# mohammadmarghzari/monte-carlo-portfolio

Measured on AMD Instinct MI355X. Metric: simulated paths/sec (16 assets x 252 steps) + VaR abs-err vs NumPy ref, higher is better.
Workload: dtype f32; 1 GPU; configs[1]: 16 synthetic assets, 1,000,000 paths per GPU, 252 steps, fp32, full pass = paths + moments + exact VaR/CVaR; n_assets=16, n_steps=252, parallelism=path-sharded x1, math=exact

## Files before the change

### include/mcport.h

```cpp
#ifndef MCPORT_H
#define MCPORT_H

#include <stddef.h>
#include <stdint.h>

#ifdef __cplusplus
extern "C" {
#endif

#define MCP_ABI_VERSION 4
#define MCP_MAX_ASSETS 64
#define MCP_SELECT_BINS 2048
#define MCP_MAX_HORIZONS 64
#define MCP_MAX_LEVELS 16
#define MCP_MAX_BOOT_ROWS (1 << 20)
#define MCP_MAX_OVERLAY_ROWS 8
#define MCP_MAX_T_DOF 32
#define MCP_MAX_ATTR_PORTFOLIOS 16
#define MCP_MAX_JUMPS 8

enum {
    MCP_OK = 0,
    MCP_E_ARG = -1,
    MCP_E_NODEVICE = -2,
// ... 63 lines not shown
    MCP_EXCHANGE_P2P = 4
};
int mcp_ctx_exchange_mode(const mcp_ctx *ctx);
const char *mcp_ctx_exchange_note(const mcp_ctx *ctx);
void mcp_ctx_destroy(mcp_ctx *ctx);

int mcp_ctx_set_terminal_budget(mcp_ctx *ctx, size_t bytes);

int mcp_simulate(mcp_ctx *ctx, const mcp_params *prm,
                 const float *mu,
                 const float *chol,
                 const float *W,
                 uint64_t seed, uint64_t path_begin, uint64_t n_paths,
                 float *terminal_out,
                 mcp_stats *stats_out  );

int mcp_simulate_drawdown(mcp_ctx *ctx, const mcp_params *prm, const float *mu, const float *chol, const float *W,
                          uint64_t seed, uint64_t path_begin, uint64_t n_paths,
                          float *terminal_out,
                          mcp_stats *stats_out,
                          float *mdd_out,
                          mcp_stats *dd_stats_out  );

int mcp_simulate_horizons(mcp_ctx *ctx, const mcp_params *prm, const float *mu, const float *chol, const float *W,
                          uint64_t seed, uint64_t path_begin, uint64_t n_paths,
                          int n_horizons, const int32_t *horizons,
                          int n_levels, const double *levels,
                          float *terminal_out,
                          mcp_stats *stats_out,
                          float *horizon_out,
                          mcp_stats *hz_stats_out,
                          double *bands_out);

typedef struct {
    const float *rows;
    int32_t n_rows;
    int32_t reserved;
    double mean_block;
} mcp_bootstrap;

int mcp_simulate_bootstrap(mcp_ctx *ctx, const mcp_params *prm, const mcp_bootstrap *boot, const float *W, uint64_t seed,
                           uint64_t path_begin, uint64_t n_paths, float *terminal_out, mcp_stats *stats_out);
int mcp_simulate_bootstrap_horizons(mcp_ctx *ctx, const mcp_params *prm, const mcp_bootstrap *boot, const float *W,
                                    uint64_t seed, uint64_t path_begin, uint64_t n_paths,
                                    int n_horizons, const int32_t *horizons,
                                    int n_levels, const double *levels,
                                    float *terminal_out,
                                    mcp_stats *stats_out,
                                    float *horizon_out,
                                    mcp_stats *hz_stats_out,
                                    double *bands_out);
int mcp_bootstrap_pivots(const mcp_params *prm, const mcp_bootstrap *boot, const float *W, double *pivots_out );

typedef struct {
    int32_t period;
    int32_t reserved;
    double cost;
} mcp_rebalance;

int mcp_simulate_rebalanced(mcp_ctx *ctx, const mcp_params *prm, const mcp_rebalance *reb,
                            const float *mu, const float *chol,
                            const mcp_bootstrap *boot,
                            const float *W, uint64_t seed, uint64_t path_begin, uint64_t n_paths,
                            int n_horizons, const int32_t *horizons,
                            int n_levels, const double *levels,
                            float *terminal_out,
                            mcp_stats *stats_out,
                            float *horizon_out,
                            mcp_stats *hz_stats_out,
                            double *bands_out);
int mcp_rebalance_pivots(const mcp_params *prm, const mcp_rebalance *reb, const float *mu, const mcp_bootstrap *boot,
                         const float *W, double *pivots_out );

typedef struct {
    int32_t dof;
    int32_t reserved;
} mcp_student_t;

int mcp_simulate_student_t(mcp_ctx *ctx, const mcp_params *prm, const mcp_student_t *st,
                           const float *mu, const float *chol, const float *W,
                           uint64_t seed, uint64_t path_begin, uint64_t n_paths,
                           int n_horizons, const int32_t *horizons, int n_levels, const double *levels,
                           float *terminal_out,
                           mcp_stats *stats_out,
                           float *mdd_out,
                           mcp_stats *dd_stats_out,
                           float *horizon_out,
                           mcp_stats *hz_stats_out,
                           double *bands_out);

typedef struct {
    double alpha, beta, h0;
    uint64_t reserved;
} mcp_garch;

int mcp_simulate_garch(mcp_ctx *ctx, const mcp_params *prm, const mcp_garch *g,
                       const mcp_student_t *st,
                       const float *mu, const float *chol, const float *W,
                       uint64_t seed, uint64_t path_begin, uint64_t n_paths,
                       int n_horizons, const int32_t *horizons, int n_levels, const double *levels,
                       float *terminal_out,
                       mcp_stats *stats_out,
                       float *mdd_out,
                       mcp_stats *dd_stats_out,
                       float *horizon_out,
                       mcp_stats *hz_stats_out,
                       double *bands_out);

typedef struct {
    const float *mu, *resid, *shock;
    int32_t n_rows;
    int32_t reserved;
    double mean_block;
} mcp_filtered;

int mcp_simulate_filtered(mcp_ctx *ctx, const mcp_params *prm, const mcp_filtered *filt, const mcp_garch *g, const float *W,
                          uint64_t seed, uint64_t path_begin, uint64_t n_paths,
                          int n_horizons, const int32_t *horizons, int n_levels, const double *levels,
                          float *terminal_out,
                          mcp_stats *stats_out,
                          float *horizon_out,
                          mcp_stats *hz_stats_out,
                          double *bands_out);
int mcp_filtered_pivots(const mcp_params *prm, const mcp_filtered *filt, const float *W, double *pivots_out );

typedef struct {
    double intensity, mean, std;
    const float *loading;
    int32_t reserved;
} mcp_jumps;

int mcp_simulate_jumps(mcp_ctx *ctx, const mcp_params *prm, const mcp_jumps *j,
                       const float *mu, const float *chol, const float *W,
                       uint64_t seed, uint64_t path_begin, uint64_t n_paths,
                       int n_horizons, const int32_t *horizons, int n_levels, const double *levels,
                       float *terminal_out,
                       mcp_stats *stats_out,
                       float *mdd_out,
                       mcp_stats *dd_stats_out,
                       float *horizon_out,
                       mcp_stats *hz_stats_out,
                       double *bands_out);
int mcp_jump_consts(const mcp_jumps *j, int n_assets, const float *mu,
                    uint32_t *thr_out , double *mean_count_out, float *drift_out );

typedef struct {
    double p01, p10, start;
    const float *mu1;
    const float *chol1;
    int32_t reserved;
} mcp_regimes;

int mcp_simulate_regimes(mcp_ctx *ctx, const mcp_params *prm, const mcp_regimes *r,
                         const float *mu, const float *chol, const float *W,
                         uint64_t seed, uint64_t path_begin, uint64_t n_paths,
                         int n_horizons, const int32_t *horizons, int n_levels, const double *levels,
                         float *terminal_out,
                         mcp_stats *stats_out,
                         float *mdd_out,
                         mcp_stats *dd_stats_out,
                         float *horizon_out,
                         mcp_stats *hz_stats_out,
                         double *bands_out);
int mcp_regime_consts(const mcp_regimes *r, uint64_t *thr_out , double *p_out );
int mcp_regime_pivots(const mcp_params *prm, const mcp_regimes *r, const float *mu, const float *W,
                      int n_horizons, const int32_t *horizons, double *pivots_out , double *hz_pivots_out );

typedef struct {
    uint64_t n_pairs, reserved;
    double cross, pair_cov, pair_corr, mean_se, mean_se_iid;
} mcp_pair;

int mcp_simulate_antithetic(mcp_ctx *ctx, const mcp_params *prm,
                            const mcp_garch *g,
                            const mcp_student_t *st,
                            const float *mu, const float *chol, const float *W,
                            uint64_t seed, uint64_t path_begin, uint64_t n_paths,
                            int n_horizons, const int32_t *horizons, int n_levels, const double *levels,
                            float *terminal_out,
                            mcp_stats *stats_out,
                            float *mdd_out,
                            mcp_stats *dd_stats_out,
                            float *horizon_out,
                            mcp_stats *hz_stats_out,
                            double *bands_out,
                            mcp_pair *pair_out);

typedef struct {
    double mean;
    double cvar;
    double vol;
    double sum, sum_tail, sum_xc;
} mcp_attr;

int mcp_simulate_attribution(mcp_ctx *ctx, const mcp_params *prm,
                             const mcp_garch *g,
                             const mcp_student_t *st,
                             const float *mu, const float *chol, const float *W,
                             uint64_t seed, uint64_t path_begin, uint64_t n_paths,
                             float *terminal_out,
                             mcp_stats *stats_out,
                             float *contrib_out,
                             mcp_attr *attr_out,
                             uint64_t *attr_counts_out);

typedef struct {
    const float *flows;
    int32_t n_flows;
    int32_t has_target;
    double target;
} mcp_cashflow;

int mcp_simulate_cashflow(mcp_ctx *ctx, const mcp_params *prm, const mcp_cashflow *cf,
                          const float *mu, const float *chol,
                          const mcp_bootstrap *boot,
                          const mcp_student_t *st,
                          const float *W, uint64_t seed, uint64_t path_begin, uint64_t n_paths,
                          int n_horizons, const int32_t *horizons, int n_levels, const double *levels,
                          float *terminal_out,
                          mcp_stats *stats_out,
                          uint64_t *counts_out,
                          float *horizon_out,
                          mcp_stats *hz_stats_out,
                          double *bands_out,
                          uint64_t *hz_counts_out);
int mcp_cashflow_pivots(const mcp_params *prm, const mcp_cashflow *cf, const float *mu, const mcp_bootstrap *boot,
                        const float *W, double *pivots_out );

#define MCP_OVERLAY_LINEAR 0
#define MCP_OVERLAY_CALL 1
#define MCP_OVERLAY_PUT 2
typedef struct {
    int32_t kind;
    float strike, premium, qty;
} mcp_overlay_row;
typedef struct {
    const mcp_overlay_row *rows;
    const int32_t *row_begin;
    const float *spot;
    int32_t n_rows;
    int32_t reserved;
} mcp_overlay;

int mcp_simulate_overlay(mcp_ctx *ctx, const mcp_params *prm, const mcp_overlay *ov,
                         const float *mu, const float *chol,
                         const mcp_student_t *st,
                         const float *W, uint64_t seed, uint64_t path_begin, uint64_t n_paths,
                         int n_horizons, const int32_t *horizons, int n_levels, const double *levels,
                         float *terminal_out,
                         mcp_stats *stats_out,
                         float *mdd_out,
                         mcp_stats *dd_stats_out,
                         float *horizon_out,
                         mcp_stats *hz_stats_out,
                         double *bands_out);
int mcp_overlay_pivots(const mcp_params *prm, const mcp_overlay *ov, const float *mu, const float *W,
                       double *pivots_out );

#define MCP_SWEEP_MAX_ROWS 4096
int mcp_sweep_historical(mcp_ctx *ctx, int n_assets, int n_rows, int n_portfolios, const double *returns,
                         const double *mean, const double *cov, const double *W, double rf, double alpha,
                         double *port_return, double *port_std, double *sharpe, double *var, double *cvar);


enum {
    MCP_WS_PARTIALS = 0,
    MCP_WS_RECORD = 1,
    MCP_WS_STATE = 2,
    MCP_WS_HIST = 3,
    MCP_WS_QUANT = 4,
    MCP_WS_STATS = 5,
    MCP_WS_BELOW = 6,
    MCP_WS_PIVOT = 7,
    MCP_WS_COUNT = 8
};
size_t mcp_ws_bytes(int which, int n_portfolios, uint64_t n_paths);
uint64_t mcp_moment_slots(int n_portfolios, uint64_t n_paths);

size_t mcp_packed_len(int n_assets, int n_portfolios);
int mcp_pack_params(int n_assets, int n_portfolios, const float *mu, const float *chol, const float *W,
                    float *packed_out, size_t packed_len);
int mcp_pivots(const mcp_params *prm, const float *mu, const float *chol, const float *W, double *pivots_out );

int mcp_launch_paths(const mcp_params *prm, const float *d_packed, const double *d_pivot, uint64_t seed, uint64_t path_begin,
                     uint64_t n_paths, float *d_terminal, uint64_t terminal_stride, void *d_partials, void *d_hist,
                     void *stream);
int mcp_launch_paths_drawdown(const mcp_params *prm, const float *d_packed, const double *d_pivot, uint64_t seed,
                              uint64_t path_begin, uint64_t n_paths, float *d_terminal, uint64_t terminal_stride,
                              float *d_mdd, uint64_t mdd_stride, void *d_partials, void *d_hist, void *stream);
int mcp_launch_paths_horizons(const mcp_params *prm, const float *d_packed, const double *d_pivot, uint64_t seed,
                              uint64_t path_begin, uint64_t n_paths, float *d_terminal, uint64_t terminal_stride,
                              int n_horizons, const int32_t *horizons, float *d_horizon, uint64_t horizon_stride,
                              void *d_partials, void *d_hist, void *stream);

int mcp_percentile_rank(uint64_t n_total, double alpha, uint64_t *rank_lo, uint64_t *rank_hi, double *gamma);
int mcp_percentile_rank_q(uint64_t n_total, double q, uint64_t *rank_lo, uint64_t *rank_hi, double *gamma);

int mcp_launch_pass0(const mcp_params *prm, const float *d_terminal, uint64_t terminal_stride, uint64_t n,
                     const double *d_pivot, void *d_partials, void *d_hist, void *stream);
int mcp_launch_scan(const mcp_params *prm, int pass, uint64_t n, uint64_t rank_lo, uint64_t rank_hi, const void *d_partials,
                    const void *d_below, const double *d_pivot, void *d_hist, void *d_state, void *d_record, void *stream);
int mcp_launch_hist(const mcp_params *prm, int pass, const float *d_terminal, uint64_t terminal_stride, uint64_t n,
                    const void *d_state, const double *d_pivot, void *d_below, void *d_hist, void *stream);
int mcp_launch_final(const mcp_params *prm, uint64_t n, double gamma, uint64_t rank_lo, uint64_t rank_hi,
                     const void *d_below, void *d_hist, const void *d_state, void *d_record, void *d_quant,
                     void *d_stats, void *stream);
int mcp_launch_stats(const mcp_params *prm, int world, const void *d_gathered, const void *d_quant, void *d_stats,
                     void *stream);
int mcp_launch_sum_u64(void *const *d_bufs, int n_bufs, size_t words, void *stream);

int mcp_stream_create(int device, int reserve_cus, void **stream_out);
int mcp_stream_destroy(void *stream);

int mcp_launch_normals(const uint32_t *d_x, uint64_t n, float *d_z, void *stream);

int mcp_icdf_table(float *out, size_t out_len);

uint32_t mcp_float_to_key(float v);
float mcp_key_to_float(uint32_t key);
double mcp_terminal_to_x(const mcp_params *prm, float terminal);

#ifdef __cplusplus
}
#endif
#endif
```

### monte_carlo_portfolio_amd/_ffi.py

```python
from __future__ import annotations

import ctypes
import importlib.util
import os
import subprocess
import sys

import numpy as np

_PKG = os.path.dirname(os.path.abspath(__file__))
LIB_PATH = os.environ.get("MCP_LIB_PATH") or os.path.join(_PKG, "libmcport.so")
CSRC = os.path.join(_PKG, "csrc")

MCP_ABI_VERSION = 4
MCP_MAX_ASSETS = 64
MCP_SELECT_BINS = 2048
MCP_MAX_HORIZONS = 64
MCP_MAX_LEVELS = 16
MCP_MAX_BOOT_ROWS = 1 << 20
MCP_MAX_T_DOF = 32
MCP_MAX_OVERLAY_ROWS = 8
MCP_MAX_ATTR_PORTFOLIOS = 16
MCP_MAX_JUMPS = 8
MCP_OVERLAY_LINEAR, MCP_OVERLAY_CALL, MCP_OVERLAY_PUT = 0, 1, 2
MCP_COMPOUND = {"simple": 0, "log": 1}
MCP_FLAG_NATIVE_MATH = 1
MCP_FLAG_FOLD = 2
MCP_FLAG_SHARD_PORTFOLIOS = 4
MCP_E_ARG, MCP_E_NODEVICE, MCP_E_NOMEM, MCP_E_UNSUPPORTED, MCP_E_HIP, MCP_E_COMM = -1, -2, -3, -4, -5, -6
(WS_PARTIALS, WS_RECORD, WS_STATE, WS_HIST, WS_QUANT, WS_STATS, WS_BELOW, WS_PIVOT) = range(8)
WS_COUNT = 8
(EXCHANGE_UNSET, EXCHANGE_NONE, EXCHANGE_RCCL, EXCHANGE_KERNEL, EXCHANGE_P2P) = range(5)


class McpError(RuntimeError):
    """Raised for any negative return code of the C ABI; carries mcp_last_error()."""


class McpParams(ctypes.Structure):
    _fields_ = [
        ("n_assets", ctypes.c_int32), ("n_steps", ctypes.c_int32), ("n_portfolios", ctypes.c_int32),
        ("compounding", ctypes.c_int32), ("flags", ctypes.c_int32), ("reserved", ctypes.c_int32),
        ("v0", ctypes.c_double), ("alpha", ctypes.c_double), ("rf", ctypes.c_double),
    ]


class McpStats(ctypes.Structure):
    _fields_ = [
        ("n", ctypes.c_uint64), ("n_tail", ctypes.c_uint64), ("mean", ctypes.c_double), ("m2", ctypes.c_double),
        ("std", ctypes.c_double), ("sharpe", ctypes.c_double), ("var", ctypes.c_double), ("cvar", ctypes.c_double),
        ("min", ctypes.c_double), ("max", ctypes.c_double), ("sum_tail", ctypes.c_double),
        ("x_lo", ctypes.c_double), ("x_hi", ctypes.c_double),
    ]


class McpBootstrap(ctypes.Structure):
    _fields_ = [("rows", ctypes.c_void_p), ("n_rows", ctypes.c_int32), ("reserved", ctypes.c_int32), ("mean_block", ctypes.c_double)]


class McpRebalance(ctypes.Structure):
    _fields_ = [("period", ctypes.c_int32), ("reserved", ctypes.c_int32), ("cost", ctypes.c_double)]


class McpStudentT(ctypes.Structure):
    _fields_ = [("dof", ctypes.c_int32), ("reserved", ctypes.c_int32)]


class McpFiltered(ctypes.Structure):
    _fields_ = [("mu", ctypes.c_void_p), ("resid", ctypes.c_void_p), ("shock", ctypes.c_void_p), ("n_rows", ctypes.c_int32),
                ("reserved", ctypes.c_int32), ("mean_block", ctypes.c_double)]


class McpGarch(ctypes.Structure):
    _fields_ = [("alpha", ctypes.c_double), ("beta", ctypes.c_double), ("h0", ctypes.c_double), ("reserved", ctypes.c_uint64)]


class McpJumps(ctypes.Structure):
    _fields_ = [("intensity", ctypes.c_double), ("mean", ctypes.c_double), ("std", ctypes.c_double), ("loading", ctypes.c_void_p),
                ("reserved", ctypes.c_int32)]


class McpRegimes(ctypes.Structure):
    _fields_ = [("p01", ctypes.c_double), ("p10", ctypes.c_double), ("start", ctypes.c_double), ("mu1", ctypes.c_void_p),
                ("chol1", ctypes.c_void_p), ("reserved", ctypes.c_int32)]


class McpCashflow(ctypes.Structure):
    _fields_ = [("flows", ctypes.c_void_p), ("n_flows", ctypes.c_int32), ("has_target", ctypes.c_int32), ("target", ctypes.c_double)]


class McpOverlay(ctypes.Structure):
    _fields_ = [("rows", ctypes.c_void_p), ("row_begin", ctypes.c_void_p), ("spot", ctypes.c_void_p), ("n_rows", ctypes.c_int32),
                ("reserved", ctypes.c_int32)]


OVERLAY_ROW_DTYPE = np.dtype([("kind", np.int32), ("strike", np.float32), ("premium", np.float32), ("qty", np.float32)])
assert OVERLAY_ROW_DTYPE.itemsize == 16

STATS_DTYPE = np.dtype([
    ("n", np.uint64), ("n_tail", np.uint64), ("mean", np.float64), ("m2", np.float64), ("std", np.float64),
    ("sharpe", np.float64), ("var", np.float64), ("cvar", np.float64), ("min", np.float64), ("max", np.float64),
    ("sum_tail", np.float64), ("x_lo", np.float64), ("x_hi", np.float64),
])
assert STATS_DTYPE.itemsize == ctypes.sizeof(McpStats)

ATTR_DTYPE = np.dtype([("mean", np.float64), ("cvar", np.float64), ("vol", np.float64), ("sum", np.float64), ("sum_tail", np.float64),
                       ("sum_xc", np.float64)])
assert ATTR_DTYPE.itemsize == 48

PAIR_DTYPE = np.dtype([("n_pairs", np.uint64), ("reserved", np.uint64), ("cross", np.float64), ("pair_cov", np.float64),
                       ("pair_corr", np.float64), ("mean_se", np.float64), ("mean_se_iid", np.float64)])
assert PAIR_DTYPE.itemsize == 56

RECORD_DTYPE = np.dtype([("n", np.float64), ("sum", np.float64), ("sumsq", np.float64), ("min", np.float64),
                         ("max", np.float64), ("below", np.float64), ("pivot", np.float64), ("pad", np.float64)])
PARTIAL_DTYPE = np.dtype([("s1", np.float64), ("s2", np.float64), ("vmin", np.float32), ("vmax", np.float32), ("n", np.uint64)])
assert PARTIAL_DTYPE.itemsize == 32
QUANT_DTYPE = np.dtype([("x_lo", np.float64), ("x_hi", np.float64), ("var", np.float64), ("level2", np.float64),
                        ("n_tail", np.uint64), ("pad", np.uint64)])
RECORD_DOUBLES = RECORD_DTYPE.itemsize // 8

_f32p = np.ctypeslib.ndpointer(dtype=np.float32, flags="C_CONTIGUOUS")
_f64p = np.ctypeslib.ndpointer(dtype=np.float64, flags="C_CONTIGUOUS")
_vp = ctypes.c_void_p
_u64 = ctypes.c_uint64
_int = ctypes.c_int
_PP = ctypes.POINTER(McpParams)

SIGNATURES = {
    "mcp_abi_version": (_int, []),
    "mcp_device_count": (_int, []),
    "mcp_last_error": (ctypes.c_char_p, []),
    "mcp_ctx_create": (_int, [_int, ctypes.POINTER(_vp)]),
    "mcp_ctx_create_multi": (_int, [ctypes.POINTER(_int), _int, ctypes.POINTER(_vp)]),
    "mcp_ctx_device_count": (_int, [_vp]),
    "mcp_ctx_exchange_mode": (_int, [_vp]),
    "mcp_ctx_exchange_note": (ctypes.c_char_p, [_vp]),
    "mcp_ctx_set_terminal_budget": (_int, [_vp, ctypes.c_size_t]),
    "mcp_ctx_destroy": (None, [_vp]),
    "mcp_simulate": (_int, [_vp, _PP, _f32p, _f32p, _f32p, _u64, _u64, _u64, _vp, _vp]),
    "mcp_sweep_historical": (_int, [_vp, _int, _int, _int, _f64p, _f64p, _f64p, _f64p, ctypes.c_double, ctypes.c_double,
                                    _f64p, _f64p, _f64p, _f64p, _f64p]),
    "mcp_ws_bytes": (ctypes.c_size_t, [_int, _int, _u64]),
    "mcp_moment_slots": (_u64, [_int, _u64]),
    "mcp_pivots": (_int, [_PP, _f32p, _f32p, _f32p, _f64p]),
    "mcp_packed_len": (ctypes.c_size_t, [_int, _int]),
    "mcp_pack_params": (_int, [_int, _int, _f32p, _f32p, _f32p, _f32p, ctypes.c_size_t]),
    "mcp_launch_paths": (_int, [_PP, _vp, _vp, _u64, _u64, _u64, _vp, _u64, _vp, _vp, _vp]),
    "mcp_simulate_drawdown": (_int, [_vp, _PP, _f32p, _f32p, _f32p, _u64, _u64, _u64, _vp, _vp, _vp, _vp]),
    "mcp_launch_paths_drawdown": (_int, [_PP, _vp, _vp, _u64, _u64, _u64, _vp, _u64, _vp, _u64, _vp, _vp, _vp]),
    "mcp_simulate_horizons": (_int, [_vp, _PP, _f32p, _f32p, _f32p, _u64, _u64, _u64, _int, _vp, _int, _vp, _vp, _vp, _vp, _vp,
                                     _vp]),
    "mcp_launch_paths_horizons": (_int, [_PP, _vp, _vp, _u64, _u64, _u64, _vp, _u64, _int, _vp, _vp, _u64, _vp, _vp, _vp]),
    "mcp_simulate_bootstrap": (_int, [_vp, _PP, ctypes.POINTER(McpBootstrap), _f32p, _u64, _u64, _u64, _vp, _vp]),
    "mcp_simulate_bootstrap_horizons": (_int, [_vp, _PP, ctypes.POINTER(McpBootstrap), _f32p, _u64, _u64, _u64, _int, _vp, _int, _vp,
                                               _vp, _vp, _vp, _vp, _vp]),
    "mcp_bootstrap_pivots": (_int, [_PP, ctypes.POINTER(McpBootstrap), _f32p, _f64p]),
    "mcp_simulate_rebalanced": (_int, [_vp, _PP, ctypes.POINTER(McpRebalance), _vp, _vp, ctypes.POINTER(McpBootstrap), _f32p, _u64, _u64,
                                       _u64, _int, _vp, _int, _vp, _vp, _vp, _vp, _vp, _vp]),
    "mcp_rebalance_pivots": (_int, [_PP, ctypes.POINTER(McpRebalance), _vp, ctypes.POINTER(McpBootstrap), _f32p, _f64p]),
    "mcp_simulate_student_t": (_int, [_vp, _PP, ctypes.POINTER(McpStudentT), _vp, _vp, _vp, _u64, _u64, _u64, _int, _vp, _int, _vp, _vp,
                                      _vp, _vp, _vp, _vp, _vp, _vp]),
    "mcp_simulate_garch": (_int, [_vp, _PP, ctypes.POINTER(McpGarch), ctypes.POINTER(McpStudentT), _vp, _vp, _vp, _u64, _u64, _u64, _int,
                                  _vp, _int, _vp, _vp, _vp, _vp, _vp, _vp, _vp, _vp]),
    "mcp_simulate_filtered": (_int, [_vp, _PP, ctypes.POINTER(McpFiltered), ctypes.POINTER(McpGarch), _vp, _u64, _u64, _u64, _int, _vp,
                                     _int, _vp, _vp, _vp, _vp, _vp, _vp]),
    "mcp_filtered_pivots": (_int, [_PP, ctypes.POINTER(McpFiltered), _f32p, _f64p]),
    "mcp_simulate_jumps": (_int, [_vp, _PP, ctypes.POINTER(McpJumps), _vp, _vp, _vp, _u64, _u64, _u64, _int, _vp, _int, _vp, _vp, _vp,
                                  _vp, _vp, _vp, _vp, _vp]),
    "mcp_jump_consts": (_int, [ctypes.POINTER(McpJumps), _int, _vp, _vp, ctypes.POINTER(ctypes.c_double), _vp]),
    "mcp_simulate_regimes": (_int, [_vp, _PP, ctypes.POINTER(McpRegimes), _vp, _vp, _vp, _u64, _u64, _u64, _int, _vp, _int, _vp, _vp, _vp,
                                    _vp, _vp, _vp, _vp, _vp]),
    "mcp_regime_consts": (_int, [ctypes.POINTER(McpRegimes), _vp, _vp]),
    "mcp_regime_pivots": (_int, [_PP, ctypes.POINTER(McpRegimes), _vp, _vp, _int, _vp, _vp, _vp]),
    "mcp_simulate_attribution": (_int, [_vp, _PP, ctypes.POINTER(McpGarch), ctypes.POINTER(McpStudentT), _vp, _vp, _vp, _u64, _u64, _u64,
                                        _vp, _vp, _vp, _vp, _vp]),
    "mcp_simulate_antithetic": (_int, [_vp, _PP, ctypes.POINTER(McpGarch), ctypes.POINTER(McpStudentT), _vp, _vp, _vp, _u64, _u64, _u64,
                                       _int, _vp, _int, _vp, _vp, _vp, _vp, _vp, _vp, _vp, _vp, _vp]),
    "mcp_simulate_cashflow": (_int, [_vp, _PP, ctypes.POINTER(McpCashflow), _vp, _vp, ctypes.POINTER(McpBootstrap),
                                     ctypes.POINTER(McpStudentT), _vp, _u64, _u64, _u64, _int, _vp, _int, _vp, _vp, _vp, _vp, _vp, _vp,
                                     _vp, _vp]),
    "mcp_cashflow_pivots": (_int, [_PP, ctypes.POINTER(McpCashflow), _vp, ctypes.POINTER(McpBootstrap), _f32p, _f64p]),
    "mcp_simulate_overlay": (_int, [_vp, _PP, ctypes.POINTER(McpOverlay), _vp, _vp, ctypes.POINTER(McpStudentT), _vp, _u64, _u64, _u64,
                                    _int, _vp, _int, _vp, _vp, _vp, _vp, _vp, _vp, _vp, _vp]),
    "mcp_overlay_pivots": (_int, [_PP, ctypes.POINTER(McpOverlay), _f32p, _f32p, _f64p]),
    "mcp_percentile_rank_q": (_int, [_u64, ctypes.c_double, ctypes.POINTER(_u64), ctypes.POINTER(_u64),
                                     ctypes.POINTER(ctypes.c_double)]),
    "mcp_percentile_rank": (_int, [_u64, ctypes.c_double, ctypes.POINTER(_u64), ctypes.POINTER(_u64),
                                   ctypes.POINTER(ctypes.c_double)]),
    "mcp_launch_pass0": (_int, [_PP, _vp, _u64, _u64, _vp, _vp, _vp, _vp]),
    "mcp_launch_scan": (_int, [_PP, _int, _u64, _u64, _u64, _vp, _vp, _vp, _vp, _vp, _vp, _vp]),
    "mcp_launch_hist": (_int, [_PP, _int, _vp, _u64, _u64, _vp, _vp, _vp, _vp, _vp]),
    "mcp_launch_final": (_int, [_PP, _u64, ctypes.c_double, _u64, _u64, _vp, _vp, _vp, _vp, _vp, _vp, _vp]),
    "mcp_launch_stats": (_int, [_PP, _int, _vp, _vp, _vp, _vp]),
    "mcp_launch_sum_u64": (_int, [ctypes.POINTER(_vp), _int, ctypes.c_size_t, _vp]),
    "mcp_stream_create": (_int, [_int, _int, ctypes.POINTER(_vp)]),
    "mcp_stream_destroy": (_int, [_vp]),
    "mcp_launch_normals": (_int, [_vp, _u64, _vp, _vp]),
    "mcp_icdf_table": (_int, [_f32p, ctypes.c_size_t]),
    "mcp_float_to_key": (ctypes.c_uint32, [ctypes.c_float]),
    "mcp_key_to_float": (ctypes.c_float, [ctypes.c_uint32]),
    "mcp_terminal_to_x": (ctypes.c_double, [_PP, ctypes.c_float]),
}

_LIB = None


def build(force: bool = False, jobs: int = 8) -> str:
    cmd = ["make", "-C", CSRC, f"-j{jobs}"] + (["-B"] if force else [])
    res = subprocess.run(cmd, capture_output=True, text=True)
    if res.returncode != 0:
        raise RuntimeError("building libmcport.so failed:\n" + res.stdout[-4000:] + res.stderr[-4000:])
    return LIB_PATH


def _preload_hip_runtime() -> None:
    if "torch" in sys.modules:
        return
    try:
        spec = importlib.util.find_spec("torch")
    except (ImportError, ValueError):
        spec = None
    if spec is not None and spec.origin:
        cand = os.path.join(os.path.dirname(spec.origin), "lib", "libamdhip64.so")
        if os.path.exists(cand):
            ctypes.CDLL(cand, mode=ctypes.RTLD_GLOBAL)


def preload_rccl() -> None:
    if os.environ.get("MCP_RCCL_LIB"):
        return
    try:
        spec = importlib.util.find_spec("torch")
    except (ImportError, ValueError):
        spec = None
    if spec is not None and spec.origin:
        cand = os.path.join(os.path.dirname(spec.origin), "lib", "librccl.so")
        if os.path.exists(cand):
            try:
                ctypes.CDLL(cand)
            except OSError:
                pass


def lib() -> ctypes.CDLL:
    global _LIB
    if _LIB is None:
        _preload_hip_runtime()
        if not os.path.exists(LIB_PATH):
            raise ImportError(
                f"{LIB_PATH} is missing: build it with `make -C {CSRC} -j8` (or __graft_entry__.build()). "
                "There is no CPU fallback for the path engine.")
        L = ctypes.CDLL(LIB_PATH)
        for name, (res, args) in SIGNATURES.items():
            fn = getattr(L, name)
            fn.restype = res
            fn.argtypes = args
        got = L.mcp_abi_version()
        if got != MCP_ABI_VERSION:
            raise ImportError(f"libmcport.so ABI {got} != binding ABI {MCP_ABI_VERSION}; rebuild")
        _LIB = L
    return _LIB


def check(rc: int) -> int:
    if rc < 0:
        raise McpError(f"libmcport error {rc}: {lib().mcp_last_error().decode('utf-8', 'replace')}")
    return rc


def make_params(n_assets, n_steps, n_portfolios, compounding="simple", v0=1.0, alpha=0.95, rf=0.0,
                native_math=False, fold=False, shard_portfolios=False) -> McpParams:
    if compounding not in MCP_COMPOUND:
        raise ValueError(f"compounding must be 'simple' or 'log', got {compounding!r}")
    return McpParams(int(n_assets), int(n_steps), int(n_portfolios), MCP_COMPOUND[compounding],
                     (MCP_FLAG_NATIVE_MATH if native_math else 0) | (MCP_FLAG_FOLD if fold else 0)
                     | (MCP_FLAG_SHARD_PORTFOLIOS if shard_portfolios else 0), 0,
                     float(v0), float(alpha), float(rf))


def pack_params(mu: np.ndarray, chol: np.ndarray, W: np.ndarray) -> np.ndarray:
    n = mu.shape[0]
    k = W.shape[0]
    out = np.zeros(lib().mcp_packed_len(n, k), np.float32)
    check(lib().mcp_pack_params(n, k, mu, chol, W, out, out.size))
    return out


def pivots(prm: McpParams, mu: np.ndarray, chol: np.ndarray, W: np.ndarray) -> np.ndarray:
    out = np.zeros(W.shape[0], np.float64)
    check(lib().mcp_pivots(ctypes.byref(prm), mu, chol, W, out))
    return out


def make_bootstrap(rows: np.ndarray, block: float) -> McpBootstrap:
    if rows.dtype != np.float32 or rows.ndim != 2 or not rows.flags.c_contiguous:
        raise ValueError("bootstrap rows must be a C-contiguous float32 [R, N] array")
    return McpBootstrap(rows.ctypes.data_as(ctypes.c_void_p), int(rows.shape[0]), 0, float(block))


def make_filtered(mu: np.ndarray, resid: np.ndarray, shock: np.ndarray, block: float) -> McpFiltered:
    for a, nd in ((mu, 1), (resid, 2), (shock, 1)):
        if a.dtype != np.float32 or a.ndim != nd or not a.flags.c_contiguous:
            raise ValueError("filtered mu [N], resid [R, N] and shock [R] must be C-contiguous float32 arrays")
    if resid.shape != (shock.shape[0], mu.shape[0]):
        raise ValueError(f"filtered resid has shape {resid.shape}, mu and shock want {(shock.shape[0], mu.shape[0])}")
    return McpFiltered(mu.ctypes.data_as(ctypes.c_void_p), resid.ctypes.data_as(ctypes.c_void_p), shock.ctypes.data_as(ctypes.c_void_p),
                       int(resid.shape[0]), 0, float(block))


def filtered_pivots(prm: McpParams, mu: np.ndarray, resid: np.ndarray, shock: np.ndarray, W: np.ndarray) -> np.ndarray:
    out = np.zeros(W.shape[0], np.float64)
    mu, resid, shock = (np.ascontiguousarray(a, np.float32) for a in (mu, resid, shock))
    ft = make_filtered(mu, resid, shock, 1.0)
    check(lib().mcp_filtered_pivots(ctypes.byref(prm), ctypes.byref(ft), W, out))
    return out


def make_jumps(intensity: float, mean: float, std: float, loading: np.ndarray | None = None) -> McpJumps:
    if loading is not None and (loading.dtype != np.float32 or loading.ndim != 1 or not loading.flags.c_contiguous):
        raise ValueError("jump loadings must be a C-contiguous float32 [N] array")
    return McpJumps(float(intensity), float(mean), float(std), loading.ctypes.data_as(ctypes.c_void_p) if loading is not None else None, 0)


def jump_consts(intensity: float, mean: float, std: float, loading=None, mu=None, n_assets: int | None = None):
    ld = np.ascontiguousarray(loading, np.float32) if loading is not None else None
    mu32 = np.ascontiguousarray(mu, np.float32) if mu is not None else None
    n = mu32.size if mu32 is not None else ld.size if ld is not None else int(n_assets or 1)
    thr = np.zeros(MCP_MAX_JUMPS, np.uint32)
    mean_count = ctypes.c_double()
    drift = np.zeros(n, np.float32) if mu32 is not None else None
    jp = make_jumps(intensity, mean, std, ld)
    ptr = lambda a: a.ctypes.data_as(_vp) if a is not None else None
    check(lib().mcp_jump_consts(ctypes.byref(jp), n, ptr(mu32), ptr(thr), ctypes.byref(mean_count), ptr(drift)))
    return thr, mean_count.value, drift


def make_regimes(p01: float, p10: float, start: float, mu1: np.ndarray | None, chol1: np.ndarray | None) -> McpRegimes:
    for a, nd in ((mu1, 1), (chol1, 2)):
        if a is not None and (a.dtype != np.float32 or a.ndim != nd or not a.flags.c_contiguous):
            raise ValueError("regime mu1 [N] and chol1 [N, N] must be C-contiguous float32 arrays")
    ptr = lambda a: a.ctypes.data_as(ctypes.c_void_p) if a is not None else None
    return McpRegimes(float(p01), float(p10), float(start), ptr(mu1), ptr(chol1), 0)


def regime_consts(p01: float, p10: float, start: float):
    thr, p = np.zeros(3, np.uint64), np.zeros(3, np.float64)
    rs = make_regimes(p01, p10, start, None, None)
    check(lib().mcp_regime_consts(ctypes.byref(rs), thr.ctypes.data_as(_vp), p.ctypes.data_as(_vp)))
    return thr, p


def regime_pivots(prm: McpParams, regimes, mu: np.ndarray, mu1: np.ndarray, W: np.ndarray, horizons=None):
    mu, mu1 = (np.ascontiguousarray(a, np.float32) for a in (mu, mu1))
    W = np.ascontiguousarray(W, np.float32)
    n = mu.size
    chol1 = np.zeros((n, n), np.float32)
    rs = make_regimes(*regimes, mu1, chol1)
    hz = np.ascontiguousarray(horizons, np.int32) if horizons is not None and len(horizons) else None
    out = np.zeros(W.shape[0], np.float64)
    hout = np.zeros((hz.size, W.shape[0]), np.float64) if hz is not None else None
    ptr = lambda a: a.ctypes.data_as(_vp) if a is not None else None
    check(lib().mcp_regime_pivots(ctypes.byref(prm), ctypes.byref(rs), ptr(mu), ptr(W), 0 if hz is None else hz.size, ptr(hz), ptr(out),
                                  ptr(hout)))
    return out, hout


def bootstrap_pivots(prm: McpParams, rows: np.ndarray, W: np.ndarray, block: float = 1.0) -> np.ndarray:
    out = np.zeros(W.shape[0], np.float64)
    rows = np.ascontiguousarray(rows, np.float32)
    bt = make_bootstrap(rows, block)
    check(lib().mcp_bootstrap_pivots(ctypes.byref(prm), ctypes.byref(bt), W, out))
    return out


def rebalance_pivots(prm: McpParams, period: int, W: np.ndarray, mu: np.ndarray | None = None, rows: np.ndarray | None = None,
                     cost: float = 0.0) -> np.ndarray:
    out = np.zeros(W.shape[0], np.float64)
    rb = McpRebalance(int(period), 0, float(cost))
    mu_p = np.ascontiguousarray(mu, np.float32) if mu is not None else None
    bt = make_bootstrap(np.ascontiguousarray(rows, np.float32), 1.0) if rows is not None else None
    check(lib().mcp_rebalance_pivots(ctypes.byref(prm), ctypes.byref(rb), mu_p.ctypes.data_as(_vp) if mu_p is not None else None,
                                     ctypes.byref(bt) if bt is not None else None, W, out))
    return out


def make_cashflow(flows: np.ndarray, target=None) -> McpCashflow:
    if flows.dtype != np.float32 or flows.ndim != 1 or not flows.flags.c_contiguous:
        raise ValueError("cash flows must be a C-contiguous float32 [n_steps] array")
    return McpCashflow(flows.ctypes.data_as(ctypes.c_void_p) if flows.size else None, int(flows.size), 0 if target is None else 1,
                       0.0 if target is None else float(target))


def cashflow_pivots(prm: McpParams, flows: np.ndarray, W: np.ndarray, mu: np.ndarray | None = None,
                    rows: np.ndarray | None = None) -> np.ndarray:
    out = np.zeros(W.shape[0], np.float64)
    flows = np.ascontiguousarray(flows, np.float32)
    cf = make_cashflow(flows)
    mu_p = np.ascontiguousarray(mu, np.float32) if mu is not None else None
    bt = make_bootstrap(np.ascontiguousarray(rows, np.float32), 1.0) if rows is not None else None
    check(lib().mcp_cashflow_pivots(ctypes.byref(prm), ctypes.byref(cf), mu_p.ctypes.data_as(_vp) if mu_p is not None else None,
                                    ctypes.byref(bt) if bt is not None else None, W, out))
    return out


def make_overlay(rows: np.ndarray, row_begin: np.ndarray, spot: np.ndarray) -> McpOverlay:
    if rows.dtype != OVERLAY_ROW_DTYPE or rows.ndim != 1 or not rows.flags.c_contiguous:
        raise ValueError("overlay rows must be a C-contiguous [n_rows] array of OVERLAY_ROW_DTYPE")
    if row_begin.dtype != np.int32 or spot.dtype != np.float32 or row_begin.ndim != 1 or spot.ndim != 1 or row_begin.size != spot.size + 1:
        raise ValueError("overlay row_begin must be int32 [N + 1] and spot float32 [N]")
    return McpOverlay(rows.ctypes.data_as(ctypes.c_void_p) if rows.size else None, row_begin.ctypes.data_as(ctypes.c_void_p),
                      spot.ctypes.data_as(ctypes.c_void_p), int(rows.size), 0)


def overlay_pivots(prm: McpParams, overlay, mu: np.ndarray, W: np.ndarray) -> np.ndarray:
    out = np.zeros(W.shape[0], np.float64)
    ov = make_overlay(*overlay)
    check(lib().mcp_overlay_pivots(ctypes.byref(prm), ctypes.byref(ov), np.ascontiguousarray(mu, np.float32), W, out))
    return out


def percentile_rank_q(n_total: int, q: float):
    lo, hi, g = _u64(), _u64(), ctypes.c_double()
    check(lib().mcp_percentile_rank_q(n_total, q, ctypes.byref(lo), ctypes.byref(hi), ctypes.byref(g)))
    return lo.value, hi.value, g.value


def percentile_rank(n_total: int, alpha: float):
    lo, hi, g = _u64(), _u64(), ctypes.c_double()
    check(lib().mcp_percentile_rank(n_total, alpha, ctypes.byref(lo), ctypes.byref(hi), ctypes.byref(g)))
    return lo.value, hi.value, g.value
```

### monte_carlo_portfolio_amd/csrc/mcp_api.cpp

```cpp
#include <hip/hip_runtime.h>
#include <dlfcn.h>

#include <algorithm>
#include <cmath>
#include <cstdarg>
#include <cstdio>
#include <cstdlib>
#include <cstring>
#include <mutex>
#include <new>
#include <string>
#include <vector>

#include "../../include/mcport.h"
#include "mcp_device.h"
#include "mcp_paths.h"
#include "mcp_stats_kernels.h"

#ifndef MCP_EXP_LEAN
#define MCP_EXP_LEAN 1
#endif

namespace {

thread_local std::string g_err;

int fail(int code, const char* fmt, ...) {
  char buf[512];
  va_list ap;
  va_start(ap, fmt);
  vsnprintf(buf, sizeof buf, fmt, ap);
  va_end(ap);
  g_err = buf;
  return code;
}

#define HIP_TRY(expr)                                                                       \
  do {                                                                                      \
    hipError_t e_ = (expr);                                                                 \
    if (e_ != hipSuccess) return fail(MCP_E_HIP, "%s: %s", #expr, hipGetErrorString(e_)); \
  } while (0)

constexpr int KT_WIDE = 8;
constexpr int K_PAD = 512;
using mcp::SWEEP_MIN_K;

int env_sweep_mt() {
  static const int v = [] { const char* e = getenv("MCP_SWEEP_MT"); return e ? atoi(e) : 0; }();
  return v;
}
bool uses_sweep(int K) { return K >= SWEEP_MIN_K && env_sweep_mt() >= 0; }

struct SweepSeg { bool shared; int mt, k_begin, k_count; };
int sweep_plan(int K, int nb, SweepSeg* out) {
  int n = 0;
  const int env_mt = env_sweep_mt();
  if (nb <= 4 && env_mt > 0) {
    out[n++] = {false, env_mt, 0, K};
    return n;
  }
  const int big = nb <= 4 ? 4 : 2, W = 128 * big;
  const int full = (K / W) * W;
  if (full) out[n++] = {true, big, 0, full};
  const int r = K - full;
  if (r == 0) return n;
  if (nb <= 4) {
    const auto per_wave = [](int k) { return k > 64 ? 4 : (k > 32 ? 2 : 1); };
    if (r <= 128) out[n++] = {false, per_wave(r), full, r};
    else if (r <= 256) out[n++] = {true, 2, full, r};
    else if (r <= 384) { out[n++] = {true, 2, full, 256}; out[n++] = {false, per_wave(r - 256), full + 256, r - 256}; }
    else out[n++] = {true, 4, full, r};
  } else {
    out[n++] = {true, r <= 128 ? 1 : 2, full, r};
  }
  return n;
}

inline int n4_of(int n) { return 4 * ((n + 3) / 4); }
inline size_t regime_block_len(int n) { const size_t n4 = (size_t)n4_of(n); return n4 + n4 * (n4 / 2 + 1); }
inline int kpad_of(int k) { return k >= SWEEP_MIN_K ? K_PAD * ((k + K_PAD - 1) / K_PAD) : KT_WIDE * ((k + KT_WIDE - 1) / KT_WIDE); }

int check_params(const mcp_params* p) {
  if (!p) return fail(MCP_E_ARG, "params is NULL");
  if (p->n_assets < 1 || p->n_assets > MCP_MAX_ASSETS)
    return fail(MCP_E_ARG, "n_assets=%d outside [1,%d]", p->n_assets, MCP_MAX_ASSETS);
  if (p->n_steps < 0) return fail(MCP_E_ARG, "n_steps=%d < 0", p->n_steps);
  if (p->n_portfolios < 1) return fail(MCP_E_ARG, "n_portfolios=%d < 1", p->n_portfolios);
  if (p->compounding != MCP_COMPOUND_SIMPLE && p->compounding != MCP_COMPOUND_LOG)
    return fail(MCP_E_ARG, "compounding=%d unknown", p->compounding);
  if (!(p->alpha > 0.0 && p->alpha < 1.0)) return fail(MCP_E_ARG, "alpha=%g outside (0,1)", p->alpha);
  if (!(p->v0 > 0.0) || !std::isfinite(p->v0)) return fail(MCP_E_ARG, "v0=%g must be positive", p->v0);
  return MCP_OK;
}

const mcp::launch_paths_fn k_launch[16] = {
    mcp::launch_paths_nb1,  mcp::launch_paths_nb2,  mcp::launch_paths_nb3,  mcp::launch_paths_nb4,
    mcp::launch_paths_nb5,  mcp::launch_paths_nb6,  mcp::launch_paths_nb7,  mcp::launch_paths_nb8,
    mcp::launch_paths_nb9,  mcp::launch_paths_nb10, mcp::launch_paths_nb11, mcp::launch_paths_nb12,
    mcp::launch_paths_nb13, mcp::launch_paths_nb14, mcp::launch_paths_nb15, mcp::launch_paths_nb16};

int check_horizons(int n_steps, int H, const int32_t* steps) {
  if (H < 1 || H > MCP_MAX_HORIZONS) return fail(MCP_E_ARG, "n_horizons=%d outside [1,%d]", H, MCP_MAX_HORIZONS);
  if (!steps) return fail(MCP_E_ARG, "horizons is NULL");
  for (int i = 0; i < H; i++) {
    if (steps[i] < 1 || steps[i] > n_steps) return fail(MCP_E_ARG, "horizon %d = %d outside [1, n_steps=%d]", i, steps[i], n_steps);
    if (i && steps[i] <= steps[i - 1]) return fail(MCP_E_ARG, "horizons must be strictly increasing (%d after %d)", steps[i], steps[i - 1]);
  }
  return MCP_OK;
}

int check_levels(int L, const double* levels) {
  if (L < 0 || L > MCP_MAX_LEVELS) return fail(MCP_E_ARG, "n_levels=%d outside [0,%d]", L, MCP_MAX_LEVELS);
  if (L && !levels) return fail(MCP_E_ARG, "levels is NULL");
  for (int i = 0; i < L; i++)
    if (!(levels[i] >= 0.0 && levels[i] <= 100.0)) return fail(MCP_E_ARG, "level %d = %g outside [0, 100]", i, levels[i]);
  return MCP_OK;
}

int check_boot(const mcp_params* prm, const mcp_bootstrap* boot) {
  if (!boot) return fail(MCP_E_ARG, "bootstrap is NULL");
  if (!boot->rows) return fail(MCP_E_ARG, "bootstrap rows is NULL");
  if (boot->n_rows < 1 || boot->n_rows > MCP_MAX_BOOT_ROWS)
    return fail(MCP_E_ARG, "n_rows=%d outside [1,%d]", boot->n_rows, MCP_MAX_BOOT_ROWS);
  const double b = boot->mean_block;
  if (!(b >= 1.0)) return fail(MCP_E_ARG, "mean_block=%g must be >= 1 (or +inf)", b);
  const size_t n = (size_t)boot->n_rows * (size_t)prm->n_assets;
  for (size_t i = 0; i < n; i++)
    if (!std::isfinite(boot->rows[i]))
      return fail(MCP_E_ARG, "bootstrap row %zu, asset %zu is not finite", i / (size_t)prm->n_assets, i % (size_t)prm->n_assets);
  return MCP_OK;
}

uint64_t boot_threshold(double b) {
  const double q = 4294967296.0 / b;
  return q >= 4294967296.0 ? (uint64_t)1 << 32 : (uint64_t)q;
}

void boot_moments(int N, const mcp_bootstrap* boot, const float* W, int K, double* m_out, double* s2_out) {
  const int R = boot->n_rows;
  std::vector<double> rho((size_t)R);
  for (int k = 0; k < K; k++) {
    const float* w = W + (size_t)k * N;
    double sum = 0.0;
    for (int j = 0; j < R; j++) {
      const float* r = boot->rows + (size_t)j * N;
      double v = 0.0;
      for (int i = 0; i < N; i++) v += (double)w[i] * (double)r[i];
      rho[(size_t)j] = v;
      sum += v;
    }
    const double m = sum / (double)R;
    double ss = 0.0;
    for (int j = 0; j < R; j++) { const double d = rho[(size_t)j] - m; ss += d * d; }
    m_out[k] = m;
    s2_out[k] = ss / (double)R;
  }
}

double boot_pivot(int compounding, int T, double m, double s2) {
  const double c = compounding == MCP_COMPOUND_LOG ? std::expm1((double)T * (m + 0.5 * s2))
                                                   : (m > -1.0 ? std::expm1((double)T * std::log1p(m)) : 0.0);
  return std::isfinite(c) ? c : 0.0;
}

int check_reb(const mcp_rebalance* reb) {
  if (!reb) return fail(MCP_E_ARG, "rebalance is NULL");
  if (reb->period < 0) return fail(MCP_E_ARG, "rebalance period=%d < 0", reb->period);
  if (reb->reserved != 0) return fail(MCP_E_ARG, "rebalance reserved=%d must be 0", reb->reserved);
  if (!(reb->cost >= 0.0 && reb->cost < 1.0)) return fail(MCP_E_ARG, "rebalance cost=%g outside [0, 1)", reb->cost);
  return MCP_OK;
}

int check_student_t(const mcp_params* prm, const mcp_student_t* st) {
  if (!st) return fail(MCP_E_ARG, "student_t is NULL");
  if (st->dof < 3 || st->dof > MCP_MAX_T_DOF) return fail(MCP_E_ARG, "dof=%d outside [3,%d]", st->dof, MCP_MAX_T_DOF);
  if (st->reserved != 0) return fail(MCP_E_ARG, "student_t reserved=%d must be 0", st->reserved);
  if ((uint64_t)prm->n_steps * (uint64_t)((st->dof + 3) / 4) > 0xFFFFFFFFull)
    return fail(MCP_E_ARG, "n_steps * ceil(dof/4) = %llu exceeds the 32-bit Philox block counter of stream 2",
                (unsigned long long)((uint64_t)prm->n_steps * (uint64_t)((st->dof + 3) / 4)));
  return MCP_OK;
}

struct GarchConsts { float a, b, g, omega, a_n; };
GarchConsts garch_consts(const mcp_garch* g, int N) {
  GarchConsts c;
  c.a = (float)g->alpha;
  c.b = (float)g->beta;
  c.g = (float)g->h0;
  c.omega = (float)(1.0 - (double)c.a - (double)c.b);
  c.a_n = (float)((double)c.a / (double)N);
  return c;
}

int check_garch(const mcp_params* prm, const mcp_garch* g) {
  if (!g) return fail(MCP_E_ARG, "garch is NULL");
  if (g->reserved != 0) return fail(MCP_E_ARG, "garch reserved=%llu must be 0", (unsigned long long)g->reserved);
  if (!std::isfinite(g->alpha) || !std::isfinite(g->beta) || !std::isfinite(g->h0))
    return fail(MCP_E_ARG, "garch alpha=%g, beta=%g, h0=%g must be finite", g->alpha, g->beta, g->h0);
  const GarchConsts c = garch_consts(g, prm->n_assets);
  if (!std::isfinite(c.a) || !std::isfinite(c.b) || !std::isfinite(c.g))
    return fail(MCP_E_ARG, "garch alpha=%g, beta=%g, h0=%g must be finite in binary32", g->alpha, g->beta, g->h0);
  if (!(c.a >= 0.0f) || !(c.b >= 0.0f)) return fail(MCP_E_ARG, "garch alpha=%g and beta=%g must be >= 0", g->alpha, g->beta);
  if (!((double)c.a + (double)c.b < 1.0) || !(c.omega > 0.0f))
    return fail(MCP_E_ARG, "garch alpha + beta = %.9g must be < 1 in binary32", (double)c.a + (double)c.b);
  if (!(c.g > 0.0f)) return fail(MCP_E_ARG, "garch h0=%g must be > 0 in binary32", g->h0);
  return MCP_OK;
}

struct JumpConsts { uint32_t thr[MCP_MAX_JUMPS]; double mean_count; float m, s; };
JumpConsts jump_consts(const mcp_jumps* j) {
  JumpConsts c;
  double p = std::exp(-j->intensity), cum = 0.0;
  c.mean_count = 0.0;
  for (int k = 1; k <= MCP_MAX_JUMPS; k++) {
    cum = cum + p;
    double v = std::floor((1.0 - cum) * 4294967296.0);
    v = v < 0.0 ? 0.0 : v > 4294967295.0 ? 4294967295.0 : v;
    c.thr[k - 1] = (uint32_t)v;
    c.mean_count += (double)c.thr[k - 1] / 4294967296.0;
    p = p * j->intensity / (double)k;
  }
  c.m = (float)j->mean;
  c.s = (float)j->std;
  return c;
}
void jump_drift(const mcp_jumps* j, const JumpConsts& c, int N, const float* mu, float* out) {
  const double d = (double)c.m * c.mean_count;
  for (int i = 0; i < N; i++) {
    const float b = j->loading ? j->loading[i] : 1.0f;
    out[i] = (d == 0.0 || b == 0.0f) ? mu[i] : (float)((double)mu[i] - (double)b * d);
  }
}

int check_jumps(int n_assets, const mcp_jumps* j) {
  if (!j) return fail(MCP_E_ARG, "jumps is NULL");
  if (j->reserved != 0) return fail(MCP_E_ARG, "jumps reserved=%d must be 0", j->reserved);
  if (!std::isfinite(j->intensity) || !std::isfinite(j->mean) || !std::isfinite(j->std))
    return fail(MCP_E_ARG, "jumps intensity=%g, mean=%g, std=%g must be finite", j->intensity, j->mean, j->std);
  if (!std::isfinite((float)j->intensity) || !std::isfinite((float)j->mean) || !std::isfinite((float)j->std))
    return fail(MCP_E_ARG, "jumps intensity=%g, mean=%g, std=%g must be finite in binary32", j->intensity, j->mean, j->std);
  if (!(j->intensity >= 0.0 && j->intensity <= 1.0)) return fail(MCP_E_ARG, "jumps intensity=%g outside [0, 1]", j->intensity);
  if (!(j->std >= 0.0)) return fail(MCP_E_ARG, "jumps std=%g must be >= 0", j->std);
  for (int i = 0; j->loading && i < n_assets; i++)
    if (!std::isfinite(j->loading[i])) return fail(MCP_E_ARG, "jumps loading, asset %d is not finite", i);
  return MCP_OK;
}

struct RegimeConsts { uint64_t thr01, thr10, thr_start; double p01, p10, start; };
inline uint64_t regime_thr(double p) {
  const double v = std::floor(p * 4294967296.0);
  return v >= 4294967296.0 ? (uint64_t)1 << 32 : (uint64_t)v;
}
RegimeConsts regime_consts(const mcp_regimes* r) {
  RegimeConsts c;
  c.thr01 = regime_thr(r->p01);
  c.thr10 = regime_thr(r->p10);
  c.thr_start = regime_thr(r->start);
  c.p01 = (double)c.thr01 / 4294967296.0;
  c.p10 = (double)c.thr10 / 4294967296.0;
  c.start = (double)c.thr_start / 4294967296.0;
  return c;
}

int check_regimes(int n_assets, const mcp_regimes* r) {
  if (!r) return fail(MCP_E_ARG, "regimes is NULL");
  if (r->reserved != 0) return fail(MCP_E_ARG, "regimes reserved=%d must be 0", r->reserved);
  if (!std::isfinite(r->p01) || !std::isfinite(r->p10) || !std::isfinite(r->start))
    return fail(MCP_E_ARG, "regimes p01=%g, p10=%g, start=%g must be finite", r->p01, r->p10, r->start);
  if (!(r->p01 >= 0.0 && r->p01 <= 1.0) || !(r->p10 >= 0.0 && r->p10 <= 1.0) || !(r->start >= 0.0 && r->start <= 1.0))
    return fail(MCP_E_ARG, "regimes p01=%g, p10=%g, start=%g outside [0, 1]", r->p01, r->p10, r->start);
  if (!r->mu1 || !r->chol1) return fail(MCP_E_ARG, "regimes mu1 or chol1 is NULL");
  for (int i = 0; i < n_assets; i++)
    if (!std::isfinite(r->mu1[i])) return fail(MCP_E_ARG, "regimes mu1, asset %d is not finite", i);
  for (size_t i = 0; i < (size_t)n_assets * n_assets; i++)
    if (!std::isfinite(r->chol1[i])) return fail(MCP_E_ARG, "regimes chol1, entry %zu is not finite", i);
  return MCP_OK;
}

void regime_pivots(int N, int K, int T, const float* mu0, const float* mu1, const RegimeConsts& c, const float* W, int H, const int32_t* steps,
                   double* out_T, double* out_hz) {
  for (int k = 0; k < K; k++) {
    const float* w = W + (size_t)k * N;
    double d0 = 0.0, d1 = 0.0;
    for (int i = 0; i < N; i++) d0 += (double)w[i] * (double)(mu0[i] + 0.0f);
    for (int i = 0; i < N; i++) d1 += (double)w[i] * (double)(mu1[i] + 0.0f);
    const bool only0 = c.thr_start == 0 && c.thr01 == 0, only1 = c.thr_start == ((uint64_t)1 << 32) && c.thr10 == 0;
    const bool one_drift = d0 == d1 || only0 || only1;
    const double m = only1 ? d1 : d0;
    d0 = 1.0 + d0;
    d1 = 1.0 + d1;
    double v0 = (1.0 - c.start) * d0, v1 = c.start * d1;
    int hi = 0;
    if (out_T) out_T[k] = 0.0;
    for (int h = 1; h <= T; h++) {
      if (h > 1) {
        const double u0 = v0 * (1.0 - c.p01) + v1 * c.p10, u1 = v0 * c.p01 + v1 * (1.0 - c.p10);
        v0 = u0 * d0;
        v1 = u1 * d1;
      }
      const double ch = one_drift ? (m > -1.0 ? std::expm1((double)h * std::log1p(m)) : 0.0) : (v0 + v1) - 1.0;
      const double piv = std::isfinite(ch) ? ch : 0.0;
      if (hi < H && steps[hi] == h) out_hz[(size_t)hi++ * K + k] = piv;
      if (h == T && out_T) out_T[k] = piv;
    }
  }
}

int check_filtered(const mcp_params* prm, const mcp_filtered* f) {
  if (!f) return fail(MCP_E_ARG, "filtered is NULL");
  if (!f->mu) return fail(MCP_E_ARG, "filtered mu is NULL");
  if (!f->resid) return fail(MCP_E_ARG, "filtered resid is NULL");
  if (!f->shock) return fail(MCP_E_ARG, "filtered shock is NULL");
  if (f->n_rows < 1 || f->n_rows > MCP_MAX_BOOT_ROWS) return fail(MCP_E_ARG, "filtered n_rows=%d outside [1,%d]", f->n_rows, MCP_MAX_BOOT_ROWS);
  if (f->reserved != 0) return fail(MCP_E_ARG, "filtered reserved=%d must be 0", f->reserved);
  if (!(f->mean_block >= 1.0)) return fail(MCP_E_ARG, "filtered mean_block=%g must be >= 1 (or +inf)", f->mean_block);
  const size_t N = (size_t)prm->n_assets, R = (size_t)f->n_rows;
  for (size_t i = 0; i < N; i++)
    if (!std::isfinite(f->mu[i])) return fail(MCP_E_ARG, "filtered mu, asset %zu is not finite", i);
  for (size_t i = 0; i < R * N; i++)
    if (!std::isfinite(f->resid[i])) return fail(MCP_E_ARG, "filtered resid row %zu, asset %zu is not finite", i / N, i % N);
  for (size_t j = 0; j < R; j++) {
    if (!std::isfinite(f->shock[j])) return fail(MCP_E_ARG, "filtered shock, row %zu is not finite", j);
    if (!(f->shock[j] >= 0.0f)) return fail(MCP_E_ARG, "filtered shock, row %zu = %g is negative", j, (double)f->shock[j]);
// ... 731 lines not shown
static mcp::BootArgs boot_block(const Request& rq, const Launch& ln) {
  mcp::BootArgs bt;
  const bool on = rq.src == SRC_BOOT || rq.src == SRC_FHS;
  bt.rows = on ? (const float4*)ln.d_rows : nullptr;
  bt.thr = on ? boot_threshold(rows_of(rq).mean_block) : 0;
  bt.n_rows = on ? (uint32_t)rows_of(rq).n_rows : 0;
  bt.pad = 0;
  return bt;
}
static mcp::FiltArgs filt_block(const Request& rq, const Launch& ln, int n_assets) {
  const GarchConsts c = garch_consts(rq.gv, n_assets);
  mcp::FiltArgs fh;
  fh.shock = ln.d_rows + (size_t)rq.filt->n_rows * (size_t)n4_of(n_assets);
  fh.a = c.a;
  fh.b = c.b;
  fh.omega = c.omega;
  fh.h0 = c.g;
  return fh;
}
static mcp::StudentArgs student_block(const Request& rq) {
  mcp::StudentArgs st;
  st.dof = rq.src == SRC_T ? rq.st->dof : 0;
  st.pad = 0;
  return st;
}
static mcp::GarchArgs garch_block(const mcp_garch* g, int n_assets) {
  const GarchConsts c = garch_consts(g, n_assets);
  mcp::GarchArgs gv;
  gv.a_n = c.a_n;
  gv.b = c.b;
  gv.omega = c.omega;
  gv.h0 = c.g;
  gv.n_assets = n_assets;
  gv.pad = 0;
  return gv;
}
static mcp::JumpArgs jump_block(const Request& rq, const Launch& ln) {
  const JumpConsts c = jump_consts(rq.jp);
  mcp::JumpArgs jp;
  jp.loading = ln.d_loading;
  for (int k = 0; k < MCP_MAX_JUMPS; k++) jp.thr[k] = c.thr[k];
  jp.m = c.m;
  jp.s = c.s;
  return jp;
}
static mcp::RegimeArgs regime_block(const Request& rq, const Launch& ln) {
  const RegimeConsts c = regime_consts(rq.rs);
  mcp::RegimeArgs rs;
  rs.block1 = ln.d_block1;
  rs.thr01 = c.thr01;
  rs.thr10 = c.thr10;
  rs.thr_start = c.thr_start;
  return rs;
}
static mcp::OverlayArgs overlay_block(const Request& rq, const Launch& ln, int n_assets) {
  mcp::OverlayArgs ov;
  const size_t row_bytes = (size_t)rq.ov->n_rows * sizeof(mcp_overlay_row);
  ov.rows = (const mcp_overlay_row*)ln.d_overlay;
  ov.row_begin = (const int32_t*)(ln.d_overlay + row_bytes);
  ov.spot = (const float*)(ln.d_overlay + row_bytes) + n4_of(n_assets) + 1;
  ov.mask = 0;
  for (int i = 0; i < n_assets; i++)
    if (rq.ov->row_begin[i + 1] > rq.ov->row_begin[i]) ov.mask |= (uint64_t)1 << i;
  return ov;
}
static mcp::AttrArgs attr_block(const Launch& ln, int n_assets) {
  mcp::AttrArgs at;
  at.var = ln.d_var;
  at.partials = ln.d_attr_partials;
  at.contrib = ln.d_contrib;
  at.contrib_stride = ln.contrib_stride;
  at.n_assets = n_assets;
  at.pad = 0;
  return at;
}

static int launch_paths_impl(const mcp_params* prm, const Request& rq, const Launch& ln) {
  const int N = prm->n_assets, nb = (N + 3) / 4;
  const int K = prm->n_portfolios;
  const bool plain = rq.src == SRC_GAUSS && !rq.dd && !rq.hz && !rq.rebalanced && !rq.cash && !rq.overlay && !rq.garch && !rq.jumps && !rq.regimes;
  mcp::PathLaunchArgs s = {};
  mcp::PathArgs& a = s.hz;
  const float4* tables = nullptr;
  int dev = 0;
  if (int rc = stream_device(ln.stream, &dev)) return rc;
  DeviceGuard guard(dev);
  if (guard.err != hipSuccess) return fail(MCP_E_HIP, "hipSetDevice(%d): %s", dev, hipGetErrorString(guard.err));
  if (int rc = device_tables(dev, ln.stream, &tables)) return rc;
  const bool sweep = plain && !ln.attr && !rq.anti && uses_sweep(K);
  a.tables = tables;
  a.packed = ln.d_packed;
  a.terminal = ln.d_terminal;
  a.pivot = ln.d_pivot;
  a.partials = (mcp::MomentPartial*)ln.d_partials;
  a.hist = sweep ? nullptr : (unsigned long long*)ln.d_hist;
  a.slots = mcp_moment_slots(K, ln.n_paths);
  a.v0d = (double)(float)prm->v0;
  a.inv_v0d = 1.0 / a.v0d;
  { int e = 0; a.v0_pow2 = std::frexp(a.v0d, &e) == 0.5; }
  a.seed = ln.seed;
  a.path_begin = ln.path_begin;
  a.n_paths = ln.n_paths;
  a.stride = ln.stride;
  a.n_steps = prm->n_steps;
  a.n_portfolios = K;
  a.compounding = prm->compounding;
  a.v0 = (float)prm->v0;
  a.k_count = K;
  a.fold_offset = (uint32_t)(n4_of(N) + n4_of(N) * (n4_of(N) / 2 + 1) + kpad_of(K) * n4_of(N));
  if (rq.anti) {
    if ((ln.path_begin | ln.n_paths | ln.stride | (rq.dd ? ln.mdd_stride : 0) | (rq.hz ? ln.hz_stride : 0)) & 1)
      return fail(MCP_E_ARG, "antithetic pairs: a launch begins, ends and strides at even path ids");
    a.path_begin = ln.path_begin / 2;
    a.n_paths = ln.n_paths / 2;
    s.pr.cross = ln.d_partials ? ln.d_cross : nullptr;
  }
  if (sweep) {
    const bool native = (prm->flags & MCP_FLAG_NATIVE_MATH) != 0;
    SweepSeg segs[4];
    const int n_seg = sweep_plan(K, nb, segs);
    hipError_t e = hipSuccess;
    for (int i = 0; i < n_seg && e == hipSuccess; i++) {
      a.k_begin = segs[i].k_begin;
      a.k_count = segs[i].k_count;
      e = segs[i].shared ? mcp::launch_sweep_shared(nb, segs[i].mt, native, a, ln.stream)
                         : mcp::launch_sweep_paths(nb, segs[i].mt, native, a, ln.stream);
    }
    if (e != hipSuccess) return fail(MCP_E_HIP, "mc_sweep_kernel launch: %s", hipGetErrorString(e));
    if (ln.d_hist) {
      e = mcp::launch_hist(*prm, K, 0, ln.d_terminal, ln.stride, ln.n_paths, nullptr, ln.d_pivot, nullptr, (unsigned long long*)ln.d_hist,
                           ln.stream);
      if (e != hipSuccess) return fail(MCP_E_HIP, "hist_kernel<0> launch: %s", hipGetErrorString(e));
    }
    return MCP_OK;
  }
  if ((!plain || rq.anti) && ln.d_partials && a.slots > (uint64_t)mcp::path_grid(a.n_paths))
    HIP_TRY(mcp::launch_pass0(*prm, K, ln.d_terminal, ln.stride, 0, nullptr, a.slots, (mcp::MomentPartial*)ln.d_partials,
                              (unsigned long long*)ln.d_hist, ln.stream));
  fill_hz(s.hz, rq, ln);
  s.mdd = rq.dd ? ln.d_mdd : nullptr;
  s.mdd_stride = rq.dd ? ln.mdd_stride : 0;
  s.bt = boot_block(rq, ln);
  s.st = student_block(rq);
  if (rq.garch) s.gv = garch_block(rq.gv, N);
  if (rq.cash) s.cf.flows = ln.d_flows;
  if (rq.overlay) s.ov = overlay_block(rq, ln, N);
  if (rq.rebalanced) { s.period = rq.reb->period; s.cost = (float)rq.reb->cost; }
  if (rq.src == SRC_FHS) s.fh = filt_block(rq, ln, N);
  if (rq.jumps) s.jp = jump_block(rq, ln);
  if (rq.regimes) s.rs = regime_block(rq, ln);
  mcp::PathKernel k = {};
  k.logc = prm->compounding == MCP_COMPOUND_LOG;
  k.fh = rq.src == SRC_FHS;
  k.boot = rq.src == SRC_BOOT || k.fh;
  k.blds = k.fh ? mcp::filt_fits_lds((uint64_t)rq.filt->n_rows, nb) : k.boot && mcp::boot_fits_lds((uint64_t)rq.boot->n_rows, nb);
  k.stt = rq.src == SRC_T;
  if (ln.attr) {
    static const mcp_garch none = {0.0, 0.0, 1.0, 0};
    k.family = mcp::FAM_AT;
    k.stt = k.gv = true;
    a.partials = nullptr;
    a.hist = nullptr;
    if (!rq.garch) s.gv = garch_block(&none, N);
    s.at = attr_block(ln, N);
  } else {
    k.family = rq.overlay ? mcp::FAM_OV : rq.cash ? mcp::FAM_CF : rq.rebalanced ? mcp::FAM_REB : rq.dd ? mcp::FAM_DD : rq.hz ? mcp::FAM_HZ : mcp::FAM_PLAIN;
    k.dd = rq.overlay && rq.dd;
    k.gv = rq.garch;
    k.jp = rq.jumps;
    k.rs = rq.regimes;
    k.kt8 = K > 1;
    k.native = (prm->flags & MCP_FLAG_NATIVE_MATH) != 0;
    k.fold = (prm->flags & MCP_FLAG_FOLD) != 0;
    k.uhi = MCP_EXP_LEAN && plain && !rq.anti && !k.kt8 && !k.native && !k.fold && nb <= mcp::LEAN_MAX_NB && mcp::lean_range(a.path_begin, a.n_paths);
    if (rq.anti) {
      static const mcp_garch none = {0.0, 0.0, 1.0, 0};
      k.anti = true;
      if (k.stt || k.gv) {
        k.stt = k.gv = true;
        if (!rq.garch) s.gv = garch_block(&none, N);
      }
    }
  }
  const hipError_t e = k_launch[nb - 1](k, s, ln.stream);
  if (e != hipSuccess) return fail(MCP_E_HIP, "path kernel launch (family %d): %s", k.family, hipGetErrorString(e));
  return MCP_OK;
}

static Launch make_launch(const float* d_packed, const double* d_pivot, uint64_t seed, uint64_t path_begin, uint64_t n_paths,
                          float* d_terminal, uint64_t stride, void* d_partials, void* d_hist, void* stream) {
  Launch ln;
  ln.d_packed = d_packed;
  ln.d_pivot = d_pivot;
  ln.seed = seed;
  ln.path_begin = path_begin;
  ln.n_paths = n_paths;
  ln.d_terminal = d_terminal;
  ln.stride = stride;
  ln.d_partials = d_partials;
  ln.d_hist = d_hist;
  ln.stream = (hipStream_t)stream;
  return ln;
}

static int launch_checked(const mcp_params* prm, const Request& rq, const Launch& ln) {
  if (int rc = check_request(prm, rq, ln.n_paths, &ln)) return rc;
  return launch_paths_impl(prm, rq, ln);
}

extern "C" {

int mcp_launch_paths(const mcp_params* prm, const float* d_packed, const double* d_pivot, uint64_t seed, uint64_t path_begin,
                     uint64_t n_paths, float* d_terminal, uint64_t stride, void* d_partials, void* d_hist, void* stream) {
  return launch_checked(prm, Request(), make_launch(d_packed, d_pivot, seed, path_begin, n_paths, d_terminal, stride, d_partials, d_hist, stream));
}

int mcp_launch_paths_drawdown(const mcp_params* prm, const float* d_packed, const double* d_pivot, uint64_t seed, uint64_t path_begin,
                              uint64_t n_paths, float* d_terminal, uint64_t terminal_stride, float* d_mdd, uint64_t mdd_stride,
                              void* d_partials, void* d_hist, void* stream) {
  Request rq;
  rq.dd = true;
  Launch ln = make_launch(d_packed, d_pivot, seed, path_begin, n_paths, d_terminal, terminal_stride, d_partials, d_hist, stream);
  ln.d_mdd = d_mdd;
  ln.mdd_stride = mdd_stride;
  return launch_checked(prm, rq, ln);
}

int mcp_launch_paths_horizons(const mcp_params* prm, const float* d_packed, const double* d_pivot, uint64_t seed, uint64_t path_begin,
                              uint64_t n_paths, float* d_terminal, uint64_t terminal_stride, int n_horizons, const int32_t* horizons,
                              float* d_horizon, uint64_t horizon_stride, void* d_partials, void* d_hist, void* stream) {
  Request rq;
  ask_horizons(rq, true, n_horizons, horizons, 0, nullptr, nullptr, nullptr, nullptr);
  Launch ln = make_launch(d_packed, d_pivot, seed, path_begin, n_paths, d_terminal, terminal_stride, d_partials, d_hist, stream);
  ln.d_hz = d_horizon;
  ln.hz_stride = horizon_stride;
  return launch_checked(prm, rq, ln);
}

#define MCP_ON_STREAM_DEVICE(stream)                                                                     \
  int dev_ = 0;                                                                                          \
  if (int rc_ = stream_device((hipStream_t)(stream), &dev_)) return rc_;                                 \
  DeviceGuard guard_(dev_);                                                                              \
  if (guard_.err != hipSuccess) return fail(MCP_E_HIP, "hipSetDevice(%d): %s", dev_, hipGetErrorString(guard_.err))

int mcp_percentile_rank(uint64_t n, double alpha, uint64_t* rank_lo, uint64_t* rank_hi, double* gamma) {
  if (n < 1 || !rank_lo || !rank_hi || !gamma) return fail(MCP_E_ARG, "bad argument");
  const double pct = (1.0 - alpha) * 100.0;
  const double q = pct / 100.0;
  const double vi = (double)(n - 1) * q;
  if (vi >= (double)(n - 1)) { *rank_lo = *rank_hi = n - 1; *gamma = 0.0; return MCP_OK; }
  if (vi < 0.0) { *rank_lo = *rank_hi = 0; *gamma = 0.0; return MCP_OK; }
  const double fl = std::floor(vi);
  *rank_lo = (uint64_t)fl;
  *rank_hi = *rank_lo + 1;
  *gamma = vi - fl;
  return MCP_OK;
}

int mcp_percentile_rank_q(uint64_t n, double q, uint64_t* rank_lo, uint64_t* rank_hi, double* gamma) {
  if (n < 1 || !rank_lo || !rank_hi || !gamma || !(q >= 0.0 && q <= 100.0)) return fail(MCP_E_ARG, "bad argument");
  const double qq = q / 100.0;
  const double vi = (double)(n - 1) * qq;
  if (vi >= (double)(n - 1)) { *rank_lo = *rank_hi = n - 1; *gamma = 0.0; return MCP_OK; }
  if (vi < 0.0) { *rank_lo = *rank_hi = 0; *gamma = 0.0; return MCP_OK; }
  const double fl = std::floor(vi);
  *rank_lo = (uint64_t)fl;
  *rank_hi = *rank_lo + 1;
  *gamma = vi - fl;
  return MCP_OK;
}

int mcp_launch_pass0(const mcp_params* prm, const float* d_terminal, uint64_t stride, uint64_t n, const double* d_pivot,
                     void* d_partials, void* d_hist, void* stream) {
  if (int rc = check_params(prm)) return rc;
  if (!d_terminal || !d_partials || !d_hist || stride < n) return fail(MCP_E_ARG, "bad argument");
  MCP_ON_STREAM_DEVICE(stream);
  HIP_TRY(mcp::launch_pass0(*prm, prm->n_portfolios, d_terminal, stride, n, d_pivot, mcp_moment_slots(prm->n_portfolios, n),
                            (mcp::MomentPartial*)d_partials, (unsigned long long*)d_hist, (hipStream_t)stream));
  return MCP_OK;
}

int mcp_launch_scan(const mcp_params* prm, int pass, uint64_t n, uint64_t rank_lo, uint64_t rank_hi, const void* d_partials,
                    const void* d_below, const double* d_pivot, void* d_hist, void* d_state, void* d_record, void* stream) {
  if (int rc = check_params(prm)) return rc;
  if (!d_partials || !d_below || !d_hist || !d_state || !d_record || pass < 0 || pass > 1) return fail(MCP_E_ARG, "bad argument");
  MCP_ON_STREAM_DEVICE(stream);
  HIP_TRY(mcp::launch_scan(*prm, prm->n_portfolios, pass, n, rank_lo, rank_hi, mcp_moment_slots(prm->n_portfolios, n),
                           (const mcp::MomentPartial*)d_partials, (const double*)d_below, d_pivot, (unsigned long long*)d_hist,
                           (mcp::SelectState*)d_state, (mcp_record*)d_record, (hipStream_t)stream));
  return MCP_OK;
}

int mcp_launch_hist(const mcp_params* prm, int pass, const float* d_terminal, uint64_t stride, uint64_t n,
                    const void* d_state, const double* d_pivot, void* d_below, void* d_hist, void* stream) {
  if (int rc = check_params(prm)) return rc;
  if (!d_terminal || !d_hist || pass < 0 || pass > 2 || stride < n || (pass > 0 && (!d_state || !d_below)))
    return fail(MCP_E_ARG, "bad argument");
  MCP_ON_STREAM_DEVICE(stream);
  HIP_TRY(mcp::launch_hist(*prm, prm->n_portfolios, pass, d_terminal, stride, n, (const mcp::SelectState*)d_state, d_pivot,
                           (double*)d_below, (unsigned long long*)d_hist, (hipStream_t)stream));
  return MCP_OK;
}

int mcp_launch_final(const mcp_params* prm, uint64_t n, double gamma, uint64_t rank_lo, uint64_t rank_hi,
                     const void* d_below, void* d_hist, const void* d_state, void* d_record, void* d_quant,
                     void* d_stats, void* stream) {
  if (int rc = check_params(prm)) return rc;
  if (!d_below || !d_hist || !d_state || !d_record || !d_quant) return fail(MCP_E_ARG, "NULL device pointer");
  MCP_ON_STREAM_DEVICE(stream);
  HIP_TRY(mcp::launch_final(*prm, prm->n_portfolios, n, gamma, rank_lo, rank_hi, (const double*)d_below,
                            (unsigned long long*)d_hist, (const mcp::SelectState*)d_state, (mcp_record*)d_record,
                            (mcp::Quantile*)d_quant, (mcp_stats*)d_stats, (hipStream_t)stream));
  return MCP_OK;
}

int mcp_launch_stats(const mcp_params* prm, int world, const void* d_gathered, const void* d_quant, void* d_stats,
                     void* stream) {
  if (int rc = check_params(prm)) return rc;
  if (world < 1 || !d_gathered || !d_quant || !d_stats) return fail(MCP_E_ARG, "bad argument");
  MCP_ON_STREAM_DEVICE(stream);
  HIP_TRY(mcp::launch_stats(*prm, prm->n_portfolios, world, (const mcp_record*)d_gathered, (const mcp::Quantile*)d_quant,
                            (mcp_stats*)d_stats, (hipStream_t)stream));
  return MCP_OK;
}

int mcp_launch_sum_u64(void* const* d_bufs, int n_bufs, size_t words, void* stream) {
  if (!d_bufs || n_bufs < 1 || n_bufs > 8) return fail(MCP_E_ARG, "n_bufs=%d outside [1,8]", n_bufs);
  for (int i = 0; i < n_bufs; i++)
    if (!d_bufs[i]) return fail(MCP_E_ARG, "NULL device pointer");
  MCP_ON_STREAM_DEVICE(stream);
  HIP_TRY(mcp::launch_sum_u64((unsigned long long* const*)d_bufs, n_bufs, words, (hipStream_t)stream));
  return MCP_OK;
}

int mcp_stream_create(int device, int reserve_cus, void** out) {
  if (!out) return fail(MCP_E_ARG, "stream_out is NULL");
  *out = nullptr;
  const int n = mcp_device_count();
  if (n <= 0) return fail(MCP_E_NODEVICE, "no HIP device visible");
  if (device < 0 || device >= n) return fail(MCP_E_ARG, "device %d outside [0,%d)", device, n);
  DeviceGuard guard(device);
  if (guard.err != hipSuccess) return fail(MCP_E_HIP, "hipSetDevice(%d): %s", device, hipGetErrorString(guard.err));
  hipStream_t s = nullptr;
  if (reserve_cus <= 0) {
    HIP_TRY(hipStreamCreateWithFlags(&s, hipStreamNonBlocking));
  } else {
    hipDeviceProp_t prop;
    HIP_TRY(hipGetDeviceProperties(&prop, device));
    const int cus = prop.multiProcessorCount;
    if (reserve_cus >= cus) return fail(MCP_E_ARG, "reserve_cus=%d leaves none of the %d compute units", reserve_cus, cus);
    std::vector<uint32_t> mask((size_t)(cus + 31) / 32, 0u);
    for (int i = 0; i < cus - reserve_cus; i++) mask[(size_t)i / 32] |= 1u << (i % 32);
    HIP_TRY(hipExtStreamCreateWithCUMask(&s, (uint32_t)mask.size(), mask.data()));
  }
  *out = (void*)s;
  return MCP_OK;
}

int mcp_stream_destroy(void* stream) {
  if (!stream) return fail(MCP_E_ARG, "stream is NULL");
  HIP_TRY(hipStreamDestroy((hipStream_t)stream));
  return MCP_OK;
}

int mcp_launch_normals(const uint32_t* d_x, uint64_t n, float* d_z, void* stream) {
  if (!d_x || !d_z) return fail(MCP_E_ARG, "NULL device pointer");
  MCP_ON_STREAM_DEVICE(stream);
  const float4* tables = nullptr;
  if (int rc = device_tables(dev_, (hipStream_t)stream, &tables)) return rc;
  HIP_TRY(mcp::launch_normals(d_x, n, tables, d_z, (hipStream_t)stream));
  return MCP_OK;
}

int mcp_icdf_table(float* out, size_t out_len) {
  if (!out || out_len < (size_t)mcp::ICDF_ENTRIES * 4) return fail(MCP_E_ARG, "buffer too small for %d x 4 floats", mcp::ICDF_ENTRIES);
  memcpy(out, k_icdf_table, sizeof k_icdf_table);
  return MCP_OK;
}

uint32_t mcp_float_to_key(float v) { return mcp::float_to_key(v); }
float mcp_key_to_float(uint32_t key) { return mcp::key_to_float(key); }

double mcp_terminal_to_x(const mcp_params* prm, float terminal) {
  if (prm->compounding == MCP_COMPOUND_LOG) return std::expm1((double)terminal);
  return (double)terminal / (double)(float)prm->v0 - 1.0;
}


static void free_shard(Shard& sh) {
  (void)hipSetDevice(sh.device);
  if (sh.stream) { (void)hipStreamSynchronize(sh.stream); (void)hipStreamDestroy(sh.stream); }
  if (sh.ev) (void)hipEventDestroy(sh.ev);
  for (int i = 0; i < MCP_WS_COUNT; i++)
    if (sh.ws[i] && i != MCP_WS_STATS) (void)hipFree(sh.ws[i]);
  release(sh.packed);
  release(sh.terminal);
  release(sh.gather);
  release(sh.h_packed);
  release(sh.h_pivot);
  release(sh.stats);
  release(sh.dd.mdd);
  release(sh.dd.stats);
  release(sh.hz.values);
  release(sh.hz.pivot);
  release(sh.hz.h_pivot);
  release(sh.hz.stats);
  release(sh.boot);
  release(sh.cf.flows);
  release(sh.overlay);
  release(sh.cf.counts);
  release(sh.cf.h_counts);
  release(sh.at.in);
  release(sh.at.h_in);
  release(sh.at.partials);
  release(sh.at.records);
  release(sh.at.h_records);
  release(sh.at.contrib);
  release(sh.pr.partials);
  release(sh.pr.cross);
  release(sh.pr.h_cross);
}

int mcp_ctx_create_multi(const int* devices, int ndev, mcp_ctx** out) {
  if (!out) return fail(MCP_E_ARG, "out is NULL");
  *out = nullptr;
  if (!devices || ndev < 1 || ndev > MAX_DEVICES) return fail(MCP_E_ARG, "ndev=%d outside [1,%d]", ndev, MAX_DEVICES);
  const int n = mcp_device_count();
  if (n <= 0) return fail(MCP_E_NODEVICE, "no HIP device visible (the product path has no CPU fallback)");
  bool all_same = true, all_distinct = true;
  for (int i = 0; i < ndev; i++) {
    if (devices[i] < 0 || devices[i] >= n) return fail(MCP_E_ARG, "device %d outside [0,%d)", devices[i], n);
    if (devices[i] != devices[0]) all_same = false;
    for (int j = 0; j < i; j++)
      if (devices[j] == devices[i]) all_distinct = false;
  }
  if (ndev > 1 && !all_same && !all_distinct)
    return fail(MCP_E_UNSUPPORTED, "devices must be all distinct (RCCL) or all the same (logical shards of one GPU)");
  if (ndev > 1 && all_same && ndev > 8) return fail(MCP_E_UNSUPPORTED, "at most 8 logical shards on one device");
  mcp_ctx* c = new (std::nothrow) mcp_ctx;
  if (!c) return fail(MCP_E_NOMEM, "out of host memory");
  struct Restore { int dev = 0; Restore() { (void)hipGetDevice(&dev); } ~Restore() { (void)hipSetDevice(dev); } } restore;
  c->all_same = ndev > 1 && all_same;
  c->sh.resize((size_t)ndev);
  for (int i = 0; i < ndev; i++) {
    Shard& sh = c->sh[(size_t)i];
    sh.device = devices[i];
    if (hipSetDevice(sh.device) != hipSuccess || hipStreamCreateWithFlags(&sh.stream, hipStreamNonBlocking) != hipSuccess ||
        hipEventCreateWithFlags(&sh.ev, hipEventDisableTiming) != hipSuccess) {
      mcp_ctx_destroy(c);
      return fail(MCP_E_HIP, "cannot create a stream on device %d", devices[i]);
    }
  }
  const char* force = getenv("MCP_FORCE_RCCL");
  c->exchange_always = ndev == 1 && force && *force == '1';
  *out = c;
  return MCP_OK;
}

static int ensure_exchange(mcp_ctx* c) {
  if (c->exchange_mode != MCP_EXCHANGE_UNSET) return MCP_OK;
  const int ndev = (int)c->sh.size();
  if (ndev == 1 && !c->exchange_always) { c->exchange_mode = MCP_EXCHANGE_NONE; return MCP_OK; }
  if (c->all_same) { c->same_device = true; c->exchange_mode = MCP_EXCHANGE_KERNEL; return MCP_OK; }
  std::vector<int> devices((size_t)ndev);
  for (int i = 0; i < ndev; i++) devices[(size_t)i] = c->sh[(size_t)i].device;
  const char* mode = getenv("MCP_EXCHANGE");
  int rc = (mode && !strcmp(mode, "p2p") && !c->exchange_always) ? fail(MCP_E_COMM, "MCP_EXCHANGE=p2p") : load_rccl(&c->rccl);
  if (rc == MCP_OK) {
    c->comms.assign((size_t)ndev, nullptr);
    const int r = c->rccl->CommInitAll(c->comms.data(), ndev, devices.data());
    if (r != 0) {
      c->comms.clear();
      rc = fail(MCP_E_COMM, "ncclCommInitAll over %d devices: %s", ndev, c->rccl->GetErrorString(r));
      c->rccl = nullptr;
    }
  }
  if (rc == MCP_OK) { c->exchange_mode = MCP_EXCHANGE_RCCL; return MCP_OK; }
  const std::string why = g_err;
  bool peers = ndev > 1 && ndev <= 8 && hipSetDevice(devices[0]) == hipSuccess;
  for (int i = 1; peers && i < ndev; i++) {
    int can = 0;
    peers = hipDeviceCanAccessPeer(&can, devices[0], devices[(size_t)i]) == hipSuccess && can;
    if (peers) {
      const hipError_t e = hipDeviceEnablePeerAccess(devices[(size_t)i], 0);
      peers = e == hipSuccess || e == hipErrorPeerAccessAlreadyEnabled;
      (void)hipGetLastError();
    }
  }
  if (!peers) return fail(MCP_E_COMM, "%s; and no peer access from device %d to the others for the kernel exchange", why.c_str(), devices[0]);
  c->rccl = nullptr;
  c->same_device = true;
  c->exchange_mode = MCP_EXCHANGE_P2P;
  c->exchange_note = why;
  return MCP_OK;
}

int mcp_ctx_exchange_mode(const mcp_ctx* c) { return c ? c->exchange_mode : MCP_EXCHANGE_UNSET; }
const char* mcp_ctx_exchange_note(const mcp_ctx* c) { return c ? c->exchange_note.c_str() : ""; }

int mcp_ctx_create(int device, mcp_ctx** out) { return mcp_ctx_create_multi(&device, 1, out); }

int mcp_ctx_device_count(const mcp_ctx* c) { return c ? (int)c->sh.size() : 0; }

int mcp_ctx_set_terminal_budget(mcp_ctx* c, size_t bytes) {
  if (!c || bytes < 4096) return fail(MCP_E_ARG, "bad argument");
  std::lock_guard<std::mutex> lock(c->mu);
  c->terminal_budget = bytes;
  return MCP_OK;
}

void mcp_ctx_destroy(mcp_ctx* c) {
  if (!c) return;
  int prev_dev = 0;
  const bool have_prev = hipGetDevice(&prev_dev) == hipSuccess;
  for (Shard& sh : c->sh)
    if (sh.stream) { (void)hipSetDevice(sh.device); (void)hipStreamSynchronize(sh.stream); }
  if (c->rccl)
    for (void* comm : c->comms)
      if (comm) (void)c->rccl->CommDestroy(comm);
  for (Shard& sh : c->sh) free_shard(sh);
  if (c->d_sweep && !c->sh.empty()) { (void)hipSetDevice(c->sh[0].device); (void)hipFree(c->d_sweep); }
  if (c->h_boot) (void)hipHostFree(c->h_boot);
  if (c->h_flows) (void)hipHostFree(c->h_flows);
  if (c->h_overlay) (void)hipHostFree(c->h_overlay);
  if (have_prev) (void)hipSetDevice(prev_dev);
  delete c;
}

namespace {

struct Job {
  int k0 = 0, kt = 0;
  uint64_t p0 = 0, pn = 0;
  bool active = false;
};

#define RCCL_TRY(c, expr)                                                                            \
  do {                                                                                               \
    int r_ = (expr);                                                                                 \
    if (r_ != 0) return fail(MCP_E_COMM, "%s: %s", #expr, (c)->rccl->GetErrorString(r_));            \
  } while (0)

int exchange_hist(mcp_ctx* c, int kt) {
  const size_t words = (size_t)kt * 2 * MCP_SELECT_BINS;
  const size_t S = c->sh.size();
  if (c->same_device) {
    Shard& s0 = c->sh[0];
    HIP_TRY(hipSetDevice(s0.device));
    unsigned long long* bufs[8];
    for (size_t s = 0; s < S; s++) {
      bufs[s] = (unsigned long long*)c->sh[s].ws[MCP_WS_HIST];
      if (s) { HIP_TRY(hipEventRecord(c->sh[s].ev, c->sh[s].stream)); HIP_TRY(hipStreamWaitEvent(s0.stream, c->sh[s].ev, 0)); }
    }
    HIP_TRY(mcp::launch_sum_u64(bufs, (int)S, words, s0.stream));
    HIP_TRY(hipEventRecord(s0.ev, s0.stream));
    for (size_t s = 1; s < S; s++) HIP_TRY(hipStreamWaitEvent(c->sh[s].stream, s0.ev, 0));
    return MCP_OK;
  }
  RCCL_TRY(c, c->rccl->GroupStart());
  for (size_t s = 0; s < S; s++) {
    void* h = c->sh[s].ws[MCP_WS_HIST];
    const int r = c->rccl->AllReduce(h, h, words, NCCL_UINT64, NCCL_SUM, c->comms[s], c->sh[s].stream);
    if (r != 0) { (void)c->rccl->GroupEnd(); return fail(MCP_E_COMM, "ncclAllReduce (shard %zu): %s", s, c->rccl->GetErrorString(r)); }
  }
  RCCL_TRY(c, c->rccl->GroupEnd());
  return MCP_OK;
}

int exchange_records(mcp_ctx* c, int kt) {
  const size_t S = c->sh.size();
  const size_t bytes = (size_t)kt * sizeof(mcp_record);
  if (c->same_device) {
    Shard& s0 = c->sh[0];
    HIP_TRY(hipSetDevice(s0.device));
    for (size_t s = 0; s < S; s++) {
      if (s) { HIP_TRY(hipEventRecord(c->sh[s].ev, c->sh[s].stream)); HIP_TRY(hipStreamWaitEvent(s0.stream, c->sh[s].ev, 0)); }
      HIP_TRY(hipMemcpyAsync((char*)s0.gather.p + s * bytes, c->sh[s].ws[MCP_WS_RECORD], bytes, hipMemcpyDeviceToDevice, s0.stream));
    }
    return MCP_OK;
  }
  RCCL_TRY(c, c->rccl->GroupStart());
  for (size_t s = 0; s < S; s++) {
    const int r = c->rccl->AllGather(c->sh[s].ws[MCP_WS_RECORD], c->sh[s].gather.p, (size_t)kt * (sizeof(mcp_record) / sizeof(double)),
                                     NCCL_FLOAT64, c->comms[s], c->sh[s].stream);
    if (r != 0) { (void)c->rccl->GroupEnd(); return fail(MCP_E_COMM, "ncclAllGather (shard %zu): %s", s, c->rccl->GetErrorString(r)); }
  }
  RCCL_TRY(c, c->rccl->GroupEnd());
  return MCP_OK;
}

enum SelectOf { SEL_TERMINAL, SEL_DRAWDOWN, SEL_HORIZON };

int run_select(mcp_ctx* c, const std::vector<mcp_params>& tp, const std::vector<Job>& jobs, bool exchange, uint64_t lo, uint64_t hi,
               double gamma, SelectOf what, int slot = 0) {
  const size_t S = c->sh.size();
  int rc;
  const int kt_x = tp[0].n_portfolios;
  const auto stats_of = [&](Shard& sh, int rows) -> void* {
    if (what == SEL_DRAWDOWN) return sh.dd.stats.dev;
    if (what == SEL_HORIZON) return (mcp_stats*)sh.hz.stats.dev + (size_t)slot * rows;
    return sh.ws[MCP_WS_STATS];
  };
  for (int pass = 0; pass < 3; pass++) {
    if (exchange && (rc = exchange_hist(c, kt_x))) return rc;
    for (size_t s = 0; s < S; s++) {
      const Job& j = jobs[s];
      if (!j.active) continue;
      Shard& sh = c->sh[s];
      HIP_TRY(hipSetDevice(sh.device));
      const uint64_t stride = j.pn ? j.pn : 1;
      const double* piv = what == SEL_DRAWDOWN ? nullptr : what == SEL_HORIZON ? sh.hz.pivot.p : (const double*)sh.ws[MCP_WS_PIVOT];
      const float* src = what == SEL_DRAWDOWN ? sh.dd.mdd.p : what == SEL_HORIZON ? sh.hz.values.p : sh.terminal.p;
      if (pass < 2) {
        if ((rc = mcp_launch_scan(&tp[s], pass, j.pn, lo, hi, sh.ws[MCP_WS_PARTIALS], sh.ws[MCP_WS_BELOW], piv, sh.ws[MCP_WS_HIST],
                                  sh.ws[MCP_WS_STATE], sh.ws[MCP_WS_RECORD], sh.stream))) return rc;
        if ((rc = mcp_launch_hist(&tp[s], pass + 1, src, stride, j.pn, sh.ws[MCP_WS_STATE], piv, sh.ws[MCP_WS_BELOW],
                                  sh.ws[MCP_WS_HIST], sh.stream))) return rc;
      } else {
        void* stats = exchange ? nullptr : stats_of(sh, tp[s].n_portfolios);
        if ((rc = mcp_launch_final(&tp[s], j.pn, gamma, lo, hi, sh.ws[MCP_WS_BELOW], sh.ws[MCP_WS_HIST], sh.ws[MCP_WS_STATE],
                                   sh.ws[MCP_WS_RECORD], sh.ws[MCP_WS_QUANT], stats, sh.stream)))
          return rc;
      }
    }
  }
  if (exchange) {
    if ((rc = exchange_records(c, kt_x))) return rc;
    Shard& s0 = c->sh[0];
    HIP_TRY(hipSetDevice(s0.device));
    if ((rc = mcp_launch_stats(&tp[0], (int)S, s0.gather.p, s0.ws[MCP_WS_QUANT], stats_of(s0, kt_x), s0.stream)))
      return rc;
  }
  return MCP_OK;
}

int tile_pivots(const mcp_params& tp, const Request& rq, int T, const float* W, const double* rmu, const double* bm, const double* bs2,
                double* out) {
  if (rq.rebalanced) {
    reb_pivots(tp.n_assets, tp.n_portfolios, T, rq.reb->period, rmu, W, out);
    return MCP_OK;
  }
  if (rq.src == SRC_BOOT) {
    for (int k = 0; k < tp.n_portfolios; k++) out[k] = boot_pivot(tp.compounding, T, bm[k], bs2[k]);
    return MCP_OK;
  }
  if (rq.src == SRC_FHS) {
    filt_pivots(tp.n_assets, tp.n_portfolios, T, rmu, W, out);
    return MCP_OK;
  }
  mcp_params p = tp;
  p.n_steps = T;
  return mcp_pivots(&p, rq.mu, rq.chol, W, out);
}

int run_tile(mcp_ctx* c, const mcp_params* prm, const Request& rq, uint64_t seed, uint64_t path_begin, uint64_t n_total,
             const std::vector<Job>& jobs, bool exchange) {
  const size_t S = c->sh.size();
  const int N = prm->n_assets;
  uint64_t lo, hi;
  double gamma;
  if (int rc = mcp_percentile_rank(n_total, prm->alpha, &lo, &hi, &gamma)) return rc;
  std::vector<mcp_params> tp(S, *prm);
  int rc;
  for (size_t s = 0; s < S; s++) {
    const Job& j = jobs[s];
    if (!j.active) continue;
    Shard& sh = c->sh[s];
    HIP_TRY(hipSetDevice(sh.device));
    tp[s].n_portfolios = j.kt;
    const size_t plen = mcp_packed_len(N, j.kt) + (rq.jumps ? (size_t)n4_of(N) : 0) + (rq.regimes ? regime_block_len(N) : 0), pn = j.pn ? j.pn : 1;
    const int rows = rq.hz ? rq.H * j.kt : j.kt;
    for (int w = 0; w < MCP_WS_COUNT; w++) {
      const size_t need = std::max(mcp_ws_bytes(w, j.kt, pn), mcp_ws_bytes(w, rows, pn));
      if (w != MCP_WS_STATS && (rc = grow_dev(&sh.ws[w], &sh.ws_cap[w], need, sh.stream, w == MCP_WS_HIST || w == MCP_WS_STATE)))
        return rc;
    }
    if ((rc = grow(sh.packed, plen)) || (rc = grow(sh.terminal, (size_t)j.kt * pn))) return rc;
    if (exchange && (rc = grow(sh.gather, S * (size_t)std::max(j.kt, rows)))) return rc;
    if ((rc = grow(sh.h_packed, plen)) || (rc = grow(sh.h_pivot, (size_t)j.kt)) || (rc = grow_mapped(sh.stats, (size_t)j.kt))) return rc;
    sh.ws[MCP_WS_STATS] = sh.stats.dev;
    if (rq.dd && ((rc = grow(sh.dd.mdd, (size_t)j.kt * pn)) || (rc = grow_mapped(sh.dd.stats, (size_t)j.kt)))) return rc;
    if (rq.hz && ((rc = grow(sh.hz.values, (size_t)rows * pn)) || (rc = grow(sh.hz.pivot, (size_t)rows)) ||
                  (rc = grow(sh.hz.h_pivot, (size_t)rows)) || (rc = grow_mapped(sh.hz.stats, (size_t)(1 + rq.L) * rows))))
      return rc;
    if (rq.cash && ((rc = grow(sh.cf.counts, 2 * (size_t)(j.kt + rows))) || (rc = grow(sh.cf.h_counts, 2 * (size_t)(j.kt + rows))))) return rc;
    if (rq.anti && ((rc = grow(sh.pr.partials, (size_t)j.kt * (size_t)mcp::path_grid(pn / 2))) || (rc = grow(sh.pr.cross, (size_t)j.kt)) ||
                    (rc = grow(sh.pr.h_cross, (size_t)j.kt))))
      return rc;
  }
  const float* shared_packed = nullptr;
  const double* shared_pivot = nullptr;
  const double* shared_hz_pivot = nullptr;
  const bool boot = rq.src == SRC_BOOT, fhs = rq.src == SRC_FHS;
  const std::vector<float> zmu(boot ? N : 0, 0.0f), zchol(boot || fhs ? (size_t)N * N : 0, 0.0f);
  std::vector<float> jmu(rq.jumps ? N : 0);
  if (rq.jumps) jump_drift(rq.jp, jump_consts(rq.jp), N, rq.mu, jmu.data());
  const size_t n_load = rq.jumps ? (size_t)n4_of(N) : rq.regimes ? regime_block_len(N) : 0;
  std::vector<float> blk1;
  if (rq.regimes) {
    blk1.resize(mcp_packed_len(N, 1));
    if ((rc = mcp_pack_params(N, 1, rq.rs->mu1, rq.rs->chol1, rq.W, blk1.data(), blk1.size()))) return rc;
  }
  const float* mu = boot ? zmu.data() : fhs ? rq.filt->mu : rq.jumps ? jmu.data() : rq.mu;
  const float* chol = boot || fhs ? zchol.data() : rq.chol;
  std::vector<double> bm, bs2, rmu(rq.rebalanced || fhs ? N : 0), cm;
  if (rq.rebalanced) reb_means(N, rq.mu, boot ? rq.boot : nullptr, rmu.data());
  if (fhs) filt_means(N, rq.filt, rmu.data());
  const bool ov_walk = rq.overlay && rq.ov->n_rows > 0;
  for (size_t s = 0; s < S; s++) {
    const Job& j = jobs[s];
    if (!j.active) continue;
    Shard& sh = c->sh[s];
    HIP_TRY(hipSetDevice(sh.device));
    const size_t plen = mcp_packed_len(N, j.kt);
    const float* src = sh.h_packed.p;
    const double* psrc = sh.h_pivot.p;
    const double* hpsrc = sh.hz.h_pivot.p;
    if (exchange && shared_packed) {
      src = shared_packed;
      psrc = shared_pivot;
      hpsrc = shared_hz_pivot;
    } else {
      const float* Wt = rq.W + (size_t)j.k0 * N;
      if ((rc = mcp_pack_params(N, j.kt, mu, chol, Wt, sh.h_packed.p, plen))) return rc;
      for (size_t i = 0; rq.jumps && i < n_load; i++) sh.h_packed.p[plen + i] = (int)i < N ? (rq.jp->loading ? rq.jp->loading[i] : 1.0f) : 0.0f;
      for (size_t i = 0; rq.regimes && i < n_load; i++) sh.h_packed.p[plen + i] = blk1[i];
      if (boot && !rq.rebalanced) {
        bm.resize((size_t)j.kt);
        bs2.resize((size_t)j.kt);
        boot_moments(N, rq.boot, Wt, j.kt, bm.data(), bs2.data());
      }
      if (rq.cash) {
        cm.resize((size_t)j.kt);
        cash_means(N, j.kt, rq.mu, boot ? rq.boot : nullptr, Wt, cm.data());
        cash_pivots(j.kt, prm->n_steps, cm.data(), rq.cf->flows, (double)(float)prm->v0, rq.hz ? rq.H : 0, rq.steps, sh.h_pivot.p,
                    sh.hz.h_pivot.p);
      } else if (ov_walk) {
        overlay_pivots(N, j.kt, prm->n_steps, rq.ov, rq.mu, Wt, rq.hz ? rq.H : 0, rq.steps, sh.h_pivot.p, sh.hz.h_pivot.p);
      } else if (rq.regimes) {
        regime_pivots(N, j.kt, prm->n_steps, rq.mu, rq.rs->mu1, regime_consts(rq.rs), Wt, rq.hz ? rq.H : 0, rq.steps, sh.h_pivot.p,
                      sh.hz.h_pivot.p);
      } else if ((rc = tile_pivots(tp[s], rq, prm->n_steps, Wt, rmu.data(), bm.data(), bs2.data(), sh.h_pivot.p))) return rc;
      for (int h = 0; rq.hz && !rq.cash && !ov_walk && !rq.regimes && h < rq.H; h++)
        if ((rc = tile_pivots(tp[s], rq, rq.steps[h], Wt, rmu.data(), bm.data(), bs2.data(), sh.hz.h_pivot.p + (size_t)h * j.kt)))
          return rc;
      if (exchange) { shared_packed = sh.h_packed.p; shared_pivot = sh.h_pivot.p; shared_hz_pivot = sh.hz.h_pivot.p; }
    }
    HIP_TRY(hipMemcpyAsync(sh.packed.p, src, (plen + n_load) * sizeof(float), hipMemcpyHostToDevice, sh.stream));
    HIP_TRY(hipMemcpyAsync(sh.ws[MCP_WS_PIVOT], psrc, (size_t)j.kt * sizeof(double), hipMemcpyHostToDevice, sh.stream));
    if (rq.hz) HIP_TRY(hipMemcpyAsync(sh.hz.pivot.p, hpsrc, (size_t)rq.H * j.kt * sizeof(double), hipMemcpyHostToDevice, sh.stream));
    if (j.pn) {
      Launch ln = make_launch(sh.packed.p, (const double*)sh.ws[MCP_WS_PIVOT], seed, path_begin + j.p0, j.pn, sh.terminal.p, j.pn,
                              sh.ws[MCP_WS_PARTIALS], sh.ws[MCP_WS_HIST], sh.stream);
      ln.d_mdd = sh.dd.mdd.p;
      ln.mdd_stride = j.pn;
      ln.d_hz = sh.hz.values.p;
      ln.hz_stride = j.pn;
      ln.d_rows = sh.boot.p;
      ln.d_flows = sh.cf.flows.p;
      ln.d_overlay = sh.overlay.p;
      ln.d_loading = sh.packed.p + plen;
      ln.d_block1 = sh.packed.p + plen;
      ln.d_cross = sh.pr.partials.p;
      if ((rc = launch_paths_impl(&tp[s], rq, ln))) return rc;
      if (rq.anti) {
        HIP_TRY(mcp::launch_attr_merge(sh.pr.partials.p, j.kt, mcp::path_grid(j.pn / 2), 1, sh.pr.cross.p, sh.stream));
        HIP_TRY(hipMemcpyAsync(sh.pr.h_cross.p, sh.pr.cross.p, (size_t)j.kt * sizeof(double), hipMemcpyDeviceToHost, sh.stream));
      }
      if (rq.cash) {
        const size_t rows_hz = rq.hz ? (size_t)rq.H * j.kt : 0;
        const bool tg = rq.cf->has_target != 0;
        const float g32 = tg ? (float)rq.cf->target : 0.0f;
        HIP_TRY(mcp::launch_zero(sh.cf.counts.p, 2 * ((size_t)j.kt + rows_hz) * sizeof(unsigned long long), sh.stream));
        HIP_TRY(mcp::launch_count_rows(sh.terminal.p, j.pn, j.pn, j.kt, tg, g32, sh.cf.counts.p, sh.stream));
        if (rows_hz)
          HIP_TRY(mcp::launch_count_rows(sh.hz.values.p, j.pn, j.pn, (int)rows_hz, tg, g32, sh.cf.counts.p + 2 * (size_t)j.kt, sh.stream));
      }
    } else {
      if ((rc = mcp_launch_pass0(&tp[s], sh.terminal.p, 1, 0, (const double*)sh.ws[MCP_WS_PIVOT], sh.ws[MCP_WS_PARTIALS],
                                 sh.ws[MCP_WS_HIST], sh.stream))) return rc;
    }
  }
  if ((rc = run_select(c, tp, jobs, exchange, lo, hi, gamma, SEL_TERMINAL))) return rc;
  if (rq.dd) {
    std::vector<mcp_params> tpd(tp);
    for (size_t s = 0; s < S; s++) {
      tpd[s].v0 = 1.0;
      tpd[s].rf = 0.0;
      const Job& j = jobs[s];
      if (!j.active) continue;
      Shard& sh = c->sh[s];
      HIP_TRY(hipSetDevice(sh.device));
      if ((rc = mcp_launch_pass0(&tpd[s], sh.dd.mdd.p, j.pn ? j.pn : 1, j.pn, nullptr, sh.ws[MCP_WS_PARTIALS], sh.ws[MCP_WS_HIST],
                                 sh.stream)))
        return rc;
    }
    if ((rc = run_select(c, tpd, jobs, exchange, lo, hi, gamma, SEL_DRAWDOWN))) return rc;
  }
  if (rq.hz) {
    std::vector<mcp_params> tph(tp);
    for (size_t s = 0; s < S; s++)
      if (jobs[s].active) tph[s].n_portfolios = rq.H * jobs[s].kt;
    for (int l = -1; l < rq.L; l++) {
      uint64_t qlo = lo, qhi = hi;
      double qg = gamma;
      if (l >= 0 && (rc = mcp_percentile_rank_q(n_total, rq.levels[l], &qlo, &qhi, &qg))) return rc;
      for (size_t s = 0; s < S; s++) {
        const Job& j = jobs[s];
        if (!j.active) continue;
        Shard& sh = c->sh[s];
        HIP_TRY(hipSetDevice(sh.device));
        if ((rc = mcp_launch_pass0(&tph[s], sh.hz.values.p, j.pn ? j.pn : 1, j.pn, sh.hz.pivot.p, sh.ws[MCP_WS_PARTIALS],
                                   sh.ws[MCP_WS_HIST], sh.stream))) return rc;
      }
      if ((rc = run_select(c, tph, jobs, exchange, qlo, qhi, qg, SEL_HORIZON, l + 1))) return rc;
    }
  }
  for (size_t s = 0; s < S; s++) {
    const Job& j = jobs[s];
    if (!j.active || !j.pn) continue;
    Shard& sh = c->sh[s];
    HIP_TRY(hipSetDevice(sh.device));
    const auto copy_out = [&](float* out, const float* d) {
      return hipMemcpy2DAsync(out + (size_t)j.k0 * n_total + j.p0, n_total * sizeof(float), d, j.pn * sizeof(float),
                              j.pn * sizeof(float), (size_t)j.kt, hipMemcpyDeviceToHost, sh.stream);
    };
    if (rq.terminal_out) HIP_TRY(copy_out(rq.terminal_out, sh.terminal.p));
    if (rq.dd && rq.mdd_out) HIP_TRY(copy_out(rq.mdd_out, sh.dd.mdd.p));
    if (rq.hz && rq.hz_out)
      for (int h = 0; h < rq.H; h++)
        HIP_TRY(copy_out(rq.hz_out + (size_t)h * prm->n_portfolios * n_total, sh.hz.values.p + (size_t)h * j.kt * j.pn));
    if (rq.cash)
      HIP_TRY(hipMemcpyAsync(sh.cf.h_counts.p, sh.cf.counts.p, 2 * (size_t)((rq.hz ? 1 + rq.H : 1) * j.kt) * sizeof(unsigned long long),
                             hipMemcpyDeviceToHost, sh.stream));
  }
  for (size_t s = 0; s < S; s++)
    if (jobs[s].active) { HIP_TRY(hipSetDevice(c->sh[s].device)); HIP_TRY(hipStreamSynchronize(c->sh[s].stream)); }
  for (size_t s = 0; rq.cash && s < S; s++) {
    const Job& j = jobs[s];
    if (!j.active || !j.pn) continue;
    const unsigned long long* hc = c->sh[s].cf.h_counts.p;
    for (int k = 0; k < j.kt; k++)
      for (int i = 0; i < 2; i++) {
        rq.counts_out[2 * (size_t)(j.k0 + k) + i] += hc[2 * (size_t)k + i];
        for (int h = 0; rq.hz && h < rq.H; h++)
          rq.hz_counts_out[2 * ((size_t)h * prm->n_portfolios + j.k0 + k) + i] += hc[2 * ((size_t)j.kt + (size_t)h * j.kt + k) + i];
      }
  }
  for (size_t s = 0; rq.anti && s < S; s++) {
    const Job& j = jobs[s];
    if (!j.active || !j.pn) continue;
    for (int k = 0; k < j.kt; k++) rq.cross_out[j.k0 + k] += c->sh[s].pr.h_cross.p[k];
  }
  for (size_t s = 0; s < S; s++) {
    const Job& j = jobs[s];
    if (!j.active || (exchange && s != 0)) continue;
    const Shard& sh = c->sh[s];
    memcpy(rq.stats_out + j.k0, sh.stats.p, (size_t)j.kt * sizeof(mcp_stats));
    if (rq.dd) {
      memcpy(rq.dd_stats_out + j.k0, sh.dd.stats.p, (size_t)j.kt * sizeof(mcp_stats));
      for (int k = 0; k < j.kt; k++) rq.dd_stats_out[j.k0 + k].sharpe = 0.0;
    }
    if (rq.hz) {
      const int rows = rq.H * j.kt;
      for (int h = 0; h < rq.H; h++)
        for (int k = 0; k < j.kt; k++) {
          const size_t o = (size_t)h * prm->n_portfolios + j.k0 + k, r = (size_t)h * j.kt + k;
          rq.hz_stats_out[o] = sh.hz.stats.p[r];
          rq.hz_stats_out[o].sharpe = 0.0;
          for (int l = 0; l < rq.L; l++) rq.bands_out[o * rq.L + l] = sh.hz.stats.p[(size_t)(1 + l) * rows + r].var;
        }
    }
  }
  return MCP_OK;
}

int tile_portfolios(size_t budget, uint64_t n_paths, int K, size_t bytes_per_path = sizeof(float)) {
  const uint64_t fit = budget / (bytes_per_path * (n_paths ? n_paths : 1));
  if (fit >= (uint64_t)K) return K;
  if (fit >= (uint64_t)K_PAD) return (int)(fit / K_PAD) * K_PAD;
  return fit >= 1 ? (int)fit : 1;
}

int run_attribution(mcp_ctx* c, const mcp_params* prm, const Request& rq, uint64_t seed, uint64_t path_begin, uint64_t n_paths,
                    const std::vector<Job>& jobs) {
  const size_t S = c->sh.size();
  const int N = prm->n_assets, K = prm->n_portfolios, n4 = n4_of(N), RL = mcp::attr_record_len(n4);
  const size_t plen = mcp_packed_len(N, K);
  int rc;
  for (size_t s = 0; s < S; s++) {
    const Job& j = jobs[s];
    if (!j.pn) continue;
    Shard& sh = c->sh[s];
    HIP_TRY(hipSetDevice(sh.device));
    const size_t grid = (size_t)mcp::path_grid(j.pn);
    if ((rc = grow(sh.packed, plen)) || (rc = grow(sh.h_packed, plen)) || (rc = grow(sh.at.in, 2 * (size_t)K)) ||
        (rc = grow(sh.at.h_in, 2 * (size_t)K)) || (rc = grow(sh.at.partials, (size_t)K * grid * RL)) ||
        (rc = grow(sh.at.records, (size_t)K * RL)) || (rc = grow(sh.at.h_records, (size_t)K * RL)))
      return rc;
    if (rq.contrib_out && (rc = grow(sh.at.contrib, (size_t)K * N * j.pn))) return rc;
    if ((rc = mcp_pack_params(N, K, rq.mu, rq.chol, rq.W, sh.h_packed.p, plen))) return rc;
    for (int k = 0; k < K; k++) sh.at.h_in.p[k] = rq.stats_out[k].var;
    if ((rc = mcp_pivots(prm, rq.mu, rq.chol, rq.W, sh.at.h_in.p + K))) return rc;
    HIP_TRY(hipMemcpyAsync(sh.packed.p, sh.h_packed.p, plen * sizeof(float), hipMemcpyHostToDevice, sh.stream));
    HIP_TRY(hipMemcpyAsync(sh.at.in.p, sh.at.h_in.p, 2 * (size_t)K * sizeof(double), hipMemcpyHostToDevice, sh.stream));
    Launch ln = make_launch(sh.packed.p, sh.at.in.p + K, seed, path_begin + j.p0, j.pn, nullptr, j.pn, nullptr, nullptr, sh.stream);
    ln.attr = true;
    ln.d_var = sh.at.in.p;
    ln.d_attr_partials = sh.at.partials.p;
    ln.d_contrib = rq.contrib_out ? sh.at.contrib.p : nullptr;
    ln.contrib_stride = j.pn;
    if ((rc = launch_paths_impl(prm, rq, ln))) return rc;
    HIP_TRY(mcp::launch_attr_merge(sh.at.partials.p, K, (int)grid, RL, sh.at.records.p, sh.stream));
    HIP_TRY(hipMemcpyAsync(sh.at.h_records.p, sh.at.records.p, (size_t)K * RL * sizeof(double), hipMemcpyDeviceToHost, sh.stream));
    if (rq.contrib_out)
// ... 485 lines not shown
```

### monte_carlo_portfolio_amd/csrc/mcp_stats_kernels.h

```cpp
#pragma once
#include <hip/hip_runtime.h>
#include <stdint.h>

#include "../../include/mcport.h"
#include "mcp_route.h"

namespace mcp {

struct SelectState {
  uint32_t prefix;
  uint32_t pad;
  uint64_t rank;
};

struct Quantile {
  double x_lo, x_hi, var;
  double level2;
  uint64_t n_tail;
  uint64_t pad;
};

struct MomentPartial {
  double s1, s2;
  float vmin, vmax;
  unsigned long long n;
};
static_assert(sizeof(MomentPartial) == 32, "MomentPartial is 32 bytes");

constexpr int PATH_GRID_CAP = 8192;
constexpr int SWEEP_MIN_K = 17;
constexpr int SWEEP_TILE_PATHS = 64;

__host__ __device__ inline int path_grid(uint64_t n) {
  uint64_t tiles = (n + 255) / 256;
  if (tiles < 1) tiles = 1;
  return (int)(tiles < (uint64_t)PATH_GRID_CAP ? tiles : (uint64_t)PATH_GRID_CAP);
}
__host__ __device__ inline uint64_t moment_slots(bool sweep, uint64_t n) {
  return sweep ? (n + SWEEP_TILE_PATHS - 1) / SWEEP_TILE_PATHS + (n == 0) : (uint64_t)path_grid(n);
}

__host__ __device__ inline int stream_slots(int K) {
  const int s = 16384 / (K < 1 ? 1 : K);
  return s > 2048 ? 2048 : (s < 1 ? 1 : s);
}

struct PathArgs;
struct PathLaunchArgs;

constexpr int LEAN_MAX_NB = 4;
enum PathFamily { FAM_PLAIN, FAM_DD, FAM_HZ, FAM_REB, FAM_CF, FAM_OV, FAM_AT };
struct PathKernel {
  int family;
  bool logc, boot, blds, stt, dd, gv, kt8, native, fold, anti, fh, uhi, jp, rs;
};

typedef hipError_t (*launch_paths_fn)(const PathKernel& k, const PathLaunchArgs& args, hipStream_t stream);
#define MCP_DECL_NB(n) hipError_t launch_paths_nb##n(const PathKernel& k, const PathLaunchArgs& args, hipStream_t stream);
MCP_DECL_NB(1) MCP_DECL_NB(2) MCP_DECL_NB(3) MCP_DECL_NB(4) MCP_DECL_NB(5) MCP_DECL_NB(6) MCP_DECL_NB(7) MCP_DECL_NB(8)
MCP_DECL_NB(9) MCP_DECL_NB(10) MCP_DECL_NB(11) MCP_DECL_NB(12) MCP_DECL_NB(13) MCP_DECL_NB(14) MCP_DECL_NB(15) MCP_DECL_NB(16)
#undef MCP_DECL_NB

hipError_t launch_sweep_shared(int nb, int mt, bool native, const PathArgs& args, hipStream_t stream);
hipError_t launch_sweep_shared_p0(int nb, int mt, bool native, const PathArgs& args, hipStream_t stream);
hipError_t launch_sweep_shared_p1(int nb, int mt, bool native, const PathArgs& args, hipStream_t stream);
hipError_t launch_sweep_shared_p2(int nb, int mt, bool native, const PathArgs& args, hipStream_t stream);
hipError_t launch_sweep_shared_p3(int nb, int mt, bool native, const PathArgs& args, hipStream_t stream);
hipError_t launch_sweep_paths(int nb, int mt, bool native, const PathArgs& args, hipStream_t stream);
hipError_t launch_normals(const uint32_t* x, uint64_t n, const float4* table, float* z, hipStream_t s);

hipError_t launch_pass0(const mcp_params& prm, int K, const float* terminal, uint64_t stride, uint64_t n, const double* pivot,
                        uint64_t slots, MomentPartial* partials, unsigned long long* hist, hipStream_t s);
hipError_t launch_scan(const mcp_params& prm, int K, int pass, uint64_t n, uint64_t rank_lo, uint64_t rank_hi, uint64_t slots,
                       const MomentPartial* partials, const double* below, const double* pivot, unsigned long long* hist,
                       SelectState* state, mcp_record* record, hipStream_t s);
hipError_t launch_hist(const mcp_params& prm, int K, int pass, const float* terminal, uint64_t stride, uint64_t n,
                       const SelectState* state, const double* pivot, double* below, unsigned long long* hist, hipStream_t s);
hipError_t launch_final(const mcp_params& prm, int K, uint64_t n, double gamma, uint64_t rank_lo, uint64_t rank_hi,
                        const double* below, unsigned long long* hist, const SelectState* state, mcp_record* record,
                        Quantile* quant, mcp_stats* stats_or_null, hipStream_t s);
hipError_t launch_stats(const mcp_params& prm, int K, int world, const mcp_record* gathered, const Quantile* quant,
                        mcp_stats* out, hipStream_t s);
hipError_t launch_zero(void* p, size_t bytes, hipStream_t s);
hipError_t launch_count_rows(const float* values, uint64_t stride, uint64_t n, int rows, bool has_target, float target,
                             unsigned long long* counts, hipStream_t s);
hipError_t launch_sum_u64(unsigned long long* const* bufs, int nsrc, size_t words, hipStream_t s);
hipError_t launch_attr_merge(const double* partials, int K, int blocks, int len, double* out, hipStream_t s);

hipError_t launch_sweep_hist(int N, int R, int P, const double* returns, const double* mean, const double* cov,
                             const double* W, double rf, uint64_t rank_lo, uint64_t rank_hi, double gamma,
                             double* out5, hipStream_t s);

}
```

### monte_carlo_portfolio_amd/csrc/mcp_stats_kernels.hip

```cpp
#include <cstdlib>

#include "mcp_paths.h"
#include "mcp_stats_kernels.h"

#ifdef MCP_DIAG_CLOCK
namespace mcp { __device__ unsigned long long mcp_diag_stamps[2 * 8192]; }
extern "C" int mcp_diag_read(unsigned long long* out, int n_blocks) {
  return (int)hipMemcpyFromSymbol(out, HIP_SYMBOL(mcp::mcp_diag_stamps), (size_t)n_blocks * 2 * sizeof(unsigned long long));
}
#endif

namespace mcp {

constexpr int SB = 256;
constexpr int PER = MCP_SELECT_BINS / SB;

__device__ __forceinline__ void pass_shape(int pass, int& shift, int& bits, int& pshift) {
  shift = pass == 0 ? 21 : (pass == 1 ? 10 : 0);
  bits = pass == 2 ? 10 : 11;
  pshift = pass == 0 ? 32 : (pass == 1 ? 21 : 10);
}

static int stream_grid(uint64_t n, int K) {
  static const uint64_t per = [] { const char* e = getenv("MCP_STREAM_ELEMS"); const long v = e ? atol(e) : 0; return (uint64_t)(v > 0 ? v : 8192); }();
  uint64_t g = (n + per - 1) / per;
  if (g < 1) g = 1;
  const uint64_t cap = (uint64_t)stream_slots(K);
  return (int)(g > cap ? cap : g);
}

template <bool LOGC>
__device__ __forceinline__ double below_term(float v, double v0d) {
  if constexpr (LOGC) return expm1((double)v);
  else return (double)v - v0d;
}

__global__ void __launch_bounds__(SB) pass0_kernel(const mcp_params prm, const float* __restrict__ terminal, uint64_t stride,
                                                   uint64_t n, int G, uint64_t slots, const double* __restrict__ pivot,
                                                   MomentPartial* __restrict__ partials, unsigned long long* __restrict__ hist) {
  __shared__ uint32_t h[MCP_SELECT_BINS];
  __shared__ double red[4][2];
  __shared__ float ext[4][2];
  __shared__ unsigned long long cnt[4];
  const int k = blockIdx.x / G, b = blockIdx.x % G;
  for (int i = threadIdx.x; i < MCP_SELECT_BINS; i += SB) h[i] = 0u;
  __syncthreads();
  const double v0d = (double)(float)prm.v0;
  const double c = pivot ? pivot[k] : 0.0;
  const float* __restrict__ src = terminal + (size_t)k * stride;
  double s1 = 0.0, s2 = 0.0;
  float mn = __builtin_inff(), mx = -__builtin_inff();
  unsigned long long m = 0;
  const uint64_t step = (uint64_t)G * SB;
  for (uint64_t i0 = (uint64_t)b * SB; i0 < n; i0 += step) {
    const uint64_t i = i0 + threadIdx.x;
    const bool live = i < n;
    const float v = live ? src[i] : 0.0f;
    if (live) {
      const double d = terminal_to_x(v, v0d, prm.compounding) - c;
      m += 1; s1 += d; s2 = __builtin_fma(d, d, s2); mn = fminf(mn, v); mx = fmaxf(mx, v);
    }
    lds_hist_add(h, float_to_key(v) >> 21, live);
  }
  s1 = wave_sum(s1); s2 = wave_sum(s2); mn = wave_minf(mn); mx = wave_maxf(mx);
  m = (unsigned long long)wave_sum((double)m);
  const int lane = threadIdx.x & 63, wv = threadIdx.x >> 6;
  if (lane == 0) { red[wv][0] = s1; red[wv][1] = s2; ext[wv][0] = mn; ext[wv][1] = mx; cnt[wv] = m; }
  __syncthreads();
  MomentPartial* row = partials + (size_t)k * slots;
  if (threadIdx.x == 0) {
    MomentPartial o;
    o.s1 = (red[0][0] + red[1][0]) + (red[2][0] + red[3][0]);
    o.s2 = (red[0][1] + red[1][1]) + (red[2][1] + red[3][1]);
    o.vmin = fminf(fminf(ext[0][0], ext[1][0]), fminf(ext[2][0], ext[3][0]));
    o.vmax = fmaxf(fmaxf(ext[0][1], ext[1][1]), fmaxf(ext[2][1], ext[3][1]));
    o.n = (cnt[0] + cnt[1]) + (cnt[2] + cnt[3]);
    row[b] = o;
  }
  for (uint64_t j = (uint64_t)G + b * (uint64_t)SB + threadIdx.x; j < slots; j += step) {
    MomentPartial e;
    e.s1 = 0.0; e.s2 = 0.0; e.vmin = __builtin_inff(); e.vmax = -__builtin_inff(); e.n = 0ull;
    row[j] = e;
  }
  unsigned long long* out = hist + (size_t)k * 2 * MCP_SELECT_BINS;
  for (int i = threadIdx.x; i < MCP_SELECT_BINS; i += SB) {
    const uint32_t v = h[i];
    if (v) atomicAdd(&out[i], (unsigned long long)v);
  }
}

constexpr int WIN = 16;
template <int PASS, bool LOGC>
__global__ void __launch_bounds__(SB) hist_kernel(const mcp_params prm, const float* __restrict__ terminal, uint64_t stride, uint64_t n,
                                                  int G, int slots, const SelectState* __restrict__ state, const double* __restrict__ pivot,
                                                  double* __restrict__ below_out, unsigned long long* __restrict__ hist) {
  constexpr int NH = PASS == 0 ? 1 : 2;
  __shared__ uint32_t h[NH][MCP_SELECT_BINS];
  __shared__ uint32_t win[PASS == 0 ? WIN : 1][64];
  __shared__ double red[4];
  const int k = blockIdx.x / G, b = blockIdx.x % G;
  for (int i = threadIdx.x; i < NH * MCP_SELECT_BINS; i += SB) (&h[0][0])[i] = 0u;
  if constexpr (PASS == 0)
    for (int i = threadIdx.x; i < WIN * 64; i += SB) (&win[0][0])[i] = 0u;
  __syncthreads();
  int shift, bits, pshift;
  pass_shape(PASS, shift, bits, pshift);
  const uint32_t mask = (1u << bits) - 1u;
  const double v0d = (double)(float)prm.v0;
  uint32_t pa = 0, pb = 0, dlo = 0;
  if constexpr (PASS == 0) {
    const double c = pivot ? pivot[k] : 0.0;
    const float vc = LOGC ? (float)log1p(c > -1.0 ? c : 0.0) : (float)(v0d * (1.0 + c));
    const uint32_t dc = float_to_key(vc) >> 21;
    dlo = dc >= WIN / 2 ? dc - WIN / 2 : 0u;
    if (dlo > (uint32_t)(MCP_SELECT_BINS - WIN)) dlo = MCP_SELECT_BINS - WIN;
  } else {
    pa = state[2 * k + 0].prefix; pb = state[2 * k + 1].prefix;
  }
  const bool two = pa != pb;
  const int lane = threadIdx.x & 63;
  const float* __restrict__ src = terminal + (size_t)k * stride;
  double below = 0.0;

  auto one = [&](float v) {
    const uint32_t key = float_to_key(v);
    if constexpr (PASS == 0) {
      const uint32_t d = key >> 21, t = d - dlo;
      if (t < (uint32_t)WIN) atomicAdd(&win[t][lane], 1u);
      else atomicAdd(&h[0][d], 1u);
    } else {
      const uint32_t pre = key >> pshift, d = (key >> shift) & mask;
      if (pre == pa) atomicAdd(&h[0][d], 1u);
      if (two && pre == pb) atomicAdd(&h[1][d], 1u);
      if (pre < pa && (PASS == 1 || (pre >> 11) == (pa >> 11))) below += below_term<LOGC>(v, v0d);
    }
  };

  const uint64_t head = n ? (uint64_t)((4 - (((uintptr_t)src >> 2) & 3)) & 3) : 0;
  const uint64_t hd = head < n ? head : n;
  const uint64_t nvec = (n - hd) / 4;
  const float4* __restrict__ vsrc = (const float4*)(src + hd);
  const uint64_t vstep = (uint64_t)G * SB;
  uint64_t j = (uint64_t)b * SB + threadIdx.x;
  for (; j + vstep < nvec; j += 2 * vstep) {
    const float4 q0 = vsrc[j], q1 = vsrc[j + vstep];
    one(q0.x); one(q0.y); one(q0.z); one(q0.w);
    one(q1.x); one(q1.y); one(q1.z); one(q1.w);
  }
  for (; j < nvec; j += vstep) {
    const float4 q0 = vsrc[j];
    one(q0.x); one(q0.y); one(q0.z); one(q0.w);
  }
  if (b == 0) {
    if (threadIdx.x < hd) one(src[threadIdx.x]);
    const uint64_t t0 = hd + 4 * nvec;
    if (t0 + threadIdx.x < n) one(src[t0 + threadIdx.x]);
  }

  if constexpr (PASS != 0) {
    below = wave_sum(below);
    const int wv = threadIdx.x >> 6;
    if (lane == 0) red[wv] = below;
  }
  __syncthreads();
  if constexpr (PASS != 0) {
    if (threadIdx.x == 0) below_out[(size_t)k * slots + b] = (red[0] + red[1]) + (red[2] + red[3]);
  } else {
    if (threadIdx.x < WIN) {
      uint32_t t = 0;
      for (int l = 0; l < 64; l++) t += win[threadIdx.x][(l + threadIdx.x) & 63];
      if (t) atomicAdd(&h[0][dlo + threadIdx.x], t);
    }
    __syncthreads();
  }
  unsigned long long* out = hist + (size_t)k * 2 * MCP_SELECT_BINS;
  const int nh = (PASS == 0 || !two) ? 1 : 2;
  for (int i = threadIdx.x; i < nh * MCP_SELECT_BINS; i += SB) {
    const uint32_t cnt = (&h[0][0])[i];
    if (cnt) atomicAdd(&out[i], (unsigned long long)cnt);
  }
}

__device__ __forceinline__ unsigned long long block_exclusive_scan(unsigned long long v, unsigned long long* wtot ) {
  const int lane = threadIdx.x & 63, wv = threadIdx.x >> 6;
  unsigned long long inc = v;
#pragma unroll
  for (int o = 1; o < 64; o <<= 1) {
    const unsigned long long t = __shfl_up(inc, o, 64);
    if (lane >= o) inc += t;
  }
  __syncthreads();
  if (lane == 63) wtot[wv] = inc;
  __syncthreads();
  unsigned long long base = 0;
  for (int w = 0; w < wv; w++) base += wtot[w];
  return base + inc - v;
}

__device__ __forceinline__ double block_sum(double v, double* scratch ) {
  v = wave_sum(v);
  __syncthreads();
  if ((threadIdx.x & 63) == 0) scratch[threadIdx.x >> 6] = v;
  __syncthreads();
  return (scratch[0] + scratch[1]) + (scratch[2] + scratch[3]);
}

__device__ __forceinline__ void descend(int pass, const unsigned long long (&c)[PER], unsigned long long tot,
                                        unsigned long long before, SelectState& st, SelectState* dst) {
  int shift, bits, pshift;
  pass_shape(pass, shift, bits, pshift);
  if (st.rank >= before && st.rank < before + tot) {
#pragma unroll
    for (int i = 0; i < PER; i++) {
      if (st.rank < before + c[i]) {
        st.prefix = (pass == 0 ? 0u : (st.prefix << bits)) | (uint32_t)(threadIdx.x * PER + i);
        st.rank -= before;
        *dst = st;
        break;
      }
      before += c[i];
    }
  }
}

__global__ void __launch_bounds__(SB) scan_kernel(const mcp_params prm, int pass, uint64_t rank_lo, uint64_t rank_hi, int G, int bslots,
                                                  uint64_t mslots, const MomentPartial* __restrict__ partials,
                                                  const double* __restrict__ below, const double* __restrict__ pivot,
                                                  unsigned long long* __restrict__ hist, SelectState* __restrict__ state,
                                                  mcp_record* __restrict__ record) {
  __shared__ unsigned long long wtot[4];
  __shared__ double red[4][2];
  __shared__ float ext[4][2];
  __shared__ unsigned long long cnt[4];
  const int k = blockIdx.x;
  if (pass == 0) {
    const MomentPartial* pp = partials + (size_t)k * mslots;
    double s1 = 0.0, s2 = 0.0;
    float mn = __builtin_inff(), mx = -__builtin_inff();
    unsigned long long m = 0;
    for (uint64_t b = threadIdx.x; b < mslots; b += SB) {
      const MomentPartial p = pp[b];
      m += p.n; s1 += p.s1; s2 += p.s2; mn = fminf(mn, p.vmin); mx = fmaxf(mx, p.vmax);
    }
    s1 = wave_sum(s1); s2 = wave_sum(s2); mn = wave_minf(mn); mx = wave_maxf(mx);
    m = (unsigned long long)wave_sum((double)m);
    const int lane = threadIdx.x & 63, wv = threadIdx.x >> 6;
    if (lane == 0) { red[wv][0] = s1; red[wv][1] = s2; ext[wv][0] = mn; ext[wv][1] = mx; cnt[wv] = m; }
    __syncthreads();
    if (threadIdx.x == 0) {
      const double v0d = (double)(float)prm.v0;
      mcp_record r;
      r.n = (double)((cnt[0] + cnt[1]) + (cnt[2] + cnt[3]));
      r.sum = (red[0][0] + red[1][0]) + (red[2][0] + red[3][0]);
      r.sumsq = (red[0][1] + red[1][1]) + (red[2][1] + red[3][1]);
      const float vmn = fminf(fminf(ext[0][0], ext[1][0]), fminf(ext[2][0], ext[3][0]));
      const float vmx = fmaxf(fmaxf(ext[0][1], ext[1][1]), fmaxf(ext[2][1], ext[3][1]));
      r.min = r.n > 0 ? terminal_to_x(vmn, v0d, prm.compounding) : __builtin_inf();
      r.max = r.n > 0 ? terminal_to_x(vmx, v0d, prm.compounding) : -__builtin_inf();
      r.below = 0.0;
      r.pivot = pivot ? pivot[k] : 0.0;
      r.pad = 0.0;
      record[k] = r;
    }
  } else {
    const double* pp = below + (size_t)k * bslots;
    double bl = 0.0;
    for (int b = threadIdx.x; b < G; b += SB) bl += pp[b];
    bl = block_sum(bl, &red[0][0]);
    if (threadIdx.x == 0) record[k].below = bl;
  }
  const SelectState in0 = pass == 0 ? SelectState{0u, 0u, rank_lo} : state[2 * k + 0];
  const SelectState in1 = pass == 0 ? SelectState{0u, 0u, rank_hi} : state[2 * k + 1];
  const bool shared_hist = pass == 0 || in0.prefix == in1.prefix;
#pragma unroll 1
  for (int w = 0; w < 2; w++) {
    unsigned long long* hh = hist + ((size_t)k * 2 + (shared_hist ? 0 : w)) * MCP_SELECT_BINS;
    unsigned long long c[PER], tot = 0;
#pragma unroll
    for (int i = 0; i < PER; i++) { c[i] = hh[threadIdx.x * PER + i]; tot += c[i]; }
    SelectState st = w ? in1 : in0;
    const unsigned long long before = block_exclusive_scan(tot, wtot);
    descend(pass, c, tot, before, st, &state[2 * k + w]);
    if (!shared_hist || w == 1) {
#pragma unroll
      for (int i = 0; i < PER; i++) hh[threadIdx.x * PER + i] = 0ull;
    }
  }
}

__device__ __forceinline__ double key_to_x(uint32_t key, double v0d, int compounding) {
  return terminal_to_x(key_to_float(key), v0d, compounding);
}

__device__ __forceinline__ void finish_stats(const mcp_params& prm, const mcp_record& m, const Quantile& q, mcp_stats* out) {
  const double v0d = (double)(float)prm.v0;
  mcp_stats s;
  s.n = (uint64_t)m.n;
  const double dm = m.n > 0 ? m.sum / m.n : 0.0;
  s.mean = m.pivot + dm;
  double m2 = m.sumsq - m.sum * dm;
  if (m2 < 0.0) m2 = 0.0;
  s.m2 = m2;
  s.std = m.n > 1 ? sqrt(m2 / (m.n - 1.0)) : 0.0;
  s.sharpe = s.std > 0.0 ? (s.mean - prm.rf) / s.std : 0.0;
  s.var = q.var; s.x_lo = q.x_lo; s.x_hi = q.x_hi;
  s.n_tail = q.n_tail;
  const double below_x = prm.compounding == MCP_COMPOUND_LOG ? m.below : m.below / v0d;
  s.sum_tail = below_x + q.level2;
  s.cvar = s.n_tail > 0 ? s.sum_tail / (double)s.n_tail : s.var;
  s.min = m.min; s.max = m.max;
  *out = s;
}

__global__ void __launch_bounds__(SB) final_kernel(const mcp_params prm, double gamma, uint64_t rank_lo, uint64_t rank_hi, int G, int bslots,
                                                   const double* __restrict__ below, unsigned long long* __restrict__ hist,
                                                   const SelectState* __restrict__ state, mcp_record* __restrict__ record,
                                                   Quantile* __restrict__ quant, mcp_stats* __restrict__ stats) {
  __shared__ unsigned long long wtot[4];
  __shared__ double red[4];
  __shared__ uint32_t s_key[2];
  __shared__ double s_q[3];
  const int k = blockIdx.x;
  const double v0d = (double)(float)prm.v0;
  const double* pp = below + (size_t)k * bslots;
  double bl = 0.0;
  for (int b = threadIdx.x; b < G; b += SB) bl += pp[b];
  bl = block_sum(bl, red);

  unsigned long long c[2][PER];
  const SelectState st0 = state[2 * k + 0], st1 = state[2 * k + 1];
  const bool shared_hist = st0.prefix == st1.prefix;
#pragma unroll
  for (int w = 0; w < 2; w++) {
    unsigned long long* hh = hist + ((size_t)k * 2 + (shared_hist ? 0 : w)) * MCP_SELECT_BINS;
    unsigned long long tot = 0;
#pragma unroll
    for (int i = 0; i < PER; i++) { c[w][i] = hh[threadIdx.x * PER + i]; tot += c[w][i]; }
    if (!shared_hist || w == 1) {
#pragma unroll
      for (int i = 0; i < PER; i++) hh[threadIdx.x * PER + i] = 0ull;
    }
    const unsigned long long before = block_exclusive_scan(tot, wtot);
    const SelectState st = w ? st1 : st0;
    if (st.rank >= before && st.rank < before + tot) {
      unsigned long long bf = before;
#pragma unroll
      for (int i = 0; i < PER; i++) {
        if (st.rank < bf + c[w][i]) { s_key[w] = (st.prefix << 10) | (uint32_t)(threadIdx.x * PER + i); break; }
        bf += c[w][i];
      }
    }
  }
  __syncthreads();
  if (threadIdx.x == 0) {
    const double a = key_to_x(s_key[0], v0d, prm.compounding), b = key_to_x(s_key[1], v0d, prm.compounding);
    const double diff = b - a;
    double r = a + diff * gamma;
    if (gamma >= 0.5) r = b - diff * (1.0 - gamma);
    s_q[0] = a; s_q[1] = b; s_q[2] = r;
  }
  __syncthreads();
  const double var = s_q[2];
  double cnt = 0.0, sum = 0.0;
#pragma unroll
  for (int w = 0; w < 2; w++) {
    if (w == 1 && shared_hist) break;
    const uint32_t pre = (w ? st1.prefix : st0.prefix) << 10;
#pragma unroll
    for (int i = 0; i < PER; i++) {
      const uint32_t d = (uint32_t)(threadIdx.x * PER + i);
      if (c[w][i] && d < 1024u) {
        const double x = key_to_x(pre | d, v0d, prm.compounding);
        if (x <= var) { cnt += (double)c[w][i]; sum += (double)c[w][i] * x; }
      }
    }
  }
  cnt = block_sum(cnt, red);
  sum = block_sum(sum, red);
  if (threadIdx.x == 0) {
    const unsigned long long n_tail = (rank_lo - st0.rank) + (unsigned long long)cnt;
    Quantile q = {s_q[0], s_q[1], var, sum, n_tail, 0ull};
    quant[k] = q;
    mcp_record m = record[k];
    m.below += bl;
    record[k] = m;
    if (stats) finish_stats(prm, m, q, &stats[k]);
  }
  (void)rank_hi;
}

__global__ void stats_kernel(const mcp_params prm, int K, int world, const mcp_record* __restrict__ gathered,
                             const Quantile* __restrict__ quant, mcp_stats* __restrict__ out) {
  const int k = blockIdx.x * blockDim.x + threadIdx.x;
  if (k >= K) return;
  mcp_record m = gathered[k];
  for (int r = 1; r < world; r++) {
    const mcp_record g = gathered[(size_t)r * K + k];
    m.n += g.n; m.sum += g.sum; m.sumsq += g.sumsq; m.min = fmin(m.min, g.min); m.max = fmax(m.max, g.max);
    m.below += g.below;
  }
  finish_stats(prm, m, quant[k], &out[k]);
}

struct PtrList { unsigned long long* p[8]; int n; };
__global__ void __launch_bounds__(SB) sum_u64_kernel(PtrList l, size_t words) {
  for (size_t i = (size_t)blockIdx.x * SB + threadIdx.x; i < words; i += (size_t)gridDim.x * SB) {
    unsigned long long t = 0;
    for (int j = 0; j < l.n; j++) t += l.p[j][i];
    for (int j = 0; j < l.n; j++) l.p[j][i] = t;
  }
}

__global__ void __launch_bounds__(256) normals_kernel(const uint32_t* __restrict__ x, uint64_t n,
                                                      const float4* __restrict__ table, float* __restrict__ z) {
  __shared__ float4 s_tab[ICDF_LDS_ENTRIES];
  for (int i = threadIdx.x; i < ICDF_ENTRIES; i += 256) s_tab[ICDF_PAD + i] = table[i];
  __syncthreads();
  const IcdfConsts kc = icdf_consts();
  for (uint64_t i = (uint64_t)blockIdx.x * 256 + threadIdx.x; i < n; i += (uint64_t)gridDim.x * 256) z[i] = normal_icdf(x[i], s_tab, kc);
}

hipError_t launch_normals(const uint32_t* x, uint64_t n, const float4* table, float* z, hipStream_t s) {
  uint64_t g = (n + 255) / 256;
  if (g < 1) g = 1;
  if (g > 4096) g = 4096;
  normals_kernel<<<(unsigned)g, 256, 0, s>>>(x, n, table, z);
  return hipGetLastError();
}

static bool grid_ok(int K, int G) { return (uint64_t)K * (uint64_t)G <= 0x7fffffffull; }

hipError_t launch_pass0(const mcp_params& prm, int K, const float* terminal, uint64_t stride, uint64_t n, const double* pivot,
                        uint64_t slots, MomentPartial* partials, unsigned long long* hist, hipStream_t s) {
  int G = stream_grid(n, K);
  if ((uint64_t)G > slots) G = (int)slots;
  if (G < 1 || !grid_ok(K, G)) return hipErrorInvalidValue;
  pass0_kernel<<<(unsigned)(K * G), SB, 0, s>>>(prm, terminal, stride, n, G, slots, pivot, partials, hist);
  return hipGetLastError();
}

hipError_t launch_scan(const mcp_params& prm, int K, int pass, uint64_t n, uint64_t rank_lo, uint64_t rank_hi, uint64_t slots,
                       const MomentPartial* partials, const double* below, const double* pivot, unsigned long long* hist,
                       SelectState* state, mcp_record* record, hipStream_t s) {
  scan_kernel<<<(unsigned)K, SB, 0, s>>>(prm, pass, rank_lo, rank_hi, stream_grid(n, K), stream_slots(K), slots, partials, below, pivot,
                                         hist, state, record);
  return hipGetLastError();
}

hipError_t launch_hist(const mcp_params& prm, int K, int pass, const float* terminal, uint64_t stride, uint64_t n,
                       const SelectState* state, const double* pivot, double* below, unsigned long long* hist, hipStream_t s) {
  const int G = stream_grid(n, K);
  if (!grid_ok(K, G)) return hipErrorInvalidValue;
  const unsigned grid = (unsigned)(K * G);
  const int bs = stream_slots(K);
  const bool lg = prm.compounding == MCP_COMPOUND_LOG;
#define MCP_HIST(P)                                                                                              \
  do {                                                                                                           \
    if (lg) hist_kernel<P, true><<<grid, SB, 0, s>>>(prm, terminal, stride, n, G, bs, state, pivot, below, hist); \
    else hist_kernel<P, false><<<grid, SB, 0, s>>>(prm, terminal, stride, n, G, bs, state, pivot, below, hist);   \
  } while (0)
  if (pass == 0) MCP_HIST(0);
  else if (pass == 1) MCP_HIST(1);
  else if (pass == 2) MCP_HIST(2);
  else return hipErrorInvalidValue;
#undef MCP_HIST
  return hipGetLastError();
}

hipError_t launch_final(const mcp_params& prm, int K, uint64_t n, double gamma, uint64_t rank_lo, uint64_t rank_hi,
                        const double* below, unsigned long long* hist, const SelectState* state, mcp_record* record,
                        Quantile* quant, mcp_stats* stats_or_null, hipStream_t s) {
  final_kernel<<<(unsigned)K, SB, 0, s>>>(prm, gamma, rank_lo, rank_hi, stream_grid(n, K), stream_slots(K), below, hist, state,
                                          record, quant, stats_or_null);
  return hipGetLastError();
}

hipError_t launch_stats(const mcp_params& prm, int K, int world, const mcp_record* gathered, const Quantile* quant,
                        mcp_stats* out, hipStream_t s) {
  stats_kernel<<<(K + 63) / 64, 64, 0, s>>>(prm, K, world, gathered, quant, out);
  return hipGetLastError();
}

__global__ void __launch_bounds__(SB) zero_u64_kernel(unsigned long long* __restrict__ p, size_t words) {
  for (size_t i = (size_t)blockIdx.x * SB + threadIdx.x; i < words; i += (size_t)gridDim.x * SB) p[i] = 0ull;
}

hipError_t launch_zero(void* p, size_t bytes, hipStream_t s) {
  const size_t words = bytes / 8;
  size_t g = (words + SB - 1) / SB;
  if (g < 1) g = 1;
  if (g > 4096) g = 4096;
  zero_u64_kernel<<<(unsigned)g, SB, 0, s>>>((unsigned long long*)p, words);
  return hipGetLastError();
}

__global__ void __launch_bounds__(SB) count_rows_kernel(const float* __restrict__ values, uint64_t stride, uint64_t n, int has_target,
                                                        float target, unsigned long long* __restrict__ counts) {
  __shared__ unsigned long long s_n[2];
  if (threadIdx.x < 2) s_n[threadIdx.x] = 0ull;
  __syncthreads();
  const float* __restrict__ row = values + (size_t)blockIdx.y * stride;
  unsigned long long nr = 0, ns = 0;
  for (uint64_t base = (uint64_t)blockIdx.x * SB; base < n; base += (uint64_t)gridDim.x * SB) {
    const uint64_t i = base + threadIdx.x;
    const bool live = i < n;
    const float v = live ? row[i] : 1.0f;
    nr += (unsigned long long)__popcll(__ballot(live && v == 0.0f));
    ns += (unsigned long long)__popcll(__ballot(live && has_target && v < target));
  }
  if ((threadIdx.x & 63) == 0) {
    if (nr) atomicAdd(&s_n[0], nr);
    if (ns) atomicAdd(&s_n[1], ns);
  }
  __syncthreads();
  if (threadIdx.x < 2 && s_n[threadIdx.x]) atomicAdd(&counts[2 * (size_t)blockIdx.y + threadIdx.x], s_n[threadIdx.x]);
}

hipError_t launch_count_rows(const float* values, uint64_t stride, uint64_t n, int rows, bool has_target, float target,
                             unsigned long long* counts, hipStream_t s) {
  if (rows < 1) return hipErrorInvalidValue;
  uint64_t g = (n + SB - 1) / SB;
  if (g < 1) g = 1;
  if (g > 256) g = 256;
  for (int r0 = 0; r0 < rows; r0 += 65535) {
    const int nr = rows - r0 < 65535 ? rows - r0 : 65535;
    count_rows_kernel<<<dim3((unsigned)g, (unsigned)nr), SB, 0, s>>>(values + (size_t)r0 * stride, stride, n, has_target ? 1 : 0, target,
                                                                    counts + 2 * (size_t)r0);
  }
  return hipGetLastError();
}

hipError_t launch_sum_u64(unsigned long long* const* bufs, int nsrc, size_t words, hipStream_t s) {
  if (nsrc < 1 || nsrc > 8) return hipErrorInvalidValue;
  PtrList l;
  for (int j = 0; j < 8; j++) l.p[j] = j < nsrc ? bufs[j] : nullptr;
  l.n = nsrc;
  size_t g = (words + SB - 1) / SB;
  if (g < 1) g = 1;
  if (g > 2048) g = 2048;
  sum_u64_kernel<<<(unsigned)g, SB, 0, s>>>(l, words);
  return hipGetLastError();
}

__global__ void __launch_bounds__(SB) attr_merge_kernel(const double* __restrict__ partials, int blocks, int len, double* __restrict__ out) {
  const int j = threadIdx.x;
  if (j >= len) return;
  const double* src = partials + (size_t)blockIdx.x * blocks * len;
  double acc = 0.0;
  for (int b = 0; b < blocks; b++) acc += src[(size_t)b * len + j];
  out[(size_t)blockIdx.x * len + j] = acc;
}

hipError_t launch_attr_merge(const double* partials, int K, int blocks, int len, double* out, hipStream_t s) {
  if (K < 1 || blocks < 1 || len < 1 || len > SB) return hipErrorInvalidValue;
  attr_merge_kernel<<<(unsigned)K, SB, 0, s>>>(partials, blocks, len, out);
  return hipGetLastError();
}

}
```

### monte_carlo_portfolio_amd/engine.py

```python
from __future__ import annotations

import ctypes
import os

import numpy as np

from . import _ffi


class HipKernels:

    device_type = "cuda"

    def __init__(self, torch, device):
        self.torch, self.device = torch, device
        self.lib = _ffi.lib()
        if self.lib.mcp_device_count() < 1:
            raise _ffi.McpError("no HIP device visible (the product path has no CPU fallback)")

    def _stream(self):
        return ctypes.c_void_p(self.torch.cuda.current_stream(self.device).cuda_stream)

    @staticmethod
    def _p(t):
        return ctypes.c_void_p(t.data_ptr()) if t is not None else None

    def paths(self, prm, packed, pivot, seed, path_begin, n, terminal, partials, hist):
        _ffi.check(self.lib.mcp_launch_paths(ctypes.byref(prm), self._p(packed), self._p(pivot), seed, path_begin, n,
                                             self._p(terminal), terminal.shape[1], self._p(partials), self._p(hist),
                                             self._stream()))

    def pass0(self, prm, terminal, n, pivot, partials, hist):
        _ffi.check(self.lib.mcp_launch_pass0(ctypes.byref(prm), self._p(terminal), terminal.shape[1], n, self._p(pivot),
                                             self._p(partials), self._p(hist), self._stream()))

    def scan(self, prm, p, n, lo, hi, partials, below, pivot, hist, state, record):
        _ffi.check(self.lib.mcp_launch_scan(ctypes.byref(prm), p, n, lo, hi, self._p(partials), self._p(below), self._p(pivot),
                                            self._p(hist), self._p(state), self._p(record), self._stream()))

    def hist(self, prm, p, terminal, n, state, pivot, below, hist):
        _ffi.check(self.lib.mcp_launch_hist(ctypes.byref(prm), p, self._p(terminal), terminal.shape[1], n, self._p(state),
                                            self._p(pivot), self._p(below), self._p(hist), self._stream()))

    def final(self, prm, n, gamma, lo, hi, below, hist, state, record, quant, stats):
        _ffi.check(self.lib.mcp_launch_final(ctypes.byref(prm), n, gamma, lo, hi, self._p(below), self._p(hist),
                                             self._p(state), self._p(record), self._p(quant), self._p(stats), self._stream()))

    def stats(self, prm, world, gathered, quant, stats):
        _ffi.check(self.lib.mcp_launch_stats(ctypes.byref(prm), world, self._p(gathered), self._p(quant), self._p(stats),
                                             self._stream()))

    def sum_u64(self, bufs, words):
        arr = (ctypes.c_void_p * len(bufs))(*[t.data_ptr() for t in bufs])
        _ffi.check(self.lib.mcp_launch_sum_u64(arr, len(bufs), words, self._stream()))


class PathEngine:

    N_STAGES = 4

    def __init__(self, mu32, chol32, W32, n_steps, n_paths_local, *, compounding="simple", v0=1.0, alpha=0.95,
                 rf=0.0, native_math=False, device=None, group=None, world_size=1, rank=0, kernels=None,
                 pipeline=True, shard="paths", n_buffers=None, fold=False, logical_shards=1, skew=None, fused=True, cu_reserve=0,
                 n_stats_streams=None):
        import torch

        self.torch = torch
        if kernels is None:
            device = torch.device("cuda", torch.cuda.current_device()) if device is None else torch.device(device)
            kernels = HipKernels(torch, device)
        self.k = kernels
        self.device = torch.device(device if device is not None else kernels.device_type)
        if shard not in ("paths", "portfolios"):
            raise ValueError("shard must be 'paths' or 'portfolios'")
        self.shard = shard
        self.gather_group, self.gather_world, self.gather_rank = group, int(world_size), int(rank)
        if shard == "portfolios":
            k_all = W32.shape[0]
            kc = -(-k_all // int(world_size))
            self.k_slice = (min(int(rank) * kc, k_all), min((int(rank) + 1) * kc, k_all))
            self.k_chunk, self.k_all = kc, k_all
            W_local = np.zeros((kc, W32.shape[1]), np.float32)
            W_local[:self.k_slice[1] - self.k_slice[0]] = W32[self.k_slice[0]:self.k_slice[1]]
            W32, group, world_size, rank = W_local, None, 1, 0
        self.group, self.world, self.rank = group, int(world_size), int(rank)
        self.S = int(logical_shards)
        if self.S < 1 or self.S > 8:
            raise ValueError("logical_shards must be in 1..8")
        if self.S > 1 and self.group is not None:
            raise ValueError("logical shards and a process group are alternatives")
        self.n_local = int(n_paths_local)
        self.n_total = self.n_local * self.world
        self.shard_n = [self.n_local // self.S + (1 if j < self.n_local % self.S else 0) for j in range(self.S)]
        self.shard_off = [sum(self.shard_n[:j]) for j in range(self.S)]
        K = W32.shape[0]
        self.K = K
        self.fused = bool(fused)
        self.prm = _ffi.make_params(mu32.shape[0], n_steps, K, compounding, v0, alpha, rf, native_math, fold)
        self.rank_lo, self.rank_hi, self.gamma = _ffi.percentile_rank(self.n_total, alpha)
        self.pipeline = bool(pipeline) and self.device.type == "cuda"
        self.exchanging = self.group is not None or self.S > 1
        self.skew = (self.group is not None and self.pipeline) if skew is None else bool(skew)
        if n_stats_streams is None:
            n_stats_streams = 1 if self.group is not None else 2
        self.depth = self.N_STAGES if self.skew else 0
        if n_buffers:
            self.n_buf = int(n_buffers) if (self.pipeline or self.skew) else 1
        else:
            self.n_buf = self.depth + 2 if self.skew else (2 if self.pipeline else 1)
        if self.skew and self.n_buf < self.depth + 1:
            raise ValueError(f"the skewed schedule keeps {self.depth + 1} batches in flight: n_buffers >= {self.depth + 1}")

        lib = _ffi.lib()
        packed = _ffi.pack_params(mu32, chol32, W32)
        self.d_packed = torch.from_numpy(packed).to(self.device)
        self.d_pivot = torch.from_numpy(_ffi.pivots(self.prm, mu32, chol32, W32)).to(self.device)
        self.bufs = []
        for _ in range(self.n_buf):
            row = []
            for j in range(self.S):
                nj = max(self.shard_n[j], 1)
                b = {"terminal": torch.empty((K, nj), dtype=torch.float32, device=self.device), "ws": {}, "n": self.shard_n[j],
                     "off": self.shard_off[j]}
                for which in range(_ffi.WS_COUNT):
                    nbytes = lib.mcp_ws_bytes(which, K, nj)
                    b["ws"][which] = torch.zeros((nbytes + 7) // 8, dtype=torch.int64, device=self.device)
                b["ws"][_ffi.WS_PIVOT] = self.d_pivot.view(torch.int64)
                b["record"] = b["ws"][_ffi.WS_RECORD].view(torch.float64).view(K, _ffi.RECORD_DOUBLES)
                b["hist"] = b["ws"][_ffi.WS_HIST]
                if self.group is not None:
                    b["gather"] = torch.empty((self.world * K, _ffi.RECORD_DOUBLES), dtype=torch.float64, device=self.device)
                elif self.S > 1 and j == 0:
                    b["gather"] = torch.empty((self.S * K, _ffi.RECORD_DOUBLES), dtype=torch.float64, device=self.device)
                row.append(b)
            self.bufs.append(row)
        self.t = 0
        self.stage_done = {}
        self.last = 0
        if self.pipeline:
            n_ps = max(1, min(int(os.environ.get("MCP_ENGINE_PATH_STREAMS", "2")), self.n_buf * self.S))
            self.cu_reserve = int(cu_reserve)
            self._raw_streams = []
            if self.cu_reserve > 0:
                self.s_paths = []
                for _ in range(n_ps):
                    h = ctypes.c_void_p()
                    _ffi.check(_ffi.lib().mcp_stream_create(self.device.index or 0, self.cu_reserve, ctypes.byref(h)))
                    self._raw_streams.append(h)
                    self.s_paths.append(torch.cuda.ExternalStream(h.value, device=self.device))
            else:
                self.s_paths = [torch.cuda.Stream(self.device) for _ in range(n_ps)]
            ns = max(1, min(int(n_stats_streams), self.n_buf))
            pool = [[torch.cuda.Stream(self.device, priority=-1) for _ in range(self.S)] for _ in range(ns)]
            self._stat_pool = pool
            self.s_stats = [pool[i % ns] for i in range(self.n_buf)]
            self.ev_paths = [[torch.cuda.Event() for _ in range(self.S)] for _ in range(self.n_buf)]
            self.ev_stats = [[torch.cuda.Event() for _ in range(self.S)] for _ in range(self.n_buf)]
            self.ev_x = [[torch.cuda.Event() for _ in range(self.S)] for _ in range(self.n_buf)]
            cur = torch.cuda.current_stream(self.device)
            for row in self.ev_stats:
                for e in row:
                    e.record(cur)
            for sp in self.s_paths:
                sp.wait_stream(cur)
            for row in pool:
                for ss in row:
                    ss.wait_stream(cur)

    @property
    def d_terminal(self):
        return self.bufs[self.last][0]["terminal"]

    @property
    def ws(self):
        return self.bufs[self.last][0]["ws"]

    def _on_stats(self, i, j):
        if not self.pipeline:
            import contextlib
            return contextlib.nullcontext()
        return self.torch.cuda.stream(self.s_stats[i][j])

    def _enqueue_paths(self, b, seed, path_base, with_stats=True):
        n, ws = b["n"], b["ws"]
        if n < 1:
            return
        stats = with_stats and self.fused
        self.k.paths(self.prm, self.d_packed, self.d_pivot, seed, path_base + self.rank * self.n_local + b["off"], n, b["terminal"],
                     ws[_ffi.WS_PARTIALS] if stats else None, ws[_ffi.WS_HIST] if stats else None)

    def _exchange_hist(self, i):
        row = self.bufs[i]
        if self.group is not None:
            with self._on_stats(i, 0):
                self.torch.distributed.all_reduce(row[0]["hist"], group=self.group)
        elif self.S > 1:
            words = row[0]["hist"].numel()
            if self.pipeline:
                s0 = self.s_stats[i][0]
                for j in range(1, self.S):
                    self.ev_x[i][j].record(self.s_stats[i][j])
                    s0.wait_event(self.ev_x[i][j])
            with self._on_stats(i, 0):
                self.k.sum_u64([b["hist"] for b in row], words)
            if self.pipeline:
                self.ev_x[i][0].record(self.s_stats[i][0])
                for j in range(1, self.S):
                    self.s_stats[i][j].wait_event(self.ev_x[i][0])

    def _stage(self, i, s):
        k, prm, lo, hi = self.k, self.prm, self.rank_lo, self.rank_hi
        row = self.bufs[i]
        if s <= 3:
            if self.exchanging:
                self._exchange_hist(i)
            for j, b in enumerate(row):
                ws, n = b["ws"], b["n"]
                with self._on_stats(i, j):
                    if s <= 2:
                        k.scan(prm, s - 1, n, lo, hi, ws[_ffi.WS_PARTIALS], ws[_ffi.WS_BELOW], self.d_pivot, ws[_ffi.WS_HIST],
                               ws[_ffi.WS_STATE], ws[_ffi.WS_RECORD])
                        k.hist(prm, s, b["terminal"], n, ws[_ffi.WS_STATE], self.d_pivot, ws[_ffi.WS_BELOW], ws[_ffi.WS_HIST])
                    else:
                        k.final(prm, n, self.gamma, lo, hi, ws[_ffi.WS_BELOW], ws[_ffi.WS_HIST], ws[_ffi.WS_STATE], ws[_ffi.WS_RECORD],
                                ws[_ffi.WS_QUANT], None if self.exchanging else ws[_ffi.WS_STATS])
        else:
            b0 = row[0]
            if self.group is not None:
                with self._on_stats(i, 0):
                    self.torch.distributed.all_gather_into_tensor(b0["gather"], b0["record"], group=self.group)
                    k.stats(prm, self.world, b0["gather"], b0["ws"][_ffi.WS_QUANT], b0["ws"][_ffi.WS_STATS])
            elif self.S > 1:
                if self.pipeline:
                    for j in range(1, self.S):
                        self.ev_x[i][j].record(self.s_stats[i][j])
                        self.s_stats[i][0].wait_event(self.ev_x[i][j])
                with self._on_stats(i, 0):
                    for j, b in enumerate(row):
                        b0["gather"][j * self.K:(j + 1) * self.K].copy_(b["record"], non_blocking=True)
                    k.stats(prm, self.S, b0["gather"], b0["ws"][_ffi.WS_QUANT], b0["ws"][_ffi.WS_STATS])
            if self.pipeline:
                self.ev_stats[i][0].record(self.s_stats[i][0])
                for j in range(1, self.S):
                    self.ev_stats[i][j].record(self.s_stats[i][j])

    def _first_stage_empty_shards(self, i):
        for j, b in enumerate(self.bufs[i]):
            if b["n"] < 1:
                with self._on_stats(i, j):
                    self.k.pass0(self.prm, b["terminal"], 0, self.d_pivot, b["ws"][_ffi.WS_PARTIALS], b["ws"][_ffi.WS_HIST])

    def _begin_batch(self, i, seed, path_base):
        row = self.bufs[i]
        if not self.pipeline:
            for b in row:
                self._enqueue_paths(b, seed, path_base)
                if not self.fused and b["n"] > 0:
                    self.k.pass0(self.prm, b["terminal"], b["n"], self.d_pivot, b["ws"][_ffi.WS_PARTIALS], b["ws"][_ffi.WS_HIST])
            self._first_stage_empty_shards(i)
            return
        torch = self.torch
        for j, b in enumerate(row):
            sp = self.s_paths[(i * self.S + j) % len(self.s_paths)]
            with torch.cuda.stream(sp):
                sp.wait_event(self.ev_stats[i][0])
                if j:
                    sp.wait_event(self.ev_stats[i][j])
                self._enqueue_paths(b, seed, path_base)
                self.ev_paths[i][j].record(sp)
            self.s_stats[i][j].wait_event(self.ev_paths[i][j])
            if not self.fused and b["n"] > 0:
                with self._on_stats(i, j):
                    self.k.pass0(self.prm, b["terminal"], b["n"], self.d_pivot, b["ws"][_ffi.WS_PARTIALS], b["ws"][_ffi.WS_HIST])
        self._first_stage_empty_shards(i)

    def step(self, seed: int, path_base: int = 0):
        t = self.t
        i = t % self.n_buf
        self._begin_batch(i, seed, path_base)
        self.stage_done[t] = 0
        self.t = t + 1
        if self.skew:
            for s in range(1, self.N_STAGES + 1):
                bt = t - s
                if bt in self.stage_done and self.stage_done[bt] == s - 1:
                    self._advance(bt)
        else:
            while t in self.stage_done:
                self._advance(t)

    def _advance(self, bt):
        s = self.stage_done[bt] + 1
        last_stage = self.N_STAGES if self.exchanging else self.N_STAGES - 1
        i = bt % self.n_buf
        if s <= last_stage:
            self._stage(i, s)
        if s >= last_stage:
            if not self.exchanging and self.pipeline:
                for j in range(self.S):
                    self.ev_stats[i][j].record(self.s_stats[i][j])
            del self.stage_done[bt]
            self.last = i
        else:
            self.stage_done[bt] = s

    def flush(self):
        while self.stage_done:
            self._advance(min(self.stage_done))

    def launch_paths_only(self, seed: int, path_base: int = 0, with_stats: bool = True, clear_hist: bool = True):
        b = self.bufs[self.last][0]
        self._enqueue_paths(b, seed, path_base, with_stats)
        if with_stats and self.fused and clear_hist:
            b["hist"].zero_()

    def close(self):
        if getattr(self, "_raw_streams", None):
            self.synchronize()
            for h in self._raw_streams:
                _ffi.lib().mcp_stream_destroy(h)
            self._raw_streams = []

    def synchronize(self):
        self.flush()
        if self.pipeline:
            for sp in self.s_paths:
                sp.synchronize()
            for row in self._stat_pool:
                for ss in row:
                    ss.synchronize()
        elif self.device.type == "cuda":
            self.torch.cuda.synchronize(self.device)

    def stats(self) -> np.ndarray:
        self.synchronize()
        nbytes = self.K * _ffi.STATS_DTYPE.itemsize
        raw = self.ws[_ffi.WS_STATS].cpu().numpy().view(np.uint8)[:nbytes]
        return raw.view(_ffi.STATS_DTYPE).copy()

    def terminal(self) -> np.ndarray:
        self.synchronize()
        return np.concatenate([b["terminal"][:, :b["n"]].cpu().numpy() for b in self.bufs[self.last]], axis=1)

    def gathered_stats(self) -> np.ndarray:
        if self.shard != "portfolios":
            return self.stats()
        torch = self.torch
        self.synchronize()
        words = self.k_chunk * _ffi.STATS_DTYPE.itemsize // 8
        mine = self.ws[_ffi.WS_STATS][:words].contiguous()
        if self.gather_world > 1:
            out = torch.empty(self.gather_world * words, dtype=torch.int64, device=self.device)
            torch.distributed.all_gather_into_tensor(out, mine, group=self.gather_group)
        else:
            out = mine
        rec = out.cpu().numpy().view(np.uint8).view(_ffi.STATS_DTYPE)
        return rec[:self.k_all].copy()
```

Measured before the change: 452.9 million paths/s.

## Fuse scan/final into histogram kernel via last-block ticket for single-shard runs

Adds a fused hist_tail kernel in which the last block to finish each portfolio's histogram, found through an atomic ticket stored in the SelectState pad word, runs the scan or final selection step itself. Reads of other blocks' results go through agent-scope atomic loads. This removes the separate scan and final kernel launches and cuts the pipeline from four stages to two when there is one shard and K<=16. In exchange it adds fences, a serial tail inside one block and reliance on the pad field being reset correctly.

```diff
diff --git a/include/mcport.h b/include/mcport.h
--- a/include/mcport.h
+++ b/include/mcport.h
@@ -389,6 +389,9 @@
                     const void *d_below, const double *d_pivot, void *d_hist, void *d_state, void *d_record, void *stream);
 int mcp_launch_hist(const mcp_params *prm, int pass, const float *d_terminal, uint64_t terminal_stride, uint64_t n,
                     const void *d_state, const double *d_pivot, void *d_below, void *d_hist, void *stream);
+int mcp_launch_hist_tail(const mcp_params *prm, int pass, const float *d_terminal, uint64_t terminal_stride, uint64_t n,
+                         double gamma, uint64_t rank_lo, uint64_t rank_hi, void *d_state, const double *d_pivot, void *d_below,
+                         void *d_hist, void *d_record, void *d_quant, void *d_stats, void *stream);
 int mcp_launch_final(const mcp_params *prm, uint64_t n, double gamma, uint64_t rank_lo, uint64_t rank_hi,
                      const void *d_below, void *d_hist, const void *d_state, void *d_record, void *d_quant,
                      void *d_stats, void *stream);
diff --git a/monte_carlo_portfolio_amd/_ffi.py b/monte_carlo_portfolio_amd/_ffi.py
--- a/monte_carlo_portfolio_amd/_ffi.py
+++ b/monte_carlo_portfolio_amd/_ffi.py
@@ -192,6 +192,7 @@
     "mcp_launch_scan": (_int, [_PP, _int, _u64, _u64, _u64, _vp, _vp, _vp, _vp, _vp, _vp, _vp]),
     "mcp_launch_hist": (_int, [_PP, _int, _vp, _u64, _u64, _vp, _vp, _vp, _vp, _vp]),
     "mcp_launch_final": (_int, [_PP, _u64, ctypes.c_double, _u64, _u64, _vp, _vp, _vp, _vp, _vp, _vp, _vp]),
+    "mcp_launch_hist_tail": (_int, [_PP, _int, _vp, _u64, _u64, ctypes.c_double, _u64, _u64, _vp, _vp, _vp, _vp, _vp, _vp, _vp, _vp]),
     "mcp_launch_stats": (_int, [_PP, _int, _vp, _vp, _vp, _vp]),
     "mcp_launch_sum_u64": (_int, [ctypes.POINTER(_vp), _int, ctypes.c_size_t, _vp]),
     "mcp_stream_create": (_int, [_int, _int, ctypes.POINTER(_vp)]),
diff --git a/monte_carlo_portfolio_amd/csrc/mcp_api.cpp b/monte_carlo_portfolio_amd/csrc/mcp_api.cpp
--- a/monte_carlo_portfolio_amd/csrc/mcp_api.cpp
+++ b/monte_carlo_portfolio_amd/csrc/mcp_api.cpp
@@ -19,6 +19,9 @@
 
 #ifndef MCP_EXP_LEAN
 #define MCP_EXP_LEAN 1
+#endif
+#ifndef MCP_EXP_FUSED_TAIL
+#define MCP_EXP_FUSED_TAIL 1
 #endif
 
 namespace {
@@ -1356,6 +1359,32 @@
   return MCP_OK;
 }
 
+int mcp_launch_hist_tail(const mcp_params* prm, int pass, const float* d_terminal, uint64_t stride, uint64_t n, double gamma,
+                         uint64_t rank_lo, uint64_t rank_hi, void* d_state, const double* d_pivot, void* d_below, void* d_hist,
+                         void* d_record, void* d_quant, void* d_stats, void* stream) {
+  if (int rc = check_params(prm)) return rc;
+  if (!d_terminal || !d_hist || !d_state || !d_below || !d_record || pass < 1 || pass > 2 || stride < n || (pass == 2 && !d_quant))
+    return fail(MCP_E_ARG, "bad argument");
+  MCP_ON_STREAM_DEVICE(stream);
+  const int K = prm->n_portfolios;
+  const hipStream_t st = (hipStream_t)stream;
+#if MCP_EXP_FUSED_TAIL
+  HIP_TRY(mcp::launch_hist_tail(*prm, K, pass, d_terminal, stride, n, gamma, rank_lo, rank_hi, (mcp::SelectState*)d_state, d_pivot,
+                                (double*)d_below, (unsigned long long*)d_hist, (mcp_record*)d_record, (mcp::Quantile*)d_quant,
+                                (mcp_stats*)d_stats, st));
+#else
+  HIP_TRY(mcp::launch_hist(*prm, K, pass, d_terminal, stride, n, (const mcp::SelectState*)d_state, d_pivot, (double*)d_below,
+                           (unsigned long long*)d_hist, st));
+  if (pass == 1)
+    HIP_TRY(mcp::launch_scan(*prm, K, 1, n, rank_lo, rank_hi, mcp_moment_slots(K, n), nullptr, (const double*)d_below, d_pivot,
+                             (unsigned long long*)d_hist, (mcp::SelectState*)d_state, (mcp_record*)d_record, st));
+  else
+    HIP_TRY(mcp::launch_final(*prm, K, n, gamma, rank_lo, rank_hi, (const double*)d_below, (unsigned long long*)d_hist,
+                              (const mcp::SelectState*)d_state, (mcp_record*)d_record, (mcp::Quantile*)d_quant, (mcp_stats*)d_stats, st));
+#endif
+  return MCP_OK;
+}
+
 int mcp_launch_final(const mcp_params* prm, uint64_t n, double gamma, uint64_t rank_lo, uint64_t rank_hi,
                      const void* d_below, void* d_hist, const void* d_state, void* d_record, void* d_quant,
                      void* d_stats, void* stream) {
@@ -1665,6 +1694,17 @@
       const uint64_t stride = j.pn ? j.pn : 1;
       const double* piv = what == SEL_DRAWDOWN ? nullptr : what == SEL_HORIZON ? sh.hz.pivot.p : (const double*)sh.ws[MCP_WS_PIVOT];
       const float* src = what == SEL_DRAWDOWN ? sh.dd.mdd.p : what == SEL_HORIZON ? sh.hz.values.p : sh.terminal.p;
+      if (!exchange && tp[s].n_portfolios < mcp::SWEEP_MIN_K) {
+        if (pass == 0) {
+          if ((rc = mcp_launch_scan(&tp[s], 0, j.pn, lo, hi, sh.ws[MCP_WS_PARTIALS], sh.ws[MCP_WS_BELOW], piv, sh.ws[MCP_WS_HIST],
+                                    sh.ws[MCP_WS_STATE], sh.ws[MCP_WS_RECORD], sh.stream))) return rc;
+        } else if ((rc = mcp_launch_hist_tail(&tp[s], pass, src, stride, j.pn, gamma, lo, hi, sh.ws[MCP_WS_STATE], piv, sh.ws[MCP_WS_BELOW],
+                                              sh.ws[MCP_WS_HIST], sh.ws[MCP_WS_RECORD], sh.ws[MCP_WS_QUANT],
+                                              pass == 2 ? stats_of(sh, tp[s].n_portfolios) : nullptr, sh.stream))) {
+          return rc;
+        }
+        continue;
+      }
       if (pass < 2) {
         if ((rc = mcp_launch_scan(&tp[s], pass, j.pn, lo, hi, sh.ws[MCP_WS_PARTIALS], sh.ws[MCP_WS_BELOW], piv, sh.ws[MCP_WS_HIST],
                                   sh.ws[MCP_WS_STATE], sh.ws[MCP_WS_RECORD], sh.stream))) return rc;
diff --git a/monte_carlo_portfolio_amd/csrc/mcp_stats_kernels.h b/monte_carlo_portfolio_amd/csrc/mcp_stats_kernels.h
--- a/monte_carlo_portfolio_amd/csrc/mcp_stats_kernels.h
+++ b/monte_carlo_portfolio_amd/csrc/mcp_stats_kernels.h
@@ -76,6 +76,9 @@
                        SelectState* state, mcp_record* record, hipStream_t s);
 hipError_t launch_hist(const mcp_params& prm, int K, int pass, const float* terminal, uint64_t stride, uint64_t n,
                        const SelectState* state, const double* pivot, double* below, unsigned long long* hist, hipStream_t s);
+hipError_t launch_hist_tail(const mcp_params& prm, int K, int pass, const float* terminal, uint64_t stride, uint64_t n, double gamma,
+                            uint64_t rank_lo, uint64_t rank_hi, SelectState* state, const double* pivot, double* below,
+                            unsigned long long* hist, mcp_record* record, Quantile* quant, mcp_stats* stats_or_null, hipStream_t s);
 hipError_t launch_final(const mcp_params& prm, int K, uint64_t n, double gamma, uint64_t rank_lo, uint64_t rank_hi,
                         const double* below, unsigned long long* hist, const SelectState* state, mcp_record* record,
                         Quantile* quant, mcp_stats* stats_or_null, hipStream_t s);
diff --git a/monte_carlo_portfolio_amd/csrc/mcp_stats_kernels.hip b/monte_carlo_portfolio_amd/csrc/mcp_stats_kernels.hip
--- a/monte_carlo_portfolio_amd/csrc/mcp_stats_kernels.hip
+++ b/monte_carlo_portfolio_amd/csrc/mcp_stats_kernels.hip
@@ -89,95 +89,24 @@
   }
 }
 
-constexpr int WIN = 16;
-template <int PASS, bool LOGC>
-__global__ void __launch_bounds__(SB) hist_kernel(const mcp_params prm, const float* __restrict__ terminal, uint64_t stride, uint64_t n,
-                                                  int G, int slots, const SelectState* __restrict__ state, const double* __restrict__ pivot,
-                                                  double* __restrict__ below_out, unsigned long long* __restrict__ hist) {
-  constexpr int NH = PASS == 0 ? 1 : 2;
-  __shared__ uint32_t h[NH][MCP_SELECT_BINS];
-  __shared__ uint32_t win[PASS == 0 ? WIN : 1][64];
-  __shared__ double red[4];
-  const int k = blockIdx.x / G, b = blockIdx.x % G;
-  for (int i = threadIdx.x; i < NH * MCP_SELECT_BINS; i += SB) (&h[0][0])[i] = 0u;
-  if constexpr (PASS == 0)
-    for (int i = threadIdx.x; i < WIN * 64; i += SB) (&win[0][0])[i] = 0u;
-  __syncthreads();
-  int shift, bits, pshift;
-  pass_shape(PASS, shift, bits, pshift);
-  const uint32_t mask = (1u << bits) - 1u;
-  const double v0d = (double)(float)prm.v0;
-  uint32_t pa = 0, pb = 0, dlo = 0;
-  if constexpr (PASS == 0) {
-    const double c = pivot ? pivot[k] : 0.0;
-    const float vc = LOGC ? (float)log1p(c > -1.0 ? c : 0.0) : (float)(v0d * (1.0 + c));
-    const uint32_t dc = float_to_key(vc) >> 21;
-    dlo = dc >= WIN / 2 ? dc - WIN / 2 : 0u;
-    if (dlo > (uint32_t)(MCP_SELECT_BINS - WIN)) dlo = MCP_SELECT_BINS - WIN;
+template <bool HO>
+__device__ __forceinline__ unsigned long long ld_u64(const unsigned long long* p) {
+  if constexpr (HO) return __hip_atomic_load(p, __ATOMIC_RELAXED, __HIP_MEMORY_SCOPE_AGENT);
+  else return *p;
+}
+template <bool HO>
+__device__ __forceinline__ double ld_f64(const double* p) {
+  if constexpr (HO) return __longlong_as_double((long long)ld_u64<true>((const unsigned long long*)p));
+  else return *p;
+}
+template <bool HO>
+__device__ __forceinline__ SelectState ld_state(const SelectState* p) {
+  if constexpr (HO) {
+    const unsigned long long* q = (const unsigned long long*)p;
+    const unsigned long long w0 = ld_u64<true>(q), w1 = ld_u64<true>(q + 1);
+    return SelectState{(uint32_t)w0, (uint32_t)(w0 >> 32), w1};
   } else {
-    pa = state[2 * k + 0].prefix; pb = state[2 * k + 1].prefix;
-  }
-  const bool two = pa != pb;
-  const int lane = threadIdx.x & 63;
-  const float* __restrict__ src = terminal + (size_t)k * stride;
-  double below = 0.0;
-
-  auto one = [&](float v) {
-    const uint32_t key = float_to_key(v);
-    if constexpr (PASS == 0) {
-      const uint32_t d = key >> 21, t = d - dlo;
-      if (t < (uint32_t)WIN) atomicAdd(&win[t][lane], 1u);
-      else atomicAdd(&h[0][d], 1u);
-    } else {
-      const uint32_t pre = key >> pshift, d = (key >> shift) & mask;
-      if (pre == pa) atomicAdd(&h[0][d], 1u);
-      if (two && pre == pb) atomicAdd(&h[1][d], 1u);
-      if (pre < pa && (PASS == 1 || (pre >> 11) == (pa >> 11))) below += below_term<LOGC>(v, v0d);
-    }
-  };
-
-  const uint64_t head = n ? (uint64_t)((4 - (((uintptr_t)src >> 2) & 3)) & 3) : 0;
-  const uint64_t hd = head < n ? head : n;
-  const uint64_t nvec = (n - hd) / 4;
-  const float4* __restrict__ vsrc = (const float4*)(src + hd);
-  const uint64_t vstep = (uint64_t)G * SB;
-  uint64_t j = (uint64_t)b * SB + threadIdx.x;
-  for (; j + vstep < nvec; j += 2 * vstep) {
-    const float4 q0 = vsrc[j], q1 = vsrc[j + vstep];
-    one(q0.x); one(q0.y); one(q0.z); one(q0.w);
-    one(q1.x); one(q1.y); one(q1.z); one(q1.w);
-  }
-  for (; j < nvec; j += vstep) {
-    const float4 q0 = vsrc[j];
-    one(q0.x); one(q0.y); one(q0.z); one(q0.w);
-  }
-  if (b == 0) {
-    if (threadIdx.x < hd) one(src[threadIdx.x]);
-    const uint64_t t0 = hd + 4 * nvec;
-    if (t0 + threadIdx.x < n) one(src[t0 + threadIdx.x]);
-  }
-
-  if constexpr (PASS != 0) {
-    below = wave_sum(below);
-    const int wv = threadIdx.x >> 6;
-    if (lane == 0) red[wv] = below;
-  }
-  __syncthreads();
-  if constexpr (PASS != 0) {
-    if (threadIdx.x == 0) below_out[(size_t)k * slots + b] = (red[0] + red[1]) + (red[2] + red[3]);
-  } else {
-    if (threadIdx.x < WIN) {
-      uint32_t t = 0;
-      for (int l = 0; l < 64; l++) t += win[threadIdx.x][(l + threadIdx.x) & 63];
-      if (t) atomicAdd(&h[0][dlo + threadIdx.x], t);
-    }
-    __syncthreads();
-  }
-  unsigned long long* out = hist + (size_t)k * 2 * MCP_SELECT_BINS;
-  const int nh = (PASS == 0 || !two) ? 1 : 2;
-  for (int i = threadIdx.x; i < nh * MCP_SELECT_BINS; i += SB) {
-    const uint32_t cnt = (&h[0][0])[i];
-    if (cnt) atomicAdd(&out[i], (unsigned long long)cnt);
+    return *p;
   }
 }
 
@@ -215,6 +144,7 @@
       if (st.rank < before + c[i]) {
         st.prefix = (pass == 0 ? 0u : (st.prefix << bits)) | (uint32_t)(threadIdx.x * PER + i);
         st.rank -= before;
+        st.pad = 0u;
         *dst = st;
         break;
       }
@@ -223,16 +153,14 @@
   }
 }
 
-__global__ void __launch_bounds__(SB) scan_kernel(const mcp_params prm, int pass, uint64_t rank_lo, uint64_t rank_hi, int G, int bslots,
-                                                  uint64_t mslots, const MomentPartial* __restrict__ partials,
-                                                  const double* __restrict__ below, const double* __restrict__ pivot,
-                                                  unsigned long long* __restrict__ hist, SelectState* __restrict__ state,
-                                                  mcp_record* __restrict__ record) {
+template <bool HO>
+__device__ __forceinline__ void scan_body(const mcp_params& prm, int pass, int k, uint64_t rank_lo, uint64_t rank_hi, int G, int bslots,
+                                          uint64_t mslots, const MomentPartial* partials, const double* below, const double* pivot,
+                                          unsigned long long* hist, SelectState* state, mcp_record* record) {
   __shared__ unsigned long long wtot[4];
   __shared__ double red[4][2];
   __shared__ float ext[4][2];
   __shared__ unsigned long long cnt[4];
-  const int k = blockIdx.x;
   if (pass == 0) {
     const MomentPartial* pp = partials + (size_t)k * mslots;
     double s1 = 0.0, s2 = 0.0;
@@ -265,19 +193,19 @@
   } else {
     const double* pp = below + (size_t)k * bslots;
     double bl = 0.0;
-    for (int b = threadIdx.x; b < G; b += SB) bl += pp[b];
+    for (int b = threadIdx.x; b < G; b += SB) bl += ld_f64<HO>(pp + b);
     bl = block_sum(bl, &red[0][0]);
     if (threadIdx.x == 0) record[k].below = bl;
   }
-  const SelectState in0 = pass == 0 ? SelectState{0u, 0u, rank_lo} : state[2 * k + 0];
-  const SelectState in1 = pass == 0 ? SelectState{0u, 0u, rank_hi} : state[2 * k + 1];
+  const SelectState in0 = pass == 0 ? SelectState{0u, 0u, rank_lo} : ld_state<HO>(state + 2 * k + 0);
+  const SelectState in1 = pass == 0 ? SelectState{0u, 0u, rank_hi} : ld_state<HO>(state + 2 * k + 1);
   const bool shared_hist = pass == 0 || in0.prefix == in1.prefix;
 #pragma unroll 1
   for (int w = 0; w < 2; w++) {
     unsigned long long* hh = hist + ((size_t)k * 2 + (shared_hist ? 0 : w)) * MCP_SELECT_BINS;
     unsigned long long c[PER], tot = 0;
 #pragma unroll
-    for (int i = 0; i < PER; i++) { c[i] = hh[threadIdx.x * PER + i]; tot += c[i]; }
+    for (int i = 0; i < PER; i++) { c[i] = ld_u64<HO>(hh + threadIdx.x * PER + i); tot += c[i]; }
     SelectState st = w ? in1 : in0;
     const unsigned long long before = block_exclusive_scan(tot, wtot);
     descend(pass, c, tot, before, st, &state[2 * k + w]);
@@ -286,6 +214,14 @@
       for (int i = 0; i < PER; i++) hh[threadIdx.x * PER + i] = 0ull;
     }
   }
+}
+
+__global__ void __launch_bounds__(SB) scan_kernel(const mcp_params prm, int pass, uint64_t rank_lo, uint64_t rank_hi, int G, int bslots,
+                                                  uint64_t mslots, const MomentPartial* __restrict__ partials,
+                                                  const double* __restrict__ below, const double* __restrict__ pivot,
+                                                  unsigned long long* __restrict__ hist, SelectState* __restrict__ state,
+                                                  mcp_record* __restrict__ record) {
+  scan_body<false>(prm, pass, blockIdx.x, rank_lo, rank_hi, G, bslots, mslots, partials, below, pivot, hist, state, record);
 }
 
 __device__ __forceinline__ double key_to_x(uint32_t key, double v0d, int compounding) {
@@ -312,30 +248,29 @@
   *out = s;
 }
 
-__global__ void __launch_bounds__(SB) final_kernel(const mcp_params prm, double gamma, uint64_t rank_lo, uint64_t rank_hi, int G, int bslots,
-                                                   const double* __restrict__ below, unsigned long long* __restrict__ hist,
-                                                   const SelectState* __restrict__ state, mcp_record* __restrict__ record,
-                                                   Quantile* __restrict__ quant, mcp_stats* __restrict__ stats) {
+template <bool HO>
+__device__ __forceinline__ void final_body(const mcp_params& prm, int k, double gamma, uint64_t rank_lo, int G, int bslots,
+                                           const double* below, unsigned long long* hist, const SelectState* state, mcp_record* record,
+                                           Quantile* quant, mcp_stats* stats) {
   __shared__ unsigned long long wtot[4];
   __shared__ double red[4];
   __shared__ uint32_t s_key[2];
   __shared__ double s_q[3];
-  const int k = blockIdx.x;
   const double v0d = (double)(float)prm.v0;
   const double* pp = below + (size_t)k * bslots;
   double bl = 0.0;
-  for (int b = threadIdx.x; b < G; b += SB) bl += pp[b];
+  for (int b = threadIdx.x; b < G; b += SB) bl += ld_f64<HO>(pp + b);
   bl = block_sum(bl, red);
 
   unsigned long long c[2][PER];
-  const SelectState st0 = state[2 * k + 0], st1 = state[2 * k + 1];
+  const SelectState st0 = ld_state<HO>(state + 2 * k + 0), st1 = ld_state<HO>(state + 2 * k + 1);
   const bool shared_hist = st0.prefix == st1.prefix;
 #pragma unroll
   for (int w = 0; w < 2; w++) {
     unsigned long long* hh = hist + ((size_t)k * 2 + (shared_hist ? 0 : w)) * MCP_SELECT_BINS;
     unsigned long long tot = 0;
 #pragma unroll
-    for (int i = 0; i < PER; i++) { c[w][i] = hh[threadIdx.x * PER + i]; tot += c[w][i]; }
+    for (int i = 0; i < PER; i++) { c[w][i] = ld_u64<HO>(hh + threadIdx.x * PER + i); tot += c[w][i]; }
     if (!shared_hist || w == 1) {
 #pragma unroll
       for (int i = 0; i < PER; i++) hh[threadIdx.x * PER + i] = 0ull;
@@ -386,7 +321,140 @@
     record[k] = m;
     if (stats) finish_stats(prm, m, q, &stats[k]);
   }
+}
+
+__global__ void __launch_bounds__(SB) final_kernel(const mcp_params prm, double gamma, uint64_t rank_lo, uint64_t rank_hi, int G, int bslots,
+                                                   const double* __restrict__ below, unsigned long long* __restrict__ hist,
+                                                   const SelectState* __restrict__ state, mcp_record* __restrict__ record,
+                                                   Quantile* __restrict__ quant, mcp_stats* __restrict__ stats) {
+  final_body<false>(prm, blockIdx.x, gamma, rank_lo, G, bslots, below, hist, state, record, quant, stats);
   (void)rank_hi;
+}
+
+constexpr int WIN = 16;
+struct TailArgs {
+  double gamma;
+  uint64_t rank_lo, rank_hi;
+  SelectState* state;
+  mcp_record* record;
+  Quantile* quant;
+  mcp_stats* stats;
+};
+template <int PASS, bool LOGC, bool FUSED = false>
+__global__ void __launch_bounds__(SB) hist_kernel(const mcp_params prm, const float* __restrict__ terminal, uint64_t stride, uint64_t n,
+                                                  int G, int slots, const SelectState* __restrict__ state, const double* __restrict__ pivot,
+                                                  double* __restrict__ below_out, unsigned long long* __restrict__ hist, const TailArgs tail) {
+  static_assert(!FUSED || PASS != 0, "pass 0 has no tail to fuse");
+  constexpr int NH = PASS == 0 ? 1 : 2;
+  __shared__ uint32_t h[NH][MCP_SELECT_BINS];
+  __shared__ uint32_t win[PASS == 0 ? WIN : 1][64];
+  __shared__ double red[4];
+  const int k = blockIdx.x / G, b = blockIdx.x % G;
+  for (int i = threadIdx.x; i < NH * MCP_SELECT_BINS; i += SB) (&h[0][0])[i] = 0u;
+  if constexpr (PASS == 0)
+    for (int i = threadIdx.x; i < WIN * 64; i += SB) (&win[0][0])[i] = 0u;
+  __syncthreads();
+  int shift, bits, pshift;
+  pass_shape(PASS, shift, bits, pshift);
+  const uint32_t mask = (1u << bits) - 1u;
+  const double v0d = (double)(float)prm.v0;
+  uint32_t pa = 0, pb = 0, dlo = 0;
+  if constexpr (PASS == 0) {
+    const double c = pivot ? pivot[k] : 0.0;
+    const float vc = LOGC ? (float)log1p(c > -1.0 ? c : 0.0) : (float)(v0d * (1.0 + c));
+    const uint32_t dc = float_to_key(vc) >> 21;
+    dlo = dc >= WIN / 2 ? dc - WIN / 2 : 0u;
+    if (dlo > (uint32_t)(MCP_SELECT_BINS - WIN)) dlo = MCP_SELECT_BINS - WIN;
+  } else {
+    pa = state[2 * k + 0].prefix; pb = state[2 * k + 1].prefix;
+  }
+  const bool two = pa != pb;
+  const int lane = threadIdx.x & 63;
+  const float* __restrict__ src = terminal + (size_t)k * stride;
+  double below = 0.0;
+
+  auto one = [&](float v) {
+    const uint32_t key = float_to_key(v);
+    if constexpr (PASS == 0) {
+      const uint32_t d = key >> 21, t = d - dlo;
+      if (t < (uint32_t)WIN) atomicAdd(&win[t][lane], 1u);
+      else atomicAdd(&h[0][d], 1u);
+    } else {
+      const uint32_t pre = key >> pshift, d = (key >> shift) & mask;
+      if (pre == pa) atomicAdd(&h[0][d], 1u);
+      if (two && pre == pb) atomicAdd(&h[1][d], 1u);
+      if (pre < pa && (PASS == 1 || (pre >> 11) == (pa >> 11))) below += below_term<LOGC>(v, v0d);
+    }
+  };
+
+  const uint64_t head = n ? (uint64_t)((4 - (((uintptr_t)src >> 2) & 3)) & 3) : 0;
+  const uint64_t hd = head < n ? head : n;
+  const uint64_t nvec = (n - hd) / 4;
+  const float4* __restrict__ vsrc = (const float4*)(src + hd);
+  const uint64_t vstep = (uint64_t)G * SB;
+  uint64_t j = (uint64_t)b * SB + threadIdx.x;
+  for (; j + vstep < nvec; j += 2 * vstep) {
+    const float4 q0 = vsrc[j], q1 = vsrc[j + vstep];
+    one(q0.x); one(q0.y); one(q0.z); one(q0.w);
+    one(q1.x); one(q1.y); one(q1.z); one(q1.w);
+  }
+  for (; j < nvec; j += vstep) {
+    const float4 q0 = vsrc[j];
+    one(q0.x); one(q0.y); one(q0.z); one(q0.w);
+  }
+  if (b == 0) {
+    if (threadIdx.x < hd) one(src[threadIdx.x]);
+    const uint64_t t0 = hd + 4 * nvec;
+    if (t0 + threadIdx.x < n) one(src[t0 + threadIdx.x]);
+  }
+
+  if constexpr (PASS != 0) {
+    below = wave_sum(below);
+    const int wv = threadIdx.x >> 6;
+    if (lane == 0) red[wv] = below;
+  }
+  __syncthreads();
+  if constexpr (PASS != 0) {
+    if (threadIdx.x == 0) below_out[(size_t)k * slots + b] = (red[0] + red[1]) + (red[2] + red[3]);
+  } else {
+    if (threadIdx.x < WIN) {
+      uint32_t t = 0;
+      for (int l = 0; l < 64; l++) t += win[threadIdx.x][(l + threadIdx.x) & 63];
+      if (t) atomicAdd(&h[0][dlo + threadIdx.x], t);
+    }
+    __syncthreads();
+  }
+  unsigned long long* out = hist + (size_t)k * 2 * MCP_SELECT_BINS;
+  const int nh = (PASS == 0 || !two) ? 1 : 2;
+  for (int i = threadIdx.x; i < nh * MCP_SELECT_BINS; i += SB) {
+    const uint32_t cnt = (&h[0][0])[i];
+    if (cnt) atomicAdd(&out[i], (unsigned long long)cnt);
+  }
+  if constexpr (FUSED) {
+    __shared__ uint32_t s_last;
+    asm volatile("s_waitcnt vmcnt(0)" ::: "memory");
+    __syncthreads();
+    if (threadIdx.x == 0) {
+      __builtin_amdgcn_fence(__ATOMIC_RELEASE, "agent");
+      asm volatile("s_waitcnt vmcnt(0)" ::: "memory");
+      uint32_t* ticket = &tail.state[2 * k].pad;
+      const uint32_t t = __hip_atomic_fetch_add(ticket, 1u, __ATOMIC_RELAXED, __HIP_MEMORY_SCOPE_AGENT);
+      const bool last = t == (uint32_t)G - 1u;
+      if (last) {
+        __hip_atomic_store(ticket, 0u, __ATOMIC_RELAXED, __HIP_MEMORY_SCOPE_AGENT);
+        __builtin_amdgcn_fence(__ATOMIC_ACQUIRE, "agent");
+        asm volatile("s_waitcnt vmcnt(0)" ::: "memory");
+      }
+      s_last = last ? 1u : 0u;
+    }
+    __syncthreads();
+    if (s_last) {
+      if constexpr (PASS == 1)
+        scan_body<true>(prm, 1, k, tail.rank_lo, tail.rank_hi, G, slots, 0, nullptr, below_out, pivot, hist, tail.state, tail.record);
+      else
+        final_body<true>(prm, k, tail.gamma, tail.rank_lo, G, slots, below_out, hist, tail.state, tail.record, tail.quant, tail.stats);
+    }
+  }
 }
 
 __global__ void stats_kernel(const mcp_params prm, int K, int world, const mcp_record* __restrict__ gathered,
@@ -454,13 +522,35 @@
   const unsigned grid = (unsigned)(K * G);
   const int bs = stream_slots(K);
   const bool lg = prm.compounding == MCP_COMPOUND_LOG;
-#define MCP_HIST(P)                                                                                              \
-  do {                                                                                                           \
-    if (lg) hist_kernel<P, true><<<grid, SB, 0, s>>>(prm, terminal, stride, n, G, bs, state, pivot, below, hist); \
-    else hist_kernel<P, false><<<grid, SB, 0, s>>>(prm, terminal, stride, n, G, bs, state, pivot, below, hist);   \
+  const TailArgs none = {0.0, 0, 0, nullptr, nullptr, nullptr, nullptr};
+#define MCP_HIST(P)                                                                                                    \
+  do {                                                                                                                 \
+    if (lg) hist_kernel<P, true><<<grid, SB, 0, s>>>(prm, terminal, stride, n, G, bs, state, pivot, below, hist, none); \
+    else hist_kernel<P, false><<<grid, SB, 0, s>>>(prm, terminal, stride, n, G, bs, state, pivot, below, hist, none);   \
   } while (0)
   if (pass == 0) MCP_HIST(0);
   else if (pass == 1) MCP_HIST(1);
+  else if (pass == 2) MCP_HIST(2);
+  else return hipErrorInvalidValue;
+#undef MCP_HIST
+  return hipGetLastError();
+}
+
+hipError_t launch_hist_tail(const mcp_params& prm, int K, int pass, const float* terminal, uint64_t stride, uint64_t n, double gamma,
+                            uint64_t rank_lo, uint64_t rank_hi, SelectState* state, const double* pivot, double* below,
+                            unsigned long long* hist, mcp_record* record, Quantile* quant, mcp_stats* stats_or_null, hipStream_t s) {
+  const int G = stream_grid(n, K);
+  if (!grid_ok(K, G)) return hipErrorInvalidValue;
+  const unsigned grid = (unsigned)(K * G);
+  const int bs = stream_slots(K);
+  const bool lg = prm.compounding == MCP_COMPOUND_LOG;
+  const TailArgs tail = {gamma, rank_lo, rank_hi, state, record, quant, stats_or_null};
+#define MCP_HIST(P)                                                                                                          \
+  do {                                                                                                                       \
+    if (lg) hist_kernel<P, true, true><<<grid, SB, 0, s>>>(prm, terminal, stride, n, G, bs, state, pivot, below, hist, tail); \
+    else hist_kernel<P, false, true><<<grid, SB, 0, s>>>(prm, terminal, stride, n, G, bs, state, pivot, below, hist, tail);   \
+  } while (0)
+  if (pass == 1) MCP_HIST(1);
   else if (pass == 2) MCP_HIST(2);
   else return hipErrorInvalidValue;
 #undef MCP_HIST
diff --git a/monte_carlo_portfolio_amd/engine.py b/monte_carlo_portfolio_amd/engine.py
--- a/monte_carlo_portfolio_amd/engine.py
+++ b/monte_carlo_portfolio_amd/engine.py
@@ -46,6 +46,11 @@
         _ffi.check(self.lib.mcp_launch_final(ctypes.byref(prm), n, gamma, lo, hi, self._p(below), self._p(hist),
                                              self._p(state), self._p(record), self._p(quant), self._p(stats), self._stream()))
 
+    def hist_tail(self, prm, p, terminal, n, gamma, lo, hi, state, pivot, below, hist, record, quant, stats):
+        _ffi.check(self.lib.mcp_launch_hist_tail(ctypes.byref(prm), p, self._p(terminal), terminal.shape[1], n, gamma, lo, hi,
+                                                 self._p(state), self._p(pivot), self._p(below), self._p(hist), self._p(record),
+                                                 self._p(quant), self._p(stats), self._stream()))
+
     def stats(self, prm, world, gathered, quant, stats):
         _ffi.check(self.lib.mcp_launch_stats(ctypes.byref(prm), world, self._p(gathered), self._p(quant), self._p(stats),
                                              self._stream()))
@@ -58,11 +63,12 @@
 class PathEngine:
 
     N_STAGES = 4
+    FUSED_TAIL_MAX_K = 16
 
     def __init__(self, mu32, chol32, W32, n_steps, n_paths_local, *, compounding="simple", v0=1.0, alpha=0.95,
                  rf=0.0, native_math=False, device=None, group=None, world_size=1, rank=0, kernels=None,
                  pipeline=True, shard="paths", n_buffers=None, fold=False, logical_shards=1, skew=None, fused=True, cu_reserve=0,
-                 n_stats_streams=None):
+                 n_stats_streams=None, fused_tail=None):
         import torch
 
         self.torch = torch
@@ -100,10 +106,15 @@
         self.rank_lo, self.rank_hi, self.gamma = _ffi.percentile_rank(self.n_total, alpha)
         self.pipeline = bool(pipeline) and self.device.type == "cuda"
         self.exchanging = self.group is not None or self.S > 1
+        can_fuse = not self.exchanging and K <= self.FUSED_TAIL_MAX_K and hasattr(self.k, "hist_tail")
+        if fused_tail and not can_fuse:
+            raise ValueError("fused_tail needs one shard, no process group, K <= 16 and kernels that offer hist_tail")
+        self.fused_tail = can_fuse if fused_tail is None else bool(fused_tail)
+        self.n_stages = 2 if self.fused_tail else self.N_STAGES
         self.skew = (self.group is not None and self.pipeline) if skew is None else bool(skew)
         if n_stats_streams is None:
             n_stats_streams = 1 if self.group is not None else 2
-        self.depth = self.N_STAGES if self.skew else 0
+        self.depth = self.n_stages if self.skew else 0
         if n_buffers:
             self.n_buf = int(n_buffers) if (self.pipeline or self.skew) else 1
         else:
@@ -211,7 +222,16 @@
     def _stage(self, i, s):
         k, prm, lo, hi = self.k, self.prm, self.rank_lo, self.rank_hi
         row = self.bufs[i]
-        if s <= 3:
+        if self.fused_tail:
+            b = row[0]
+            ws, n = b["ws"], b["n"]
+            with self._on_stats(i, 0):
+                if s == 1:
+                    k.scan(prm, 0, n, lo, hi, ws[_ffi.WS_PARTIALS], ws[_ffi.WS_BELOW], self.d_pivot, ws[_ffi.WS_HIST],
+                           ws[_ffi.WS_STATE], ws[_ffi.WS_RECORD])
+                k.hist_tail(prm, s, b["terminal"], n, self.gamma, lo, hi, ws[_ffi.WS_STATE], self.d_pivot, ws[_ffi.WS_BELOW],
+                            ws[_ffi.WS_HIST], ws[_ffi.WS_RECORD], ws[_ffi.WS_QUANT], ws[_ffi.WS_STATS] if s == 2 else None)
+        elif s <= 3:
             if self.exchanging:
                 self._exchange_hist(i)
             for j, b in enumerate(row):
@@ -281,7 +301,7 @@
         self.stage_done[t] = 0
         self.t = t + 1
         if self.skew:
-            for s in range(1, self.N_STAGES + 1):
+            for s in range(1, self.n_stages + 1):
                 bt = t - s
                 if bt in self.stage_done and self.stage_done[bt] == s - 1:
                     self._advance(bt)
@@ -291,7 +311,7 @@
 
     def _advance(self, bt):
         s = self.stage_done[bt] + 1
-        last_stage = self.N_STAGES if self.exchanging else self.N_STAGES - 1
+        last_stage = self.n_stages if self.exchanging or self.fused_tail else self.n_stages - 1
         i = bt % self.n_buf
         if s <= last_stage:
             self._stage(i, s)
```

Result: no change. 452.6 million paths/s (-0.1%).
